# SUSTech-SLAM-XYZZY/SurfelMapping

Hardware: AMD Instinct MI355X
Metric: frames/sec per GPU, 1242x375 KITTI-shaped RGB-D+semantic, full associate+fuse+merge (higher is better)
Workload: dtype f32; 1 GPU; BASELINE configs[1]: KITTI 1242x375 synthetic street sequence, 0.8 m/frame, depth noise 15.0 mm, metricise+conflict+cull+splat+associate+fuse+append per frame; frames=5..6245, multi_gpu=single stream, surfels_start=157613, surfels_end=5487352

## Files before the change

include/sm_c_api.h:

```cpp
#ifndef SM_C_API_H
#define SM_C_API_H

#include <stddef.h>
#include <stdint.h>

#ifdef __cplusplus
extern "C" {
#endif

#define SM_API_VERSION 4

enum {
    SM_OK = 0,
    SM_E_ARG = -1,
    SM_E_CAPACITY = -2,
    SM_E_UNSUPPORTED = -3,
    SM_E_HIP = -4,
    SM_E_NO_DEVICE = -5,
    SM_E_STALL = -6
};

typedef struct sm_config {
    int32_t width, height;
    float fx, fy, cx, cy;
// ... 238 lines not shown
int sm_track_debug_window(sm_ctx *s, const uint16_t *depth_mm, const float *pose16_eval, int32_t min_time, int32_t max_time,
                          int32_t *pred_slot, double *sys29);
int sm_track_frame_rgb_window(sm_ctx *s, const uint8_t *rgb, const uint16_t *depth_mm, const float *guess16, const sm_track_params *params,
                              const sm_track_rgb_params *rgb_params, int32_t min_time, int32_t max_time, float *pose16_out,
                              sm_track_info *info, sm_track_rgb_info *rgb_info, float *anchor_time);
int sm_track_rgb_debug_window(sm_ctx *s, const uint8_t *rgb, const uint16_t *depth_mm, const float *pose16_eval, int level, int which,
                              int32_t min_time, int32_t max_time, int32_t *pred_slot, double *sys29);
int sm_close_loop_rgb(sm_ctx *s, const uint8_t *rgb, const uint16_t *depth_mm, const float *pose16, const sm_map_source *src,
                      const sm_track_params *tp, const sm_track_rgb_params *rp, const sm_loop_params *lp, float *pose16_out,
                      sm_loop_info *info);
int sm_old_in_view(sm_ctx *s, const float *pose16, int32_t max_time, uint32_t *n);
typedef struct sm_auto_loop_params {
    int32_t every, rest;
    uint32_t min_old;
    sm_loop_params loop;
} sm_auto_loop_params;
typedef struct sm_auto_loop_stats_t {
    uint32_t checked, attempts;
    uint32_t closed, none, rejected, failed, no_old_map;
    uint32_t last_census;
    sm_loop_info last;
} sm_auto_loop_stats_t;
int sm_default_auto_loop_params(const sm_config *c, sm_auto_loop_params *p);
int sm_set_auto_loop(sm_ctx *s, const sm_auto_loop_params *p, const sm_map_source *src);
int sm_auto_loop_stats(sm_ctx *s, sm_auto_loop_stats_t *out);

typedef struct sm_search_params {
    int32_t levels;
    float trans_half[3];
    float trans_step[3];
    float rot_half_deg[3];
    float rot_step_deg[3];
    int32_t refine;
    int32_t stride0;
    int32_t top_k;
    float colour_thresh;
} sm_search_params;
typedef struct sm_search_info {
    int32_t status;
    int32_t levels_run;
    uint32_t candidates[4];
    uint32_t best_score[4];
    int32_t winner_rank;
    sm_track_info track;
    float start[16];
    float anchor_time;
    float score_ms, total_ms;
} sm_search_info;
#define SM_SEARCH_MAX_CANDIDATES (1u << 20)
int sm_default_search_params(sm_search_params *p);
int sm_score_poses_window(sm_ctx *s, const uint8_t *rgb, const uint16_t *depth_mm, const float *cand16, uint32_t n,
                          const sm_track_params *tp, int32_t stride, float colour_thresh, int32_t min_time, int32_t max_time,
                          uint32_t *scores);
int sm_search_pose(sm_ctx *s, const uint8_t *rgb, const uint16_t *depth_mm, const float *centre16, const sm_track_params *tp,
                   const sm_track_rgb_params *rp, const sm_search_params *sp, int32_t min_time, int32_t max_time, float *pose16_out,
                   sm_search_info *info);
int sm_close_loop_search(sm_ctx *s, const uint8_t *rgb, const uint16_t *depth_mm, const float *pose16, const sm_map_source *src,
                         const sm_track_params *tp, const sm_track_rgb_params *rp, const sm_loop_params *lp, const sm_search_params *sp,
                         float *pose16_out, sm_loop_info *info);
int sm_set_auto_loop_search(sm_ctx *s, const sm_search_params *sp);

int sm_set_frame(sm_ctx *s, const uint8_t *rgb, const float *depth_metric,
                 const uint8_t *semantic);
int sm_set_tick(sm_ctx *s, int32_t tick);
int sm_stage_conflict(sm_ctx *s, const float *pose16, float min_depth, float max_depth,
                      float fuse_thresh, int is_clean);
int sm_stage_cull(sm_ctx *s);
int sm_stage_splat(sm_ctx *s, const float *pose16, int32_t time, float depth_cutoff,
                   int32_t time_delta);
int sm_stage_associate_fuse(sm_ctx *s, const float *pose16, int32_t time, float depth_min,
                            float depth_max);

int sm_stage_timings(sm_ctx *s, sm_timings *out);
int sm_read_frame_log(sm_ctx *s, sm_frame_log *out, uint32_t n, uint32_t *written);

void *sm_device_alloc(sm_ctx *s, size_t bytes);
int sm_device_free(sm_ctx *s, void *p);
int sm_device_upload(sm_ctx *s, void *dst_device, const void *src_host, size_t bytes);
int sm_export_model_device(sm_ctx *s, void **d_aos, uint32_t *n);
int sm_append_model_aos_device(sm_ctx *s, const float *d_src12, uint32_t n);
int sm_device_download(sm_ctx *s, void *dst_host, const void *src_device, size_t bytes);

int sm_debug_slow_frames(sm_ctx *s, uint32_t *n);
int sm_gpu_process_count(sm_ctx *s);

enum { SM_COLL_SUM = 0, SM_COLL_MIN = 1, SM_COLL_GATHER = 2 };
typedef int (*sm_collective_fn)(void *user, const void *send, void *recv, size_t count, int op, void *hip_stream);
int sm_shard_stream_configure(sm_ctx *s, int rank, int world);
int sm_shard_set_collective(sm_ctx *s, sm_collective_fn fn, void *user);
int sm_shard_rccl_unique_id(void *out128);
int sm_shard_rccl_init(sm_ctx *s, const void *id128);
int sm_shard_rccl_finalize(sm_ctx *s);
int sm_shard_rccl_nranks(sm_ctx *s);
int sm_shard_frame_device(sm_ctx *s, const uint8_t *d_rgb, const uint16_t *d_depth_mm, const uint8_t *d_semantic, const float *pose16);
int sm_shard_frame(sm_ctx *s, const uint8_t *rgb, const uint16_t *depth_mm, const uint8_t *semantic, const float *pose16);
int sm_shard_compact(sm_ctx *s);
int sm_shard_export_dense_device(sm_ctx *s, const float **d_out12, uint32_t *count);

int sm_rig_configure(sm_ctx *s, int rank, int world);
int sm_rig_consolidate(sm_ctx *s, const uint16_t *depth_mm, const uint8_t *semantic, const float *pose16, sm_ctx *global,
                       uint32_t *view_conflicts, uint32_t *total);
int sm_rig_consolidate_step(sm_ctx *s, const uint16_t *depth_mm, const uint8_t *semantic, const float *pose16, sm_ctx *global,
                            uint32_t *new_surfels, uint32_t *global_count);

#ifdef __cplusplus
}
#endif
#endif
```

surfelmapping_amd/capi.py:

```python
from __future__ import annotations

import ctypes as C
import os

import numpy as np

_PKG = os.path.dirname(os.path.abspath(__file__))
LIB_PATH = os.environ.get("SM_HIP_LIB") or os.path.join(_PKG, "libsurfelmapping_hip.so")
API_VERSION = 4

SM_OK, SM_E_ARG, SM_E_CAPACITY, SM_E_UNSUPPORTED, SM_E_HIP, SM_E_NO_DEVICE = 0, -1, -2, -3, -4, -5
TEX_DEPTH_METRIC, TEX_DEPTH_FILTERED, TEX_LAST = 0, 1, 2

SYMBOLS = (
    "sm_api_version", "sm_last_error", "sm_default_config", "sm_create", "sm_destroy",
    "sm_process_frame", "sm_process_frame_device", "sm_process_frame_async",
    "sm_inputs_consumed", "sm_host_alloc", "sm_host_alloc_frame", "sm_host_free", "sm_debug_slow_frames", "sm_sync", "sm_clean_points", "sm_clean_points_ex", "sm_clean_points_cb", "sm_reset",
    "sm_get_counts", "sm_download_model_aos", "sm_upload_model_aos", "sm_save_map", "sm_load_map",
    "sm_download_index_map", "sm_download_raw_cloud", "sm_download_depth", "sm_render_image", "sm_render_model",
    "sm_render_model_device", "sm_render_image_maps", "sm_render_model_maps", "sm_render_maps_stats", "sm_set_frame", "sm_set_tick",
    "sm_stage_conflict", "sm_stage_cull", "sm_stage_splat", "sm_stage_associate_fuse",
    "sm_stage_timings", "sm_read_frame_log", "sm_device_alloc", "sm_device_free", "sm_device_upload",
    "sm_export_model_device", "sm_append_model_aos_device", "sm_device_download",
    "sm_shard_stream_configure", "sm_shard_set_collective", "sm_shard_rccl_unique_id", "sm_shard_rccl_init",
    "sm_shard_rccl_finalize", "sm_shard_rccl_nranks", "sm_shard_frame_device", "sm_shard_frame", "sm_shard_compact", "sm_shard_export_dense_device",
    "sm_gpu_process_count", "sm_rig_configure", "sm_rig_consolidate", "sm_rig_consolidate_step",
    "sm_default_track_params", "sm_track_frame", "sm_track_debug",
    "sm_default_track_rgb_params", "sm_track_frame_rgb", "sm_track_rgb_debug",
    "sm_default_retire_params", "sm_retire", "sm_retire_device", "sm_set_auto_retire", "sm_auto_retire_stats",
    "sm_default_recall_params", "sm_recall", "sm_recall_stats", "sm_set_auto_recall", "sm_auto_recall_stats",
    "sm_warp_by_time", "sm_warp_stats", "sm_loop_spread", "sm_track_frame_old", "sm_track_debug_old",
    "sm_default_loop_params", "sm_close_loop",
    "sm_track_frame_window", "sm_track_debug_window", "sm_track_frame_rgb_window", "sm_track_rgb_debug_window", "sm_close_loop_rgb",
    "sm_old_in_view", "sm_default_auto_loop_params", "sm_set_auto_loop", "sm_auto_loop_stats",
    "sm_default_search_params", "sm_score_poses_window", "sm_search_pose", "sm_close_loop_search", "sm_set_auto_loop_search",
)

SM_COLL_SUM, SM_COLL_MIN, SM_COLL_GATHER = 0, 1, 2
COLLECTIVE_FN = C.CFUNCTYPE(C.c_int, C.c_void_p, C.c_void_p, C.c_void_p, C.c_size_t, C.c_int, C.c_void_p)
CAP_FN = C.CFUNCTYPE(C.c_longlong, C.c_void_p, C.c_uint32)


class SmConfig(C.Structure):
    _fields_ = [
        ("width", C.c_int32), ("height", C.c_int32),
        ("fx", C.c_float), ("fy", C.c_float), ("cx", C.c_float), ("cy", C.c_float),
        ("near_clip", C.c_float), ("far_clip", C.c_float), ("fuse_thresh", C.c_float),
        ("max_sqrt_vertices", C.c_int32), ("time_delta", C.c_int32),
        ("stereo_border", C.c_float), ("preprocess", C.c_int32), ("conflict_cap", C.c_int32),
        ("device", C.c_int32), ("enable_timing", C.c_int32), ("disable_tile_bounds", C.c_int32),
        ("compact_period", C.c_int32),
    ]


class SmCounts(C.Structure):
    _fields_ = [
        ("count", C.c_uint32), ("offset", C.c_uint32), ("data_count", C.c_uint32),
        ("conflict_count", C.c_uint32), ("unstable_count", C.c_uint32),
        ("fused_count", C.c_uint32), ("visible_count", C.c_uint32), ("tick", C.c_int32),
    ]

    def as_dict(self):
        return {n: getattr(self, n) for n, _ in self._fields_}


class SmTimings(C.Structure):
    _fields_ = [(n, C.c_float) for n in (
        "preprocess", "conflict", "index_map", "data_association", "concatenate", "run",
        "k_prep", "k_conflict", "k_scan_cull", "k_compact", "k_associate", "k_scan_new",
        "k_append")] + [("frames", C.c_uint32), ("event_overhead", C.c_float), ("k_compact_own", C.c_float),
                        ("k_cull_lazy", C.c_float), ("frames_compact", C.c_uint32)] + [(n, C.c_float) for n in (
        "k_surfel_pass", "k_pass_fixup", "k_conflict_own", "k_associate_direct", "k_associate_own", "k_append_own")] + [
        ("frames_one_pass", C.c_uint32), ("frames_direct", C.c_uint32), ("k_assoc_prep", C.c_float), ("k_prep_own", C.c_float),
        ("frames_merged", C.c_uint32), ("frames_assoc_alone", C.c_uint32), ("k_scan_own", C.c_float)]

    def as_dict(self):
        return {n: getattr(self, n) for n, _ in self._fields_}


FRAME_LOG_LEN = 1024
FRAME_LOG_DTYPE = np.dtype([(n, np.uint32) for n in (
    "tick", "n_before", "n_after_cull", "n_kill", "conflict_count", "visible_count",
    "fused_count", "unstable_count", "n_static", "n_conf_skipped", "n_splat_skipped", "n_slots")])


class SmModelView(C.Structure):
    _fields_ = [
        ("mvp", C.c_float * 16), ("mv_inv", C.c_float * 16), ("threshold", C.c_float), ("color_type", C.c_int32),
        ("draw_unstable", C.c_int32), ("draw_points", C.c_int32), ("draw_window", C.c_int32), ("time", C.c_int32),
        ("time_delta", C.c_int32), ("width", C.c_int32), ("height", C.c_int32), ("clear_rgba", C.c_uint8 * 4),
    ]


class SmMapSource(C.Structure):
    _fields_ = [("paths", C.POINTER(C.c_char_p)), ("n_paths", C.c_uint32), ("include_model", C.c_int32)]


class SmMapsStats(C.Structure):
    _fields_ = [("surfels_read", C.c_uint64), ("chunks", C.c_uint32), ("passes", C.c_uint32), ("pairs_tested", C.c_uint64),
                ("pairs_skipped", C.c_uint64), ("read_ms", C.c_float), ("copy_ms", C.c_float), ("device_ms", C.c_float),
# ... 229 lines not shown
    def __init__(self, what, rc, detail=""):
        super().__init__(f"{what} failed: rc={rc} {detail}".strip())
        self.rc = rc


_lib = None


def _preload_torch_hip_runtime():
    if os.environ.get("SM_NO_TORCH_HIP_PRELOAD") == "1":
        return
    import importlib.util
    import sys
    if "torch" in sys.modules:
        return
    try:
        spec = importlib.util.find_spec("torch")
    except (ImportError, ValueError):
        return
    if not spec or not spec.submodule_search_locations:
        return
    cand = os.path.join(list(spec.submodule_search_locations)[0], "lib", "libamdhip64.so")
    if os.path.exists(cand):
        try:
            C.CDLL(cand, mode=C.RTLD_GLOBAL)
        except OSError:
            pass


def _choose_rccl():
    if os.environ.get("SM_RCCL_LIB") or os.environ.get("SM_NO_TORCH_HIP_PRELOAD") == "1":
        return
    import importlib.util
    try:
        spec = importlib.util.find_spec("torch")
    except (ImportError, ValueError):
        return
    if spec and spec.submodule_search_locations:
        cand = os.path.join(list(spec.submodule_search_locations)[0], "lib", "librccl.so")
        if os.path.exists(cand):
            os.environ["SM_RCCL_LIB"] = cand


def rccl_unique_id() -> bytes:
    _choose_rccl()
    L = load()
    buf = C.create_string_buffer(128)
    rc = L.sm_shard_rccl_unique_id(buf)
    if rc:
        raise SurfelMapError("sm_shard_rccl_unique_id", rc, L.sm_last_error().decode())
    return buf.raw


def load():
    global _lib
    if _lib is not None:
        return _lib
    if not os.path.exists(LIB_PATH):
        raise ImportError(
            f"{LIB_PATH} is missing: build it with `python -c 'import __graft_entry__ as g; g.build()'` "
            "(make -C surfelmapping_amd/csrc). surfelmapping_amd has no CPU fallback.")
    _preload_torch_hip_runtime()
    L = C.CDLL(LIB_PATH)
    vp, u32p = C.c_void_p, C.POINTER(C.c_uint32)
    L.sm_api_version.restype = C.c_int
    if L.sm_api_version() != API_VERSION:
        raise ImportError(f"{LIB_PATH} has API version {L.sm_api_version()}, this binding expects {API_VERSION}: rebuild it "
                          "(python -c 'import __graft_entry__ as g; g.build()')")
    L.sm_last_error.restype = C.c_char_p
    L.sm_default_config.argtypes = [C.POINTER(SmConfig), C.c_int, C.c_int] + [C.c_float] * 4
    L.sm_create.restype = vp
    L.sm_create.argtypes = [C.POINTER(SmConfig)]
    L.sm_destroy.restype = None
    L.sm_destroy.argtypes = [vp]
    L.sm_process_frame.argtypes = [vp, vp, vp, vp, vp]
    L.sm_process_frame_device.argtypes = [vp, vp, vp, vp, vp]
    L.sm_process_frame_async.argtypes = [vp, vp, vp, vp, vp]
    L.sm_inputs_consumed.argtypes = [vp]
    L.sm_host_alloc.restype = vp
    L.sm_host_alloc.argtypes = [vp, C.c_size_t]
    L.sm_host_free.argtypes = [vp, vp]
    L.sm_host_alloc_frame.argtypes = [vp, C.POINTER(vp), C.POINTER(vp), C.POINTER(vp)]
    L.sm_debug_slow_frames.argtypes = [vp, u32p]
    L.sm_sync.argtypes = [vp]
    L.sm_clean_points.argtypes = [vp, vp, vp, vp]
    L.sm_clean_points_ex.argtypes = [vp, vp, vp, vp, C.c_int]
    L.sm_clean_points_cb.argtypes = [vp, vp, vp, vp, C.c_int, CAP_FN, vp]
    L.sm_reset.argtypes = [vp]
    L.sm_get_counts.argtypes = [vp, C.POINTER(SmCounts)]
    L.sm_download_model_aos.argtypes = [vp, vp, C.c_uint32, u32p]
    L.sm_upload_model_aos.argtypes = [vp, vp, C.c_uint32]
    L.sm_save_map.argtypes = [vp, C.c_char_p, C.c_int32, C.c_int32]
    L.sm_load_map.argtypes = [vp, C.c_char_p, C.POINTER(C.c_int32), C.POINTER(C.c_int32)]
    L.sm_download_index_map.argtypes = [vp, vp, vp, vp, vp]
    L.sm_download_raw_cloud.argtypes = [vp, vp, C.c_uint32, u32p]
    L.sm_download_depth.argtypes = [vp, C.c_int, vp]
    L.sm_render_image.argtypes = [vp, vp, C.c_int, C.c_int] + [C.c_float] * 4 + [vp, vp]
    L.sm_render_model.argtypes = [vp, C.POINTER(SmModelView), vp, vp, vp]
    L.sm_render_model_device.argtypes = [vp, C.POINTER(SmModelView), vp, vp, vp]
    L.sm_render_image_maps.argtypes = [vp, C.POINTER(SmMapSource), vp, C.c_uint32, C.c_int, C.c_int] + [C.c_float] * 4 + [vp, vp]
    L.sm_render_model_maps.argtypes = [vp, C.POINTER(SmMapSource), C.POINTER(SmModelView), C.c_uint32, vp, vp, vp]
    L.sm_render_maps_stats.argtypes = [vp, C.POINTER(SmMapsStats)]
    L.sm_set_frame.argtypes = [vp, vp, vp, vp]
    L.sm_set_tick.argtypes = [vp, C.c_int32]
    L.sm_stage_conflict.argtypes = [vp, vp, C.c_float, C.c_float, C.c_float, C.c_int]
    L.sm_stage_cull.argtypes = [vp]
    L.sm_stage_splat.argtypes = [vp, vp, C.c_int32, C.c_float, C.c_int32]
    L.sm_stage_associate_fuse.argtypes = [vp, vp, C.c_int32, C.c_float, C.c_float]
    L.sm_stage_timings.argtypes = [vp, C.POINTER(SmTimings)]
    L.sm_read_frame_log.argtypes = [vp, vp, C.c_uint32, u32p]
    L.sm_device_alloc.restype = vp
    L.sm_device_alloc.argtypes = [vp, C.c_size_t]
    L.sm_device_free.argtypes = [vp, vp]
    L.sm_device_upload.argtypes = [vp, vp, vp, C.c_size_t]
    L.sm_export_model_device.argtypes = [vp, C.POINTER(vp), u32p]
    L.sm_append_model_aos_device.argtypes = [vp, vp, C.c_uint32]
    L.sm_device_download.argtypes = [vp, vp, vp, C.c_size_t]
    L.sm_shard_stream_configure.argtypes = [vp, C.c_int, C.c_int]
    L.sm_shard_set_collective.argtypes = [vp, COLLECTIVE_FN, vp]
    L.sm_shard_rccl_unique_id.argtypes = [vp]
    L.sm_shard_rccl_init.argtypes = [vp, vp]
    L.sm_shard_rccl_finalize.argtypes = [vp]
    L.sm_shard_rccl_nranks.argtypes = [vp]
    L.sm_shard_frame_device.argtypes = [vp, vp, vp, vp, vp]
    L.sm_shard_frame.argtypes = [vp, vp, vp, vp, vp]
    L.sm_shard_compact.argtypes = [vp]
    L.sm_shard_export_dense_device.argtypes = [vp, C.POINTER(vp), u32p]
    L.sm_gpu_process_count.argtypes = [vp]
    L.sm_rig_configure.argtypes = [vp, C.c_int, C.c_int]
    L.sm_rig_consolidate.argtypes = [vp, vp, vp, vp, vp, u32p, u32p]
    L.sm_rig_consolidate_step.argtypes = [vp, vp, vp, vp, vp, u32p, u32p]
    L.sm_default_track_params.argtypes = [C.POINTER(SmTrackParams)]
    L.sm_track_frame.argtypes = [vp, vp, vp, C.POINTER(SmTrackParams), vp, C.POINTER(SmTrackInfo)]
    L.sm_track_debug.argtypes = [vp, vp, vp, vp, vp]
    L.sm_default_track_rgb_params.argtypes = [C.POINTER(SmTrackRgbParams)]
    L.sm_track_frame_rgb.argtypes = [vp, vp, vp, vp, C.POINTER(SmTrackParams), C.POINTER(SmTrackRgbParams), vp,
                                     C.POINTER(SmTrackInfo), C.POINTER(SmTrackRgbInfo)]
    L.sm_track_rgb_debug.argtypes = [vp, vp, vp, vp, C.c_int, C.c_int, vp]
    L.sm_default_retire_params.argtypes = [C.POINTER(SmConfig), C.POINTER(SmRetireParams)]
    L.sm_retire.argtypes = [vp, vp, C.POINTER(SmRetireParams), vp, C.c_uint32, u32p]
    L.sm_retire_device.argtypes = [vp, vp, C.POINTER(SmRetireParams), vp, C.c_uint32, u32p]
    L.sm_set_auto_retire.argtypes = [vp, C.POINTER(SmRetireParams), C.c_int32, C.c_char_p]
    L.sm_auto_retire_stats.argtypes = [vp, u32p, C.POINTER(C.c_uint64)]
    L.sm_default_recall_params.argtypes = [C.POINTER(SmConfig), C.POINTER(SmRecallParams)]
    L.sm_recall.argtypes = [vp, C.POINTER(SmMapSource), vp, C.POINTER(SmRecallParams), C.c_int32, u32p]
    L.sm_recall_stats.argtypes = [vp, C.POINTER(SmRecallStats)]
    L.sm_set_auto_recall.argtypes = [vp, C.POINTER(SmRecallParams)]
    L.sm_auto_recall_stats.argtypes = [vp, u32p, C.POINTER(C.c_uint64)]
    L.sm_warp_by_time.argtypes = [vp, C.POINTER(SmMapSource), C.c_int32, C.c_uint32, vp]
    L.sm_warp_stats.argtypes = [vp, C.POINTER(SmWarpStats)]
    L.sm_loop_spread.argtypes = [vp, C.c_int32, C.c_int32, vp]
    L.sm_track_frame_old.argtypes = [vp, vp, vp, C.POINTER(SmTrackParams), C.c_int32, vp, C.POINTER(SmTrackInfo), C.POINTER(C.c_float)]
    L.sm_track_debug_old.argtypes = [vp, vp, vp, C.c_int32, vp, vp]
    L.sm_default_loop_params.argtypes = [C.POINTER(SmConfig), C.POINTER(SmLoopParams)]
    L.sm_close_loop.argtypes = [vp, vp, vp, C.POINTER(SmMapSource), C.POINTER(SmTrackParams), C.POINTER(SmLoopParams), vp,
                                C.POINTER(SmLoopInfo)]
    i32, tpp, rpp, lpp = C.c_int32, C.POINTER(SmTrackParams), C.POINTER(SmTrackRgbParams), C.POINTER(SmLoopParams)
    L.sm_track_frame_window.argtypes = [vp, vp, vp, tpp, i32, i32, vp, C.POINTER(SmTrackInfo), C.POINTER(C.c_float)]
    L.sm_track_debug_window.argtypes = [vp, vp, vp, i32, i32, vp, vp]
    L.sm_track_frame_rgb_window.argtypes = [vp, vp, vp, vp, tpp, rpp, i32, i32, vp, C.POINTER(SmTrackInfo), C.POINTER(SmTrackRgbInfo),
                                            C.POINTER(C.c_float)]
    L.sm_track_rgb_debug_window.argtypes = [vp, vp, vp, vp, C.c_int, C.c_int, i32, i32, vp, vp]
    L.sm_close_loop_rgb.argtypes = [vp, vp, vp, vp, C.POINTER(SmMapSource), tpp, rpp, lpp, vp, C.POINTER(SmLoopInfo)]
    L.sm_old_in_view.argtypes = [vp, vp, i32, u32p]
    L.sm_default_auto_loop_params.argtypes = [C.POINTER(SmConfig), C.POINTER(SmAutoLoopParams)]
    L.sm_set_auto_loop.argtypes = [vp, C.POINTER(SmAutoLoopParams), C.POINTER(SmMapSource)]
# ... 11 lines not shown


def _ptr(a):
    return None if a is None else a.ctypes.data_as(C.c_void_p)


def make_config(width, height, fx, fy, cx, cy, **over) -> SmConfig:
    c = SmConfig()
    load().sm_default_config(C.byref(c), width, height, fx, fy, cx, cy)
    for k, v in over.items():
        if not hasattr(c, k):
            raise KeyError(k)
        setattr(c, k, v)
    return c


class SurfelMap:

    def __init__(self, cfg: SmConfig):
        self._L = load()
        self.cfg = cfg
        self.W, self.H = cfg.width, cfg.height
        self.P = self.W * self.H
        self._h = self._L.sm_create(C.byref(cfg))
        if not self._h:
            raise SurfelMapError("sm_create", SM_E_NO_DEVICE, self._L.sm_last_error().decode())

    def _chk(self, rc, what, allow=(0,)):
        if rc not in allow:
            raise SurfelMapError(what, rc, self._L.sm_last_error().decode())
        return rc

    def close(self):
        if getattr(self, "_h", None):
            self._L.sm_destroy(self._h)
            self._h = None

    def __del__(self):
        try:
            self.close()
        except Exception:
            pass

    def process_frame(self, rgb, depth, sem, pose, allow=(0,)):
        rgb = np.ascontiguousarray(rgb, np.uint8)
        depth = None if depth is None else np.ascontiguousarray(depth, np.uint16)
        sem = None if sem is None else np.ascontiguousarray(sem, np.uint8)
        pose = np.ascontiguousarray(pose, np.float32)
        return self._chk(self._L.sm_process_frame(self._h, _ptr(rgb), _ptr(depth), _ptr(sem), _ptr(pose)),
                         "sm_process_frame", allow)

    def process_frame_device(self, d_rgb, d_depth, d_sem, pose):
        pose = np.ascontiguousarray(pose, np.float32)
        return self._chk(self._L.sm_process_frame_device(self._h, d_rgb, d_depth, d_sem, _ptr(pose)),
                         "sm_process_frame_device")

    def process_frame_async(self, rgb, depth, sem, pose):
        assert rgb.dtype == np.uint8 and rgb.flags.c_contiguous
        pose = np.ascontiguousarray(pose, np.float32)
        return self._chk(self._L.sm_process_frame_async(self._h, _ptr(rgb), _ptr(depth), _ptr(sem), _ptr(pose)), "sm_process_frame_async")

    def host_array(self, shape, dtype) -> np.ndarray:
        n = int(np.prod(shape)) * np.dtype(dtype).itemsize
        p = self._L.sm_host_alloc(self._h, n)
        if not p:
            raise SurfelMapError("sm_host_alloc", SM_E_HIP, self._L.sm_last_error().decode())
        buf = (C.c_ubyte * n).from_address(p)
        return np.frombuffer(buf, dtype=dtype).reshape(shape)

    def host_frame(self):
        a, b, c = C.c_void_p(), C.c_void_p(), C.c_void_p()
        self._chk(self._L.sm_host_alloc_frame(self._h, C.byref(a), C.byref(b), C.byref(c)), "sm_host_alloc_frame")
        H, W = self.H, self.W
        rgb = np.frombuffer((C.c_ubyte * (H * W * 3)).from_address(a.value), dtype=np.uint8).reshape(H, W, 3)
        dep = np.frombuffer((C.c_ubyte * (H * W * 2)).from_address(b.value), dtype=np.uint16).reshape(H, W)
        sem = np.frombuffer((C.c_ubyte * (H * W)).from_address(c.value), dtype=np.uint8).reshape(H, W)
        return rgb, dep, sem

    def debug_slow_frames(self) -> int:
        n = C.c_uint32()
        self._chk(self._L.sm_debug_slow_frames(self._h, C.byref(n)), "sm_debug_slow_frames")
        return int(n.value)

    def inputs_consumed(self):
        self._chk(self._L.sm_inputs_consumed(self._h), "sm_inputs_consumed")

    def sync(self, allow=(0,)):
        return self._chk(self._L.sm_sync(self._h), "sm_sync", allow)

    def clean_points(self, depth, sem, pose):
        depth = np.ascontiguousarray(depth, np.uint16)
        sem = np.ascontiguousarray(sem, np.uint8)
        pose = np.ascontiguousarray(pose, np.float32)
        self._chk(self._L.sm_clean_points(self._h, _ptr(depth), _ptr(sem), _ptr(pose)), "sm_clean_points")

    def clean_points_slice(self, depth, sem, pose, exempt_first: bool, cap_hook=None):
        depth = np.ascontiguousarray(depth, np.uint16)
        sem = np.ascontiguousarray(sem, np.uint8)
        pose = np.ascontiguousarray(pose, np.float32)
        if cap_hook is None:
            self._chk(self._L.sm_clean_points_ex(self._h, _ptr(depth), _ptr(sem), _ptr(pose), 1 if exempt_first else 0), "sm_clean_points_ex")
            return
        err = []

        def tramp(user, local):
            try:
                return int(cap_hook(int(local)))
            except Exception as e:
                err.append(e)
                return SM_E_HIP
        cb = CAP_FN(tramp)
        rc = self._L.sm_clean_points_cb(self._h, _ptr(depth), _ptr(sem), _ptr(pose), 1 if exempt_first else 0, cb, None)
        if err:
            raise err[0]
        self._chk(rc, "sm_clean_points_cb")

    def reset(self):
        self._chk(self._L.sm_reset(self._h), "sm_reset")

    def track(self, depth, guess=None, **params):
        depth = np.ascontiguousarray(depth, np.uint16)
        assert depth.size == self.P, depth.shape
        g = None if guess is None else _mat16(guess)
        p = track_params(**params) if params else None
        out = np.zeros(16, np.float32)
        info = SmTrackInfo()
        self._chk(self._L.sm_track_frame(self._h, _ptr(depth), _ptr(g), C.byref(p) if p is not None else None, _ptr(out),
                                         C.byref(info)), "sm_track_frame")
        d = dict(status=TRACK_STATUS.get(info.status, str(info.status)), status_code=int(info.status),
                 iterations=int(info.iterations), inliers=int(info.inliers), rmse=float(info.rmse),
                 guess=np.array(info.guess[:], np.float32).reshape(4, 4).T.copy())
        return out.reshape(4, 4).T.copy(), d

    def track_debug(self, depth, pose_eval):
        depth = np.ascontiguousarray(depth, np.uint16)
        assert depth.size == self.P, depth.shape
        pe = _mat16(pose_eval)
        pred = np.zeros((self.H, self.W), np.int32)
        sys29 = np.zeros(29, np.float64)
        self._chk(self._L.sm_track_debug(self._h, _ptr(depth), _ptr(pe), _ptr(pred), _ptr(sys29)), "sm_track_debug")
        return pred, sys29

    def track_stats(self):
        f = self._L.sm_debug_track_stats
        f.argtypes = [C.c_void_p, C.POINTER(C.c_float), C.c_int, C.POINTER(C.c_int)]
        ms, n = (C.c_float * 256)(), C.c_int()
        self._chk(f(self._h, ms, 256, C.byref(n)), "sm_debug_track_stats")
        return [float(x) for x in ms[:n.value]]

    def process_frame_tracked(self, rgb, depth, sem, guess=None, **params):
        pose, info = self.track(depth, guess, **params)
        self.process_frame(rgb, depth, sem, _mat16(pose))
        return pose, info

    _RGB_KEYS = ("levels", "iters", "rgb_weight", "rgb_max_residual")

    def track_rgb(self, rgb, depth, guess=None, **params):
        rgb = np.ascontiguousarray(rgb, np.uint8)
        depth = np.ascontiguousarray(depth, np.uint16)
        assert depth.size == self.P and rgb.size == self.P * 3, (depth.shape, rgb.shape)
        g = None if guess is None else _mat16(guess)
        icp = {k: v for k, v in params.items() if k not in self._RGB_KEYS}
        col = {k: v for k, v in params.items() if k in self._RGB_KEYS}
        p = track_params(**icp) if icp else None
        q = track_rgb_params(**col) if col else None
        out = np.zeros(16, np.float32)
# ... 551 lines not shown
```

surfelmapping_amd/csrc/sm_api.hip:

```cpp
#include "sm_ctx.h"
#include "sm_kernels.h"

#include <hip/hip_runtime.h>

#include <dirent.h>
#include <link.h>

#include <algorithm>
#include <chrono>
#include <cmath>
#include <cstdio>
#include <cstdlib>
#include <cstring>
#include <atomic>
#include <functional>
#include <memory>
#include <mutex>
#include <string>
#include <thread>
#include <vector>

using namespace sm;

namespace {
// ... 60 lines not shown
    if (sscanf(bus, "%x:%x:%x.%x", &dom, &b, &d, &f) != 4) return -1;
    const unsigned long want_loc = ((unsigned long)b << 8) | ((unsigned long)d << 3) | f;
    unsigned long gpuid = 0;
    bool found = false;
    for (int n = 0; n < 64 && !found; ++n) {
        char path[128];
        snprintf(path, sizeof path, "/sys/class/kfd/kfd/topology/nodes/%d/properties", n);
        FILE *fp = fopen(path, "r");
        if (!fp) { if (n > 16) break; continue; }
        char key[64]; unsigned long val, loc = ~0ul, domain = 0;
        while (fscanf(fp, "%63s %lu", key, &val) == 2) {
            if (!strcmp(key, "location_id")) loc = val;
            else if (!strcmp(key, "domain")) domain = val;
        }
        fclose(fp);
        if (loc == want_loc && domain == dom) {
            snprintf(path, sizeof path, "/sys/class/kfd/kfd/topology/nodes/%d/gpu_id", n);
            FILE *fg = fopen(path, "r");
            if (fg) { found = fscanf(fg, "%lu", &gpuid) == 1 && gpuid != 0; fclose(fg); }
        }
    }
    if (!found) return -1;
    DIR *pd = opendir("/sys/class/kfd/kfd/proc");
    if (!pd) return -1;
    int procs = 0;
    while (struct dirent *pe = readdir(pd)) {
        if (pe->d_name[0] < '0' || pe->d_name[0] > '9') continue;
        char qdir[256];
        snprintf(qdir, sizeof qdir, "/sys/class/kfd/kfd/proc/%s/queues", pe->d_name);
        DIR *qd = opendir(qdir);
        if (!qd) continue;
        bool here = false;
        while (struct dirent *qe = readdir(qd)) {
            if (qe->d_name[0] < '0' || qe->d_name[0] > '9') continue;
            char gp[400];
            snprintf(gp, sizeof gp, "%s/%s/gpuid", qdir, qe->d_name);
            FILE *fg = fopen(gp, "r");
            unsigned long g = 0;
            if (fg) { if (fscanf(fg, "%lu", &g) == 1 && g == gpuid) here = true; fclose(fg); }
            if (here) break;
        }
        closedir(qd);
        if (here) ++procs;
    }
    closedir(pd);
    return procs;
}

bool gpu_shared_with_other_process(int dev)
{
    static std::mutex mu;
    static std::chrono::steady_clock::time_point last[MAX_DEV];
    static int cached[MAX_DEV];
    static bool valid[MAX_DEV] = {};
    if (dev < 0 || dev >= MAX_DEV) return false;
    std::lock_guard<std::mutex> lk(mu);
    const auto now = std::chrono::steady_clock::now();
    if (!valid[dev] || std::chrono::duration_cast<std::chrono::milliseconds>(now - last[dev]).count() > 1000) {
        cached[dev] = kfd_processes_on_gpu(dev);
        last[dev] = now; valid[dev] = true;
    }
    return cached[dev] > 1;
}

bool compaction_needs_tickets(const sm_ctx *s)
{
    const int dev = s->cfg.device;
    if (s->sw.compact_tickets >= 0) return s->sw.compact_tickets != 0;
    if (dev < 0 || dev >= MAX_DEV) return true;
    {
        std::lock_guard<std::mutex> lk(g_compact_mu);
        if (g_ctx_on_dev[dev] > 1) return true;
    }
    return gpu_shared_with_other_process(dev);
}

Switches read_switches()
{
    Switches sw;
    auto off = [](const char *name) { const char *e = std::getenv(name); return e && e[0] == '0'; };
    auto num = [](const char *name, long unset) { const char *e = std::getenv(name); return e ? std::atol(e) : unset; };
    sw.defer_assoc = !off("SM_DEFER_ASSOC");
    sw.two_launch = !off("SM_TWO_LAUNCH");
    sw.pass_split = (int)num("SM_PASS_SPLIT", 0);
    if (const char *e = std::getenv("SM_PASS_TRACE")) { sw.trace = true; sw.trace_prefix = e; }
    if (std::getenv("SM_COMPACT_TICKETS")) sw.compact_tickets = off("SM_COMPACT_TICKETS") ? 0 : 1;
    sw.capacity_wait_us = num("SM_CAPACITY_WAIT_US", 2000);
    sw.check_alive = std::getenv("SM_CHECK_ALIVE") != nullptr;
    if (std::getenv("SM_PASS_WG_PER_CU")) sw.pass_wg_per_cu = (int)std::max(1l, num("SM_PASS_WG_PER_CU", 1));
    if (std::getenv("SM_COMPACT_WG_PER_CU")) sw.compact_wg_per_cu = (int)std::max(1l, num("SM_COMPACT_WG_PER_CU", 1));
    return sw;
}

void resident_grids(const Switches &sw, int device, int *pass_grid, int *compact_grid)
{
    int cus = 0, per_cu = 0;
    if (hipDeviceGetAttribute(&cus, hipDeviceAttributeMultiprocessorCount, device) != hipSuccess || cus <= 0) return;
    if (hipOccupancyMaxActiveBlocksPerMultiprocessor(&per_cu, k_surfel_pass<1>, 256, 0) == hipSuccess && per_cu > 0) {
        const int want = sw.pass_wg_per_cu ? sw.pass_wg_per_cu : std::max(1, per_cu - 1);
        *pass_grid = std::max(256, std::min(cus * want, MAX_GRID));
    }
    if (hipOccupancyMaxActiveBlocksPerMultiprocessor(&per_cu, k_compact<true>, 256, 0) == hipSuccess && per_cu > 0) {
        const int want = sw.compact_wg_per_cu ? std::min(per_cu, sw.compact_wg_per_cu) : std::min(per_cu, 4);
        *compact_grid = std::max(1, cus * want);
    }
}

int alloc_set(SetBufs &b, size_t cap)
{
    return dalloc(b.pos_conf, cap) || dalloc(b.norm_rad, cap) || dalloc(b.color, cap) || dalloc(b.init_time, cap) ||
           dalloc(b.time, cap) ? SM_E_HIP : SM_OK;
}

int grid_surfels(const sm_ctx *s)
{
    return (int)std::min<uint64_t>(std::max<uint64_t>(s->slots.tiles(), 1), MAX_GRID);
}

void check_alive(sm_ctx *s, uint32_t stage)
{
    if (!s->d_chk) return;
    hipLaunchKernelGGL(k_check_alive, dim3(64), dim3(256), 0, s->stream, s->d_state, s->d_alive, s->d_tile_dead, s->d_chk, stage);
}

int take_error(sm_ctx *s)
{
    if (s->h_state->error != 0) {
        const int e = s->h_state->error;
        s->h_state->error = 0;
        HIPCK(hipMemcpyAsync(&s->d_state->error, &s->h_state->error, sizeof(int32_t), hipMemcpyHostToDevice, s->stream));
        HIPCK(hipStreamSynchronize(s->stream));
        g_err = e == SM_E_CAPACITY ? "model capacity (MAX_VERTICES) exceeded; frame's new surfels dropped"
              : e == SM_E_UNSUPPORTED ? "unsupported operation flagged on the device"
              : "device-side error";
        return e;
    }
    return SM_OK;
}


static inline uint32_t assoc_wgs(const sm_ctx *s)
{
    return (uint32_t)(s->n_pix_blocks + 1) / 2u;
}

int launch_fixup(sm_ctx *s, const FrameParams &fp, const FixArgs &x)
{
    hipLaunchKernelGGL(k_pass_fixup, dim3(x.n_crew + 1), dim3(256), 0, s->stream, s->M, s->d_state, fp, x);
    HIPCK(hipGetLastError());
    return SM_OK;
}

int launch_assoc(sm_ctx *s, const AssocArgs &a, uint32_t stage)
{
    hipLaunchKernelGGL((k_associate_direct<false>), dim3(assoc_wgs(s)), dim3(PIX_BLOCK), 0, s->stream, a, ShardArgs{});
    HIPCK(hipGetLastError());
    check_alive(s, stage + 16u * (uint32_t)(s->tick & 0xFFFF));
    return SM_OK;
}

int launch_settle(sm_ctx *s, const ShardSettle &ss)
{
    hipLaunchKernelGGL(k_shard_settle, dim3(ss.n), dim3(PIX_BLOCK), 0, s->stream, ss);
    HIPCK(hipGetLastError());
    return SM_OK;
}
// ... 2 lines not shown
{
    FixArgs *fx;
    if (const AssocArgs *a = s->held.take_assoc(fx)) {
        if (fx && launch_fixup(s, a->fp, *fx)) return SM_E_HIP;
        if (launch_assoc(s, *a, 3u)) return SM_E_HIP;
    }
    if (!all) return SM_OK;
    if (const ShardSettle *ss = s->held.take_settle()) if (launch_settle(s, *ss)) return SM_E_HIP;
    if (uint32_t *nf = s->held.take_stats()) {
        hipLaunchKernelGGL(k_frame_finalize, dim3(1), dim3(256), 0, s->stream, s->d_state, nf, s->part.fix_cur(), s->part.n_fix, s->d_log);
        HIPCK(hipGetLastError());
    }
    return SM_OK;
}

int launch_prep(sm_ctx *s, const uint8_t *rgb, const uint16_t *raw, const uint8_t *sem, const FrameParams &fp, bool clear_keys,
                bool tile_flags = false, bool carry = false, const ChainArgs *chain = nullptr)
{
    const int tiles = ((s->W + 31) / 32) * ((s->H + 31) / 32);
    TilePrep tp{};
    const uint64_t ntl = s->slots.tiles();
    const FrameSet &f = s->cur();
    if (clear_keys && tile_flags) {
        tp.nfb = (uint32_t)std::min<uint64_t>(std::max<uint64_t>((ntl + 1023) / 1024, 1), 64);
        tp.st = s->d_state; tp.tb = s->d_tb; tp.tile_flags = f.tile_flags; tp.wave_cnt = f.wave_cnt; tp.prep_part = f.prep_part;
    }
    FixArgs *fxp = nullptr;
    AssocArgs *carried = carry ? s->held.take_assoc(fxp) : nullptr;
    s->tl.frame().merged = carried || chain;
    uint32_t *conf_sub = clear_keys ? f.conf_sub : nullptr;
    if (carried || chain) {
        if (const ShardSettle *ss = chain ? s->held.take_settle() : nullptr) if (launch_settle(s, *ss)) return SM_E_HIP;
        static const AssocArgs none{};
        const AssocArgs &a = carried ? *carried : none;
        if (tp.nfb) {
            tp.nfb = (uint32_t)std::min<uint64_t>(std::max<uint64_t>((ntl + 255) / 256, 1), 128);
            if (carried) { tp.grp_cand = a.grp_cand; tp.n_grp = a.n_grp; tp.prev_time = a.fp.time; }
        }
        const FixArgs fx = fxp ? *fxp : FixArgs{};
        const uint32_t n_fix = fxp ? 1u + fx.n_crew : 0u;
        if (fxp) {
            carried->slow_conf_sub = fx.conf_sub; carried->slow_need = n_fix;
            if (tp.nfb) { tp.slow_conf_sub = fx.conf_sub; tp.slow_cap = a.fp.conflict_cap; tp.slow_need = n_fix; tp.slow_par = a.fp.par; }
        }
        PrepArgs pa;
        pa.rgb = rgb; pa.depth_raw = raw; pa.sem = sem; pa.depth_f32 = nullptr; pa.depthT = f.depthT; pa.rgbsT = f.rgbsT;
        pa.keyT = clear_keys ? s->keyT() : nullptr; pa.dcT = f.dcT;
        pa.conf_sub = conf_sub;
        const uint32_t n_assoc = carried ? assoc_wgs(s) : 0u;
        const ChainArgs ca = chain ? *chain : ChainArgs{};
        const uint32_t n_img = chain ? (uint32_t)(((s->W + CH_TX - 1) / CH_TX) * ((s->H + CH_TY - 1) / CH_TY)) : (uint32_t)tiles;
        if (s->d_ap_trace) { s->ap_trace_n[0] = (int)n_assoc; s->ap_trace_n[1] = (int)tp.nfb; s->ap_trace_n[2] = (int)n_img; s->ap_trace_n[3] = (int)n_fix; }
        const dim3 grid(n_fix + tp.nfb + n_assoc + n_img);
        const auto assoc_prep = chain ? k_assoc_prep<true> : k_assoc_prep<false>;
        hipLaunchKernelGGL(assoc_prep, grid, dim3(PIX_BLOCK), 0, s->stream, a, pa, fp, tp, n_assoc, n_img, ca, fx, n_fix, s->d_ap_trace);
        HIPCK(hipGetLastError());
        return (int)tp.nfb;
    }
    const ShardSettle *held = s->held.take_settle();
    const ShardSettle ss = held ? *held : ShardSettle{};
    hipLaunchKernelGGL(k_prep, dim3(tiles + tp.nfb + (ss.n + 3u) / 4u), dim3(1024), 0, s->stream, rgb, raw, sem, (const float *)nullptr, f.depthT, f.rgbsT,
                       clear_keys ? s->keyT() : nullptr, fp, f.dcT, conf_sub, tp, ss);
    HIPCK(hipGetLastError());
    return (int)tp.nfb;
}

int launch_conflict_test(sm_ctx *s, const FrameParams &fp, bool timed = false)
{
    if (finalize_if_pending(s)) return SM_E_HIP;
    s->n_conf_part = (uint32_t)grid_surfels(s);
    hipLaunchKernelGGL(k_conflict, dim3(s->n_conf_part), dim3(256), 0, s->stream, s->M, s->d_state, fp, s->cur().dcT,
                       s->d_cm, s->d_dm, s->d_zm, s->d_tile_cnt, s->d_tb, s->cur().tile_flags, s->d_conf_part, s->d_alive,
                       s->cur().conf_sub);
    HIPCK(hipGetLastError());
    if (s->tl.mark(s->stream, 2, timed)) return SM_E_HIP;
    return SM_OK;
}

int launch_conflict_finalize(sm_ctx *s, const FrameParams &fp, bool timed = false)
{
    if (fp.compact_now) {
        const int ngroups = std::max<int>(1, (int)((s->slots.tiles() + GROUP - 1) / GROUP));
        hipLaunchKernelGGL(k_scan_cull, dim3(ngroups), dim3(1024), 0, s->stream, s->d_state, s->d_tile_cnt, s->d_tile_allow,
                           s->d_tile_keep, s->d_group_tot, s->d_tile_dead);
        HIPCK(hipGetLastError());
    }
    hipLaunchKernelGGL(k_cull_finalize, dim3(1), dim3(1024), 0, s->stream, s->d_state, fp, s->d_cm, s->d_dm, s->d_zm,
                       s->d_tile_cnt, s->d_tile_allow, s->d_tile_keep, s->d_group_tot, s->d_group_base, s->d_conf_part, s->n_conf_part,
                       s->d_alive, s->d_tile_dead, s->d_stat);
    HIPCK(hipGetLastError());
    if (s->tl.mark(s->stream, 3, timed)) return SM_E_HIP;
    return SM_OK;
}

int launch_conflict(sm_ctx *s, const FrameParams &fp, bool timed = false)
{
    int rc = launch_conflict_test(s, fp, timed);
    if (rc) return rc;
    return launch_conflict_finalize(s, fp, timed);
}

struct PassGrid { int split, grid, fix_workers; };

PassGrid pass_grid_policy(sm_ctx *s, bool two, bool direct)
{
    const uint64_t tiles_b = s->slots.tiles_of(s->slots.estimate_slots());
    const bool persistent = tiles_b > (uint64_t)(4 * MAX_GRID);
    PassGrid g;
    g.split = s->sw.pass_split == 1 || s->sw.pass_split == 4 ? s->sw.pass_split : persistent ? 1 : 4;
    g.grid = persistent ? std::min(grid_surfels(s), s->pass_grid) : grid_surfels(s);
    if (g.split == 4) {
        const int max_seq = 3 * MAX_GRID / 16;
        g.grid = 4 * (int)std::min<uint64_t>(std::max<uint64_t>(s->slots.tiles(), 1), (uint64_t)max_seq);
    }
    g.fix_workers = two ? (int)sm_ctx::N_CREW
                  : direct ? std::max(std::min(g.grid, s->fix_grid), (int)std::min<uint32_t>(s->n_grp, MAX_GRID)) : std::min(g.grid, s->fix_grid);
    return g;
}

int launch_surfel_pass(sm_ctx *s, const FrameParams &fp, bool timed, bool direct, uint32_t n_prep)
{
    if (n_prep == 0) { g_err = "internal: one-pass frame without tile flags from the preparation launch"; return SM_E_ARG; }
    const bool two = s->sw.two_launch && s->defer_ok && timed && direct;
    const PassGrid g = pass_grid_policy(s, two, direct);
    const int grid = g.grid;
    PassPartials &pp = s->part;
    const uint32_t n_fix_prev = pp.n_fix;
    const uint2 *fix_prev = pp.fix_cur();
    pp.fix_set ^= 1;
    s->n_conf_part = (uint32_t)grid;
    pp.n_compact = (uint32_t)grid;
    pp.pass_live = true;
    pp.n_fix = (uint32_t)g.fix_workers;
    const FrameSet &f = s->cur();
    uint32_t *sub = f.conf_sub;
    const uint32_t tile_bound = (uint32_t)std::max<uint64_t>(s->slots.tiles(), 1);
    if (s->d_pass_trace) s->pass_trace_grid = grid;
    CandArgs ca{};
    ca.n_pass = (uint32_t)grid;
    if (two) {
        ca.n_grp = s->n_grp; ca.cg = s->cand_group; ca.n_pix_blocks = s->n_pix_blocks;
        ca.depthT = f.depthT; ca.xs = s->d_xs; ca.ys = s->d_ys; ca.blk_cand = s->d_blk_cand; ca.grp_cand = s->d_grp_cand;
    }
    const auto pass = g.split == 4 ? k_surfel_pass<4> : k_surfel_pass<1>;
    hipLaunchKernelGGL(pass, dim3(grid + (two ? (int)s->n_grp : 0)), dim3(256), 0, s->stream, s->M, s->d_state, fp, f.dcT, s->d_cm, s->d_dm ,
                       f.wave_cnt, s->d_tb, f.tile_flags, pp.d_lazy, s->d_alive, s->d_tile_dead, sub, s->keyT(), s->d_undo, tile_bound,
                       s->d_frame_sub, ca, s->d_pass_trace);
    HIPCK(hipGetLastError());
    if (s->tl.mark(s->stream, 2, timed) || s->tl.mark(s->stream, 3, timed)) return SM_E_HIP;
    FixArgs x{};
    DirectArgs &da = x.da;
    da.on = direct ? (two ? 2 : 1) : 0;
    da.blk_cand = s->d_blk_cand; da.grp_cand = s->d_grp_cand; da.n_grp = s->n_grp; da.cg = s->cand_group; da.n_pix_blocks = s->n_pix_blocks;
    da.depthT = f.depthT; da.xs = s->d_xs; da.ys = s->d_ys;
    da.frame_sub = s->d_frame_sub;
    da.nf_prev = s->prev().nf_sub;
    da.fix_prev = fix_prev; da.n_fix_prev = s->held.take_stats() ? n_fix_prev : 0u;
    da.log = s->d_log;
    x.cm = s->d_cm; x.km = s->d_dm; x.wave_cnt = f.wave_cnt; x.tile_flags = f.tile_flags; x.part = pp.d_lazy; x.n_part = (uint32_t)grid;
    x.fix_part = pp.fix_cur(); x.alive = s->d_alive; x.tile_dead = s->d_tile_dead; x.conf_sub = sub; x.keyT = s->keyT(); x.undo = s->d_undo;
    x.host_stat = s->d_stat; x.prep_part = f.prep_part; x.n_prep = n_prep; x.tb = s->d_tb; x.n_crew = (uint32_t)g.fix_workers;
    if (two) s->held.hold_fixup(x);
    else if (launch_fixup(s, fp, x)) return SM_E_HIP;
    if (s->tl.mark(s->stream, 4, timed)) return SM_E_HIP;
    check_alive(s, 1u + 16u * (uint32_t)(s->tick & 0xFFFF));
    return SM_OK;
}

void fill_assoc_args(const sm_ctx *s, const FrameParams &fp, AssocArgs &a)
{
    a.M = s->M; a.st = s->d_state; a.fp = fp;
    const FrameSet &f = s->cur();
    a.depthT = f.depthT; a.rgbsT = f.rgbsT; a.keyT = s->keyT(); a.xs = s->d_xs; a.ys = s->d_ys;
    a.blk_cand = s->d_blk_cand; a.grp_cand = s->d_grp_cand; a.nf = f.nf_sub; a.tb = s->d_tb;
    a.alive = s->d_alive; a.tile_dead = s->d_tile_dead; a.n_grp = s->n_grp; a.cg = s->cand_group; a.host_stat = s->d_stat;
    a.slow_conf_sub = nullptr; a.slow_need = 0u;
}

int launch_associate_direct(sm_ctx *s, const FrameParams &fp, bool timed)
{
    AssocArgs a;
    fill_assoc_args(s, fp, a);
    s->tl.frame().deferred = s->defer_ok;
    if (s->defer_ok && timed) s->held.hold_assoc(a);
    else if (launch_assoc(s, a, 2u)) return SM_E_HIP;
    s->part.clear();
    s->held.hold_stats(s->cur().nf_sub);
    s->slots.append_enqueued();
    if (s->tl.mark(s->stream, 5, timed) || s->tl.mark(s->stream, 6, timed) || s->tl.mark(s->stream, 7, timed)) return SM_E_HIP;
    return SM_OK;
}

int launch_compact(sm_ctx *s, const FrameParams &fp, bool splat, bool timed)
{
    s->part.clear();
    if (!fp.compact_now) {
        if (splat) { g_err = "internal: a frame's cull that only marks the dead is k_surfel_pass"; return SM_E_ARG; }
        const int grid = grid_surfels(s);
        s->part.n_compact = 0u;
        hipLaunchKernelGGL(k_cull_lazy, dim3(grid), dim3(256), 0, s->stream, s->M, s->d_state, fp, s->d_cm, s->d_dm, s->d_zm,
                           s->d_tile_cnt, s->d_tile_allow, s->d_alive, s->d_tile_dead);
        HIPCK(hipGetLastError());
        if (s->tl.mark(s->stream, 4, timed)) return SM_E_HIP;
        return SM_OK;
    }
    const int grid = std::min(grid_surfels(s), s->compact_grid);
    const uint32_t epoch = s->slots.next_cull_epoch();
    if (!fp.maintenance) s->part.n_compact = splat ? (uint32_t)grid : 0u;
    FrameParams fpc = fp;
    fpc.compact_tickets = compaction_needs_tickets(s) ? 1 : 0;
    const auto compact = splat ? k_compact<true> : k_compact<false>;
    hipLaunchKernelGGL(compact, dim3(grid), dim3(256), 0, s->stream, s->M, s->d_state, fpc, s->d_cm,
                       s->d_dm, s->d_zm, s->d_tile_cnt, s->d_tile_allow, s->d_tile_keep, s->keyT(), s->d_tile_flag, epoch,
                       s->d_group_base, s->d_tb, s->cur().tile_flags, s->part.d_compact, s->d_alive, s->d_tile_dead);
    HIPCK(hipGetLastError());
    if (s->tl.mark(s->stream, 4, timed)) return SM_E_HIP;
    return SM_OK;
}

int launch_post_fill(sm_ctx *s)
{
    hipLaunchKernelGGL(k_post_fill, dim3(1024), dim3(256), 0, s->stream, s->d_state, s->d_alive, s->d_tile_dead);
    HIPCK(hipGetLastError());
    check_alive(s, 4u + 16u * (uint32_t)(s->tick & 0xFFFF));
    return SM_OK;
}

int ss_compact(sm_ctx *s);

int launch_associate_only(sm_ctx *s, const FrameParams &fp)
{
    hipLaunchKernelGGL(k_associate, dim3(s->n_pix_blocks), dim3(PIX_BLOCK), 0, s->stream, s->M, s->d_state, fp,
                       s->cur().depthT, s->cur().rgbsT, s->keyT(), s->d_xs, s->d_ys, s->d_validmask, s->d_fusedmask, s->d_blk_cnt, s->d_tb);
    HIPCK(hipGetLastError());
    return SM_OK;
}

int launch_associate(sm_ctx *s, const FrameParams &fp, bool timed)
{
    int rc = launch_associate_only(s, fp);
    if (rc) return rc;
    if (s->tl.mark(s->stream, 5, timed) || s->tl.mark(s->stream, 6, timed)) return SM_E_HIP;
    const PassPartials::Fold f = s->part.fold();
    hipLaunchKernelGGL(k_append_scan, dim3(s->n_pix_blocks), dim3(PIX_BLOCK), 0, s->stream, s->M, s->d_state, fp, s->cur().depthT,
                       s->cur().rgbsT, s->d_xs, s->d_ys, s->d_validmask, s->d_fusedmask, s->d_blk_cnt, s->d_log, s->d_tb, f.compact,
                       f.n_compact, s->d_alive, s->d_tile_dead, s->d_stat, f.lazy, f.fix, f.n_fix);
    s->part.clear();
    s->slots.append_enqueued();
    HIPCK(hipGetLastError());
    if (s->tl.mark(s->stream, 7, timed)) return SM_E_HIP;
    check_alive(s, 5u + 16u * (uint32_t)(s->tick & 0xFFFF));
    return SM_OK;
}

int discard_model(sm_ctx *s)
{
    int rc = pull_state(s);
    if (rc) return rc;
    if (s->h_state->count == 0 && !s->slots.maybe_garbage() && s->h_state->conflict_count == 0 && s->h_state->visible_count == 0) return SM_OK;
    if (s->slots.maybe_garbage()) {
        HIPCK(hipMemsetAsync(s->d_alive, 0xFF, s->alive_words * 8, s->stream));
        HIPCK(hipMemsetAsync(s->d_tile_dead, 0, s->dead_tiles * 4, s->stream));
        s->slots.model_discarded();
    }
    s->h_state->conflict_count = 0; s->h_state->visible_count = 0;
    return publish_dense(s, 0, 0);
}

void end_frame(sm_ctx *s, bool timed = true)
{
    if (s->cfg.preprocess) std::swap(s->d_lastT, s->d_filteredT);
    memcpy(s->last_pose, s->curr_pose, 64);
    s->tl.end_frame(timed);
    s->tick++;
}

int begin_frame(sm_ctx *s, const uint8_t *d_rgb, const uint16_t *d_raw, const uint8_t *d_sem, const float *pose, bool tile_flags, bool carry,
                FrameParams *fp_out, uint32_t *n_prep)
{
    if (s->pending_cull) { g_err = "sm_stage_conflict without sm_stage_cull"; return SM_E_ARG; }
    memcpy(s->curr_pose, pose, 64);
    s->trk.note_pose(pose);
    FrameParams fp = make_params(s, pose);
    const bool fusing = s->ref_set && s->tick != 0;
    int rc;
    if ((rc = s->tl.mark(s->stream, 8, fusing))) return rc;
    if ((rc = s->tl.mark(s->stream, 0, fusing))) return rc;
    const bool will_splat = fusing;
    s->plane_set ^= 1;
    fp.par = s->plane_set;
    if (s->defer_ok && will_splat) s->key_set ^= 1;
    ChainArgs ca{};
    if (s->cfg.preprocess) {
        ca.lastT = s->d_lastT; ca.filteredT = s->d_filteredT; memcpy(ca.w, s->h_wtab, sizeof ca.w);
        ca.border = (int)std::ceil(s->cfg.stereo_border - 0.5f);
        ca.do_movings = s->ref_set ? 1 : 0;
        if (s->ref_set) {
            float linv[16];
            invert4(s->last_pose, linv);
            mul4(linv, s->curr_pose, ca.t_c2l.m);
        }
    }
    if ((rc = launch_prep(s, d_rgb, d_raw, d_sem, fp, will_splat, tile_flags, carry, s->cfg.preprocess ? &ca : nullptr)) < 0) return rc;
    *n_prep = (uint32_t)rc;
    if (!s->ref_set) {
        if (s->cfg.preprocess) std::swap(s->d_lastT, s->d_filteredT);
        memcpy(s->last_pose, s->curr_pose, 64);
        s->ref_set = true;
        s->tick++;
        return 0;
    }
    if ((rc = s->tl.mark(s->stream, 1, fusing))) return rc;
    s->raw_valid = true;
    s->raw_tick = s->tick;
    if (s->tick == 0) {
        fp.init_mode = 1;
        fp.log_frame = 0;
        if ((rc = discard_model(s))) return rc;
        s->part.clear();
        s->part.n_compact = 0;
        if ((rc = launch_associate(s, fp, false))) return rc;
        end_frame(s, false);
        return 0;
    }
    fp.splat_follows = 1;
    fp.log_frame = 1;
    *fp_out = fp;
    return 1;
}

int enqueue_frame(sm_ctx *s, const uint8_t *d_rgb, const uint16_t *d_raw, const uint8_t *d_sem, const float *pose)
{
    if (s->ss_on) { g_err = "context is configured for sharding: use the sm_shard_* entry points"; return SM_E_ARG; }
    FrameParams fp;
    const bool fusing = s->ref_set && s->tick != 0 && !s->pending_cull;
    const bool compact_now = fusing ? s->slots.decide_compact() : true;
    const bool carry = fusing && s->defer_ok;
    int rc = SM_OK;
    uint32_t n_prep = 0;
    if (!carry && (rc = complete_held(s, false))) return rc;
    rc = begin_frame(s, d_rgb, d_raw, d_sem, pose, fusing && !compact_now, carry, &fp, &n_prep);
    if (rc <= 0) return rc;
    fp.compact_now = compact_now ? 1u : 0u;
    s->slots.cull_noted(fp.compact_now != 0u);
    s->slots.keys_drawn(fp.compact_now == 0u);
    const bool one_pass = !fp.compact_now;
    Timeline::Flags &fl = s->tl.frame();
    fl.compacted = !one_pass; fl.one_pass = fl.direct = one_pass;
    if (one_pass) {
        if ((rc = launch_surfel_pass(s, fp, true, true, n_prep))) return rc;
        if ((rc = launch_associate_direct(s, fp, true))) return rc;
        end_frame(s);
        return SM_OK;
    }
    if ((rc = launch_conflict(s, fp, true))) return rc;
    if ((rc = launch_compact(s, fp, true, true))) return rc;
    if ((rc = launch_associate(s, fp, true))) return rc;
    end_frame(s);
    return SM_OK;
}

int upload_inputs(sm_ctx *s, const uint8_t *rgb, const uint16_t *depth, const uint8_t *sem)
{
    const size_t P = (size_t)s->P;
    hipStream_t st = s->stream;
    if (rgb) HIPCK(hipMemcpyAsync(s->d_rgb, rgb, P * 3, hipMemcpyHostToDevice, st));
    if (depth) HIPCK(hipMemcpyAsync(s->d_depth_raw, depth, P * 2, hipMemcpyHostToDevice, st));
    if (sem) HIPCK(hipMemcpyAsync(s->d_sem, sem, P, hipMemcpyHostToDevice, st));
    return SM_OK;
}

int alloc_frame_set(sm_ctx *s, FrameSet &f)
{
    auto get = [s](auto *&p, size_t n, bool zero) -> int {
        Dev<void> m;
        const size_t bytes = std::max<size_t>(n, 1) * sizeof *p;
        HIPCK(hipMalloc(m.put(), bytes));
        if (zero) HIPCK(hipMemset(m, 0, bytes));
        p = static_cast<std::remove_reference_t<decltype(p)>>(m.get());
        s->frame_mem.push_back(std::move(m));
        return SM_OK;
    };
    const size_t P = (size_t)s->P;
    return get(f.depthT, P, true) || get(f.rgbsT, P, true) || get(f.dcT, P, true) || get(f.tile_flags, s->tb_tiles, true) ||
           get(f.wave_cnt, s->dead_tiles, false) || get(f.prep_part, 256, false) ? SM_E_HIP : SM_OK;
}

int alloc_ctx(sm_ctx *s)
{
    const size_t P = (size_t)s->P, cap = s->cap, nwords = s->alive_words, ntiles = s->dead_tiles, tb = s->tb_tiles;
    if (hipStreamCreateWithFlags(s->stream.put(), hipStreamNonBlocking) != hipSuccess ||
        alloc_set(s->m_bufs[0], cap) ||
        dalloc(s->d_state, 1) || dalloc(s->d_log, FRAME_LOG_LEN) || hipHostMalloc(s->h_state.put(), sizeof(DevState), hipHostMallocDefault) != hipSuccess ||
        hipHostMalloc(s->h_stat.put(), 8, hipHostMallocMapped) != hipSuccess || hipHostGetDevicePointer((void **)&s->d_stat, s->h_stat, 0) != hipSuccess ||
        dalloc(s->d_filteredT, P) || dalloc(s->d_lastT, P) ||
        alloc_frame_set(s, s->fset[0]) || dalloc(s->d_key[0], P) ||
        (s->defer_ok && (alloc_frame_set(s, s->fset[1]) || dalloc(s->d_key[1], P))) ||
        dalloc(s->d_rgb, P * 3) || dalloc(s->d_sem, P) || dalloc(s->d_depth_raw, P) || dalloc(s->d_depth_f32, P) ||
        dalloc(s->d_xs, (size_t)s->W * 2) || dalloc(s->d_ys, (size_t)s->H * 2) ||
        dalloc(s->d_cm, nwords) || dalloc(s->d_dm, nwords) || dalloc(s->d_zm, nwords) ||
        dalloc(s->d_alive, nwords) || hipMemset(s->d_alive, 0xFF, nwords * 8) != hipSuccess ||
        dalloc(s->d_tile_dead, ntiles) || hipMemset(s->d_tile_dead, 0, ntiles * 4) != hipSuccess ||
        dalloc(s->d_tile_cnt, ntiles * 3) || dalloc(s->d_tile_allow, ntiles) || dalloc(s->d_tile_keep, ntiles) || dalloc(s->d_tile_flag, ntiles) ||
        hipMemset(s->d_tile_flag, 0, ntiles * 4) != hipSuccess ||
        dalloc(s->d_group_tot, (ntiles / GROUP + 2) * 4) || dalloc(s->d_group_base, ntiles / GROUP + 2) ||
        dalloc(s->d_conf_part, (size_t)MAX_GRID * 4) || dalloc(s->part.d_compact, (size_t)MAX_GRID) || dalloc(s->part.d_lazy, (size_t)MAX_GRID) ||
        dalloc(s->part.d_fix, (size_t)MAX_GRID * 2 + 2) || dalloc(s->d_undo, cap + TILE) ||
        dalloc(s->d_conf_sub, (size_t)2 * SUB_SET) || hipMemset(s->d_conf_sub, 0, (size_t)2 * SUB_SET * 4) != hipSuccess ||
        dalloc(s->d_tb, tb * 8) ||
        dalloc(s->d_validmask, (P + 63) / 64 + 4) || dalloc(s->d_fusedmask, (P + 63) / 64 + 4) || dalloc(s->d_blk_cnt, (size_t)s->n_pix_blocks) ||
        dalloc(s->d_blk_cand, (size_t)s->n_grp * CAND_GROUP_MAX) || dalloc(s->d_grp_cand, (size_t)s->n_grp) ||
        dalloc(s->d_frame_sub, (size_t)6 * SUB_SET) || hipMemset(s->d_frame_sub, 0, (size_t)6 * SUB_SET * 4) != hipSuccess)
        return SM_E_HIP;
    s->M.s[0] = s->m_bufs[0].view();
    *s->h_stat = 0ull;
    for (int i = 0; i < 2; ++i) { s->fset[i].nf_sub = s->d_frame_sub + (2 + 2 * i) * SUB_SET; s->fset[i].conf_sub = s->d_conf_sub + i * SUB_SET; }
    if (!s->defer_ok) s->alias_frame_sets();
    return SM_OK;
}

}


void sm_impl::invert4(const float *m, float *out)
{
    float a[16];
    a[0] = m[5] * m[10] * m[15] - m[5] * m[11] * m[14] - m[9] * m[6] * m[15] + m[9] * m[7] * m[14] +
           m[13] * m[6] * m[11] - m[13] * m[7] * m[10];
    a[4] = -m[4] * m[10] * m[15] + m[4] * m[11] * m[14] + m[8] * m[6] * m[15] - m[8] * m[7] * m[14] -
           m[12] * m[6] * m[11] + m[12] * m[7] * m[10];
    a[8] = m[4] * m[9] * m[15] - m[4] * m[11] * m[13] - m[8] * m[5] * m[15] + m[8] * m[7] * m[13] +
           m[12] * m[5] * m[11] - m[12] * m[7] * m[9];
    a[12] = -m[4] * m[9] * m[14] + m[4] * m[10] * m[13] + m[8] * m[5] * m[14] - m[8] * m[6] * m[13] -
// ... 22 lines not shown
            m[8] * m[1] * m[7] + m[8] * m[3] * m[5];
    a[15] = m[0] * m[5] * m[10] - m[0] * m[6] * m[9] - m[4] * m[1] * m[10] + m[4] * m[2] * m[9] +
            m[8] * m[1] * m[6] - m[8] * m[2] * m[5];
    const float det = m[0] * a[0] + m[1] * a[4] + m[2] * a[8] + m[3] * a[12];
    const float rdet = 1.0f / det;
    for (int i = 0; i < 16; ++i) out[i] = a[i] * rdet;
}

FrameParams sm_impl::make_params(const sm_ctx *s, const float *pose)
{
    FrameParams fp;
    memset(&fp, 0, sizeof fp);
    memcpy(fp.pose, pose, 64);
    invert4(pose, fp.t_inv);
    const sm_config &c = s->cfg;
    fp.fx = c.fx; fp.fy = c.fy; fp.cx = c.cx; fp.cy = c.cy;
    fp.inv_fx = (float)(1.0 / (double)c.fx);
    fp.inv_fy = (float)(1.0 / (double)c.fy);
    fp.cols = (float)c.width; fp.rows = (float)c.height;
    fp.W = c.width; fp.H = c.height; fp.P = s->P;
    fp.min_depth = c.near_clip; fp.max_depth = c.far_clip;
    fp.conflict_thresh = c.fuse_thresh;
    fp.fuse_thresh = c.fuse_thresh;
    fp.stereo_border = c.stereo_border;
    fp.is_clean = 0;
    fp.time = s->tick;
    fp.time_delta = c.time_delta;
    fp.depth_cutoff = c.far_clip;
    fp.conflict_cap = c.conflict_cap ? (uint32_t)s->P : 0xFFFFFFFFu;
    fp.max_vertices = s->cap;
    fp.init_mode = 0;
    fp.inv_fx_fb = 1.0f / c.fx;
    fp.inv_fy_fb = 1.0f / c.fy;
    fp.use_bounds = c.disable_tile_bounds ? 0 : 1;
    fp.compact_now = 1;
    fp.maintenance = 0;
    fp.par = s->plane_set;
    return fp;
}

int sm_impl::push_state(sm_ctx *s)
{
    HIPCK(hipMemcpyAsync(s->d_state, s->h_state, sizeof(DevState), hipMemcpyHostToDevice, s->stream));
    HIPCK(hipStreamSynchronize(s->stream));
    s->slots.state_pushed(s->h_state->stat_frames, s->h_state->count);
    return SM_OK;
}

int sm_impl::finalize_if_pending(sm_ctx *s)
{
    return complete_held(s, true);
}

int sm_impl::pull_state(sm_ctx *s)
{
    int rcf = finalize_if_pending(s);
    if (rcf) return rcf;
    HIPCK(hipMemcpyAsync(s->h_state, s->d_state, sizeof(DevState), hipMemcpyDeviceToHost, s->stream));
    HIPCK(hipStreamSynchronize(s->stream));
    const DevState &d = *s->h_state;
    s->counts.count = s->pending_cull ? s->count_before_cull : d.count - d.garbage;
    s->counts.offset = d.offset - (d.garbage - d.holes_last);
    s->counts.data_count = d.data_count;
    s->counts.conflict_count = d.conflict_count;
    s->counts.unstable_count = d.unstable_count;
    s->counts.fused_count = d.fused_count;
    s->counts.visible_count = d.visible_count;
    s->counts.tick = s->tick;
    s->slots.state_pulled(d.count, d.cull_n, s->pending_cull);
    return SM_OK;
}

int sm_impl::ensure_compact(sm_ctx *s)
{
    if (finalize_if_pending(s)) return SM_E_HIP;
    if (s->ss_on) {
        int rc = ss_compact(s);
        if (rc) return rc;
        HIPCK(hipStreamSynchronize(s->stream));
        return SM_OK;
    }
    if (!s->slots.maybe_garbage()) return SM_OK;
    if (s->pending_cull) { g_err = "internal: deferred compaction with a pending per-pass cull"; return SM_E_ARG; }
    FrameParams fp = make_params(s, s->curr_pose);
    fp.maintenance = 1;
    fp.compact_now = 1;
    fp.conflict_cap = 0xFFFFFFFFu;
    const uint64_t tiles = s->slots.tiles() + 1;
    const size_t words = std::min<size_t>(tiles * TILE_WORDS, s->alive_words);
    HIPCK(hipMemsetAsync(s->d_cm, 0, words * 8, s->stream));
    HIPCK(hipMemsetAsync(s->d_dm, 0, words * 8, s->stream));
    HIPCK(hipMemsetAsync(s->d_zm, 0, words * 8, s->stream));
    HIPCK(hipMemsetAsync(s->d_tile_cnt, 0, std::min<size_t>(tiles, s->dead_tiles) * 12, s->stream));
    const int ngroups = std::max<int>(1, (int)((tiles + GROUP - 1) / GROUP));
    hipLaunchKernelGGL(k_scan_cull, dim3(ngroups), dim3(1024), 0, s->stream, s->d_state, s->d_tile_cnt, s->d_tile_allow,
                       s->d_tile_keep, s->d_group_tot, s->d_tile_dead);
    hipLaunchKernelGGL(k_cull_finalize, dim3(1), dim3(1024), 0, s->stream, s->d_state, fp, s->d_cm, s->d_dm, s->d_zm,
                       s->d_tile_cnt, s->d_tile_allow, s->d_tile_keep, s->d_group_tot, s->d_group_base, s->d_conf_part, 0u,
                       s->d_alive, s->d_tile_dead, s->d_stat);
    if (s->slots.keys_are_slots())
        hipLaunchKernelGGL(k_remap_keys, dim3((s->P + 255) / 256), dim3(256), 0, s->stream, s->d_state, s->keyT(), s->P, s->d_alive,
                           s->d_tile_keep, s->d_group_base);
    HIPCK(hipGetLastError());
    int rc = launch_compact(s, fp, false, false);
    if (rc) return rc;
    if ((rc = launch_post_fill(s))) return rc;
    s->slots.compacted_outside_frame();
    HIPCK(hipStreamSynchronize(s->stream));
    return SM_OK;
}

int sm_impl::rebuild_bounds(sm_ctx *s, uint32_t first_surfel, uint32_t count)
{
    const uint32_t t0 = first_surfel / TILE;
    if (t0 < s->tb_tiles) {
        const uint32_t n = s->tb_tiles - t0;
        hipLaunchKernelGGL(k_tile_bounds_reset, dim3((n + 255) / 256), dim3(256), 0, s->stream, s->d_tb, t0, n);
        HIPCK(hipGetLastError());
    }
    const uint32_t k0 = t0 * TILE;
    if (count > k0) {
        hipLaunchKernelGGL(k_tile_bounds_build, dim3((count - k0 + 255) / 256), dim3(256), 0, s->stream, s->M, s->d_state, s->d_tb, k0);
        HIPCK(hipGetLastError());
    }
    HIPCK(hipStreamSynchronize(s->stream));
    return SM_OK;
}

int sm_impl::publish_dense(sm_ctx *s, uint32_t count, uint32_t first_new)
{
    DevState &d = *s->h_state;
    d.count = count;
    d.offset = count;
    d.garbage = 0; d.garbage_prev = 0; d.first_live = 0; d.do_compact = 0;
    s->slots.published_dense();
    int rc = push_state(s);
    if (rc) return rc;
    if ((rc = rebuild_bounds(s, first_new, count))) return rc;
    return pull_state(s);
}

int sm_impl::ensure_export(sm_ctx *s, size_t bytes)
{
    s->rm.scratch_reused();
    if (bytes <= s->export_bytes) return SM_OK;
    s->export_bytes = 0;
    HIPCK(hipMalloc(s->d_export.put(), bytes));
    s->export_bytes = bytes;
    return SM_OK;
}

void sm_impl::fill_keys(sm_ctx *s, uint64_t *key, size_t n)
{
    hipLaunchKernelGGL(k_fill_keys, dim3((unsigned)((n + 255) / 256)), dim3(256), 0, s->stream, key, (int)n);
}

int sm_impl::clean_points_device(sm_ctx *s, const uint16_t *d_depth_mm, const uint8_t *d_semantic, const float *pose16, int exempt_first,
                                 const std::function<long long(uint32_t)> *cap_hook)
{
    if (s->pending_cull) { g_err = "sm_stage_conflict without sm_stage_cull"; return SM_E_ARG; }
    int rc = ensure_compact(s);
    if (rc) return rc;
    memcpy(s->curr_pose, pose16, 64);
    FrameParams fp = make_params(s, pose16);
    if ((rc = launch_prep(s, s->d_rgb, d_depth_mm, d_semantic, fp, false)) < 0) return rc;
    fp.max_depth = s->cfg.far_clip - 15.0f;
    fp.conflict_thresh = 0.1f;
    fp.is_clean = 1;
    fp.no_exempt = exempt_first ? 0 : 1;
    fp.compact_now = s->slots.decide_compact() ? 1u : 0u;
    if ((rc = launch_conflict_test(s, fp))) return rc;
    if (cap_hook) {
        std::vector<uint32_t> part((size_t)s->n_conf_part * 4);
        HIPCK(hipMemcpyAsync(part.data(), s->d_conf_part, part.size() * 4, hipMemcpyDeviceToHost, s->stream));
        HIPCK(hipStreamSynchronize(s->stream));
        uint64_t local = 0;
        for (uint32_t b = 0; b < s->n_conf_part; ++b) local += part[(size_t)b * 4 + 1];
        const long long allow = (*cap_hook)((uint32_t)local);
        if (allow < 0) return (int)allow;
        fp.conflict_cap = (uint32_t)std::min<long long>(allow, 0xFFFFFFFFll);
    }
    s->slots.cull_noted(fp.compact_now != 0u);
    if ((rc = launch_conflict_finalize(s, fp))) return rc;
    if ((rc = launch_compact(s, fp, false, false))) return rc;
    if ((rc = launch_post_fill(s))) return rc;
    return sm_sync(s);
}
// ... 386 lines not shown
    int rc = s->pending_cull ? SM_OK : ensure_compact(s);
    if (rc) return rc;
    if ((rc = pull_state(s))) return rc;
    if (s->pending_cull) {
        s->h_state->count = s->h_state->cull_n;
        s->h_state->cur = s->h_state->cull_src;
        s->h_state->offset = s->offset_before_cull;
        s->pending_cull = false;
        if ((rc = push_state(s))) return rc;
        if ((rc = pull_state(s))) return rc;
    }
    memcpy(s->curr_pose, pose16, 64);
    FrameParams fp = make_params(s, pose16);
    fp.min_depth = min_depth; fp.max_depth = max_depth; fp.conflict_thresh = fuse_thresh; fp.is_clean = is_clean;
    s->count_before_cull = s->h_state->count;
    s->offset_before_cull = s->h_state->offset;
    if ((rc = launch_conflict(s, fp))) return rc;
    s->pending_cull = true;
    return sm_sync(s);
}

int sm_stage_cull(sm_ctx *s)
{
    if (!s) return SM_E_ARG;
    HIPCK(hipSetDevice(s->cfg.device));
    if (!s->pending_cull) { g_err = "sm_stage_cull without sm_stage_conflict"; return SM_E_ARG; }
    FrameParams fp = make_params(s, s->curr_pose);
    int rc = launch_compact(s, fp, false, false);
    if (rc) return rc;
    s->pending_cull = false;
    return sm_sync(s);
}

int sm_stage_splat(sm_ctx *s, const float *pose16, int32_t time, float depth_cutoff, int32_t time_delta)
{
    if (!s || !pose16) return SM_E_ARG;
    HIPCK(hipSetDevice(s->cfg.device));
    if (s->pending_cull) { g_err = "sm_stage_splat between sm_stage_conflict and sm_stage_cull"; return SM_E_ARG; }
    int rc = ensure_compact(s);
    if (rc) return rc;
    if ((rc = pull_state(s))) return rc;
    memcpy(s->curr_pose, pose16, 64);
    FrameParams fp = make_params(s, pose16);
    fp.time = time; fp.depth_cutoff = depth_cutoff; fp.time_delta = time_delta;
    HIPCK(hipMemsetAsync(&s->d_state->visible_count, 0, 4, s->stream));
    s->part.clear();
    s->part.n_compact = 0;
    fill_keys(s, s->keyT(), s->P);
    HIPCK(hipGetLastError());
    const int grid = (int)std::min<uint64_t>(std::max<uint64_t>(((uint64_t)s->h_state->count + 255) / 256, 1), MAX_GRID);
    hipLaunchKernelGGL(k_splat, dim3(grid), dim3(256), 0, s->stream, s->M, s->d_state, fp, s->keyT());
    HIPCK(hipGetLastError());
    return sm_sync(s);
}

int sm_stage_associate_fuse(sm_ctx *s, const float *pose16, int32_t time, float depth_min, float depth_max)
{
    if (!s || !pose16) return SM_E_ARG;
    HIPCK(hipSetDevice(s->cfg.device));
    if (s->pending_cull) { g_err = "sm_stage_associate_fuse between sm_stage_conflict and sm_stage_cull"; return SM_E_ARG; }
    memcpy(s->curr_pose, pose16, 64);
    FrameParams fp = make_params(s, pose16);
    fp.time = time; fp.min_depth = depth_min; fp.max_depth = depth_max;
    int rc = ensure_compact(s);
    if (rc) return rc;
    if ((rc = launch_associate(s, fp, false))) return rc;
    return sm_sync(s);
}

int sm_stage_timings(sm_ctx *s, sm_timings *out)
{
    if (!s || !out) return SM_E_ARG;
    memset(out, 0, sizeof *out);
    if (!s->tl.ev) { g_err = "sm_stage_timings: create the context with enable_timing=1"; return SM_E_UNSUPPORTED; }
    HIPCK(hipSetDevice(s->cfg.device));
    HIPCK(hipStreamSynchronize(s->stream));
    Timeline &tl = s->tl;
    uint64_t first = tl.read;
    if (tl.frames - first > EV_RING) first = tl.frames - EV_RING;
    double seg[7] = {0}, run = 0, ovh = 0, cull[2] = {0, 0};
    double own[6] = {0};
    double prep2[2] = {0, 0};
    double scan_own = 0;
    uint32_t nfr = 0, ncls[2] = {0, 0}, n_op = 0, n_dir = 0, n_merged = 0, n_alone = 0;
    for (uint64_t f = first; f < tl.frames; ++f) {
        const int slot = (int)(f % EV_RING);
        const Timeline::Flags &fl = tl.flags[slot];
        float ms = 0;
        bool ok = true;
        double loc[7];
        for (int k = 0; k < 7 && ok; ++k) {
            ok = hipEventElapsedTime(&ms, tl.ev[k][slot], tl.ev[k + 1][slot]) == hipSuccess;
            loc[k] = ms;
        }
        float o = 0;
        if (!ok || hipEventElapsedTime(&ms, tl.ev[0][slot], tl.ev[7][slot]) != hipSuccess ||
            hipEventElapsedTime(&o, tl.ev[8][slot], tl.ev[0][slot]) != hipSuccess)
            continue;
        for (int k = 0; k < 7; ++k) seg[k] += loc[k];
        cull[fl.compacted ? 1 : 0] += loc[3];
        ncls[fl.compacted ? 1 : 0]++;
        if (fl.one_pass) { own[0] += loc[1]; own[1] += loc[3]; n_op++; } else { own[2] += loc[1]; scan_own += loc[2]; }
        if (fl.direct) { n_dir++; if (!fl.deferred) { own[3] += loc[4]; n_alone++; } } else { own[4] += loc[4]; own[5] += loc[6]; }
        prep2[fl.merged ? 1 : 0] += loc[0];
        if (fl.merged) n_merged++;
        run += ms;
        ovh += o;
        nfr++;
    }
    tl.read = tl.frames;
    out->frames = nfr;
    if (nfr) {
        const double inv = 1.0 / nfr;
        const double oh = ovh * inv;
        out->event_overhead = (float)oh;
        for (double &x : seg) x = std::max(0.0, x - oh * nfr);
        out->k_prep = (float)(seg[0] * inv); out->k_conflict = (float)(seg[1] * inv); out->k_scan_cull = (float)(seg[2] * inv);
        out->k_compact = (float)(seg[3] * inv); out->k_associate = (float)(seg[4] * inv); out->k_scan_new = (float)(seg[5] * inv);
        out->k_append = (float)(seg[6] * inv);
        out->k_cull_lazy = ncls[0] ? (float)std::max(0.0, cull[0] / ncls[0] - oh) : 0.0f;
        out->k_compact_own = ncls[1] ? (float)std::max(0.0, cull[1] / ncls[1] - oh) : 0.0f;
        out->frames_compact = ncls[1];
        auto avg = [&](double sum, uint32_t n) { return n ? (float)std::max(0.0, sum / n - oh) : 0.0f; };
        out->k_surfel_pass = avg(own[0], n_op); out->k_pass_fixup = avg(own[1], n_op); out->k_conflict_own = avg(own[2], nfr - n_op);
        out->k_scan_own = avg(scan_own, nfr - n_op);
        out->k_associate_direct = avg(own[3], n_alone); out->k_associate_own = avg(own[4], nfr - n_dir); out->k_append_own = avg(own[5], nfr - n_dir);
        out->frames_one_pass = n_op; out->frames_direct = n_dir;
        out->k_assoc_prep = avg(prep2[1], n_merged); out->k_prep_own = avg(prep2[0], nfr - n_merged);
        out->frames_merged = n_merged; out->frames_assoc_alone = n_alone;
        out->preprocess = out->k_prep;
        out->conflict = out->k_conflict + out->k_scan_cull + out->k_compact;
        out->index_map = 0.0f;
        out->data_association = out->k_associate;
        out->concatenate = out->k_scan_new + out->k_append;
        out->run = (float)(run * inv);
    }
    return SM_OK;
}

int sm_read_frame_log(sm_ctx *s, sm_frame_log *out, uint32_t n, uint32_t *written)
{
    if (!s || !out || !written) return SM_E_ARG;
    static_assert(sizeof(sm_frame_log) == sizeof(FrameLog), "frame log layout");
    static_assert(SM_FRAME_LOG_LEN == FRAME_LOG_LEN, "frame log length");
    HIPCK(hipSetDevice(s->cfg.device));
    int rc = pull_state(s);
    if (rc) return rc;
    const uint32_t total = s->h_state->frames_logged;
    uint32_t m = std::min(std::min(n, total), (uint32_t)FRAME_LOG_LEN);
    std::vector<FrameLog> ring(FRAME_LOG_LEN);
    HIPCK(hipMemcpy(ring.data(), s->d_log, sizeof(FrameLog) * FRAME_LOG_LEN, hipMemcpyDeviceToHost));
    for (uint32_t k = 0; k < m; ++k) {
        const uint32_t idx = (total - m + k) % FRAME_LOG_LEN;
        memcpy(&out[k], &ring[idx], sizeof(FrameLog));
    }
    *written = m;
    return SM_OK;
}

int sm_debug_slow_frames(sm_ctx *s, uint32_t *n)
{
    if (!s || !n) return SM_E_ARG;
    HIPCK(hipSetDevice(s->cfg.device));
    int rc = pull_state(s);
    if (rc) return rc;
    *n = s->h_state->slow_frames;
    return SM_OK;
}

int sm_gpu_process_count(sm_ctx *s)
{
    if (!s) return SM_E_ARG;
    return kfd_processes_on_gpu(s->cfg.device);
}

}


int sm_impl::ss_collective(sm_ctx *s, const void *send, void *recv, size_t count, int op)
{
    if (!s->ss_coll) {
        if (s->ss_world == 1) {
            if (send != recv) HIPCK(hipMemcpyAsync(recv, send, count * 8, hipMemcpyDeviceToDevice, s->stream));
            return SM_OK;
        }
        g_err = "sharded stream: no collective installed (sm_shard_rccl_init or sm_shard_set_collective)";
        return SM_E_ARG;
    }
    const int rc = s->ss_coll(s->ss_user, send, recv, count, op, s->stream);
    if (rc && g_err.empty()) g_err = "sharded stream: the collective callback failed";
    return rc;
}

namespace {

int ss_compact(sm_ctx *s)
{
    if (finalize_if_pending(s)) return SM_E_HIP;
    const uint64_t nw = ((uint64_t)s->slots.bound() + 63) / 64;
    const uint64_t tiles = s->slots.tiles();
    const int g1 = (int)std::min<uint64_t>(std::max<uint64_t>((nw + 255) / 256, 1), 1024);
    const int gt = (int)std::min<uint64_t>(std::max<uint64_t>(tiles, 1), MAX_GRID);
    hipLaunchKernelGGL(k_shard_alive_copy, dim3(g1), dim3(256), 0, s->stream, s->d_state, s->d_alive, s->d_galive, s->d_new_alive, (uint32_t)nw);
    HIPCK(hipGetLastError());
    int rc = ss_collective(s, s->d_galive, s->d_galive, (size_t)nw, SM_COLL_SUM);
    if (rc) return rc;
    hipLaunchKernelGGL(k_shard_tile_popc, dim3(std::max(1, std::min(gt / 16 + 1, 256))), dim3(256), 0, s->stream, s->d_state, s->d_galive, s->d_tile_keep);
    hipLaunchKernelGGL(k_shard_scan, dim3(1), dim3(1024), 0, s->stream, s->d_state, s->d_tile_keep, s->d_tile_allow, s->d_ss_info, s->d_stat);
    hipLaunchKernelGGL(k_shard_stage, dim3(gt), dim3(256), 0, s->stream, s->M, s->d_state, s->d_alive, s->d_galive, s->d_tile_allow, s->d_ss_info,
                       s->d_new_alive);
    hipLaunchKernelGGL(k_shard_unstage, dim3(gt), dim3(256), 0, s->stream, s->M, s->d_state, s->d_ss_info, s->d_new_alive, s->d_alive,
                       s->d_tile_dead, s->d_tb);
    HIPCK(hipGetLastError());
    s->slots.compacted_sharded();
    s->part.clear();
    return SM_OK;
}

}

extern "C" {

int sm_shard_stream_configure(sm_ctx *s, int rank, int world)
{
    if (!s || world < 1 || rank < 0 || rank >= world) return SM_E_ARG;
    HIPCK(hipSetDevice(s->cfg.device));
    if (s->ss_on) { g_err = "sm_shard_stream_configure: already configured"; return SM_E_ARG; }
    int rc = pull_state(s);
    if (rc) return rc;
    if (s->h_state->count != 0 || s->slots.maybe_garbage() || s->tick != 0 || s->ref_set) {
        g_err = "sm_shard_stream_configure: the context must be new (no frame, no model)";
        return SM_E_ARG;
    }
    SetBufs set1;
    Dev<uint64_t> galive, new_alive, gmask, capx;
    Dev<uint32_t> info;
    if ((rc = alloc_set(set1, s->cap)) || (rc = dalloc(galive, s->alive_words)) || (rc = dalloc(new_alive, s->alive_words)) ||
        (rc = dalloc(gmask, (size_t)(s->P + 63) / 64 + 4)) || (rc = dalloc(info, 4)) ||
        (rc = dalloc(capx, (size_t)1 + (size_t)(2 + TILE_WORDS) * s->dead_tiles)))
        return rc;
    HIPCK(hipMemset(info, 0, 16));
    s->M.s[1] = set1.view();
    s->m_bufs[1] = std::move(set1);
    s->d_galive = std::move(galive); s->d_new_alive = std::move(new_alive); s->d_gmask = std::move(gmask);
    s->d_ss_info = std::move(info); s->d_capx = std::move(capx);
    s->ss_on = true; s->ss_rank = rank; s->ss_world = world; s->ss_frames = 0;
    s->aloop.on = false;
    s->defer_ok = false;
    s->alias_frame_sets();
    return SM_OK;
}

int sm_shard_set_collective(sm_ctx *s, sm_collective_fn fn, void *user)
{
    if (!s || !(s->ss_on || s->rig_on)) { g_err = "sm_shard_set_collective: call sm_shard_stream_configure or sm_rig_configure first"; return SM_E_ARG; }
    s->ss_coll = fn; s->ss_user = user;
    return SM_OK;
}

int sm_shard_compact(sm_ctx *s)
{
    if (!s || !s->ss_on) return SM_E_ARG;
    HIPCK(hipSetDevice(s->cfg.device));
    return ss_compact(s);
}

int sm_shard_frame_device(sm_ctx *s, const uint8_t *d_rgb, const uint16_t *d_depth_mm, const uint8_t *d_semantic, const float *pose16)
{
    if (!s || !d_rgb || !pose16) { g_err = "sm_shard_frame_device: null argument"; return SM_E_ARG; }
    if (!s->ss_on) { g_err = "sm_shard_frame_device: call sm_shard_stream_configure first"; return SM_E_ARG; }
    HIPCK(hipSetDevice(s->cfg.device));
    if (s->pending_cull) { g_err = "sm_stage_conflict without sm_stage_cull"; return SM_E_ARG; }
    if (s->ref_set && s->tick == 0) { g_err = "reset() is not supported in sharded mode"; return SM_E_UNSUPPORTED; }
    const bool fusing = s->ref_set && s->tick != 0;
    int rc;
    if (fusing) {
        bool compact = s->slots.period_due();
        if (!compact && s->slots.bound_may_overflow()) {
            if ((rc = pull_state(s))) return rc;
            compact = s->slots.bound_may_overflow();
        }
        if (compact && s->slots.culls_since_compact() > 0) {
            if ((rc = ss_compact(s))) return rc;
            if (s->slots.bound_may_overflow() && (rc = pull_state(s))) return rc;
        }
    }
    FrameParams fp;
    uint32_t n_prep = 0;
    rc = begin_frame(s, d_rgb, d_depth_mm ? d_depth_mm : s->d_depth_raw, d_semantic ? d_semantic : s->d_sem, pose16, fusing, false, &fp, &n_prep);
    if (rc <= 0) return rc;
    fp.compact_now = 0u;
    fp.conflict_cap = 0xFFFFFFFFu;
    fp.shard_slots = 1;
    s->slots.cull_noted(false);
    s->slots.keys_drawn(true);
    Timeline::Flags &fl = s->tl.frame();
    fl.compacted = false; fl.one_pass = fl.direct = true;
    if ((rc = launch_surfel_pass(s, fp, true, true, n_prep))) return rc;
    if (s->cfg.conflict_cap && (uint64_t)s->slots.bound() > (uint64_t)s->P) {
        const uint32_t tbnd = (uint32_t)std::min<uint64_t>(s->slots.tiles(), s->dead_tiles);
        const int gp = (int)std::min<uint32_t>(std::max<uint32_t>((tbnd * (uint32_t)TILE_WORDS + 255u) / 256u, 1u), 1024u);
        hipLaunchKernelGGL(k_shard_cap_pack, dim3(gp), dim3(256), 0, s->stream, s->d_state, s->cur().wave_cnt, s->d_cm,
                           s->cur().conf_sub, s->d_capx, tbnd);
        HIPCK(hipGetLastError());
        if ((rc = ss_collective(s, s->d_capx, s->d_capx, (size_t)1 + (size_t)(2 + TILE_WORDS) * tbnd, SM_COLL_SUM))) return rc;
        hipLaunchKernelGGL(k_shard_cap_repair, dim3(std::min<uint32_t>(std::max<uint32_t>(tbnd, 1u), (uint32_t)MAX_GRID)), dim3(256), 0, s->stream, s->M,
                           s->d_state, fp, s->d_capx, tbnd, (uint32_t)s->P, s->cur().wave_cnt, s->d_dm , s->cur().tile_flags, s->d_alive,
                           s->d_tile_dead, s->keyT(), s->d_undo, s->d_tb);
        HIPCK(hipGetLastError());
    }
    if ((rc = ss_collective(s, s->keyT(), s->keyT(), (size_t)s->P, SM_COLL_MIN))) return rc;
    ShardArgs sh;
    sh.validmask = s->d_validmask; sh.ownmask = s->d_fusedmask; sh.gmask = s->d_gmask; sh.nwords = (uint32_t)((s->P + 63) / 64);
    sh.owner = (int)(s->ss_frames % (uint32_t)s->ss_world) == s->ss_rank ? 1 : 0;
    AssocArgs aa;
    fill_assoc_args(s, fp, aa);
    hipLaunchKernelGGL((k_associate_direct<true>), dim3(assoc_wgs(s)), dim3(PIX_BLOCK), 0, s->stream, aa, sh);
    HIPCK(hipGetLastError());
    if ((rc = s->tl.mark(s->stream, 5, true))) return rc;
    if ((rc = ss_collective(s, s->d_gmask, s->d_gmask, (size_t)sh.nwords + 4, SM_COLL_SUM))) return rc;
    ShardSettle ss;
    ss.n = (uint32_t)s->n_pix_blocks; ss.st = s->d_state; ss.validmask = s->d_validmask; ss.ownmask = s->d_fusedmask; ss.gmask = s->d_gmask;
    ss.nwords = sh.nwords; ss.blk_cand = s->d_blk_cand; ss.grp_cand = s->d_grp_cand; ss.nf = s->cur().nf_sub; ss.alive = s->d_alive;
    ss.tile_dead = s->d_tile_dead; ss.owner = sh.owner; ss.cap_pixels = s->cfg.conflict_cap ? (uint32_t)s->P : 0xFFFFFFFFu; ss.max_vertices = s->cap; ss.cg = s->cand_group;
    s->held.hold_settle(ss);
    if ((rc = s->tl.mark(s->stream, 6, true)) || (rc = s->tl.mark(s->stream, 7, true))) return rc;
    s->part.clear();
    s->held.hold_stats(s->cur().nf_sub);
    s->slots.append_enqueued();
    s->ss_frames++;
    end_frame(s);
    return SM_OK;
}

int sm_shard_frame(sm_ctx *s, const uint8_t *rgb, const uint16_t *depth_mm, const uint8_t *semantic, const float *pose16)
{
    if (!s || !rgb || !pose16) { g_err = "sm_shard_frame: null argument"; return SM_E_ARG; }
    HIPCK(hipSetDevice(s->cfg.device));
    int rc = upload_inputs(s, rgb, depth_mm, semantic);
    if (rc) return rc;
    if ((rc = sm_shard_frame_device(s, s->d_rgb, s->d_depth_raw, s->d_sem, pose16))) return rc;
    return sm_sync(s);
}

int sm_shard_export_dense_device(sm_ctx *s, const float **d_out12, uint32_t *count)
{
    if (!s || !d_out12 || !count || !s->ss_on) return SM_E_ARG;
    HIPCK(hipSetDevice(s->cfg.device));
    if (hip_runtime_conflict("sm_shard_export_dense_device")) return SM_E_HIP;
    int rc = ensure_compact(s);
    if (rc) return rc;
    if ((rc = pull_state(s))) return rc;
    const uint32_t n = s->h_state->count;
    if ((rc = ensure_export(s, (size_t)std::max<uint32_t>(n, 1) * 48))) return rc;
    if (n) hipLaunchKernelGGL(k_shard_export_aos, dim3((n + 255) / 256), dim3(256), 0, s->stream, s->M, s->d_state, s->d_alive, (float *)s->d_export.get(), n);
    HIPCK(hipGetLastError());
    HIPCK(hipStreamSynchronize(s->stream));
    *d_out12 = (const float *)s->d_export.get();
    *count = n;
    return SM_OK;
}

}
```

surfelmapping_amd/csrc/sm_ctx.h:

```cpp
#pragma once

#include "../../include/sm_c_api.h"
#include "sm_device.h"
#include "sm_slots.h"

#include <hip/hip_runtime.h>

#include <algorithm>
#include <cassert>
#include <cmath>
#include <cstdio>
#include <cstring>
#include <functional>
#include <map>
#include <memory>
#include <string>
#include <utility>
#include <vector>

namespace sm { struct TrackState; struct TrackRgbState; struct RenderParams; struct ViewParams; struct ViewShade; struct RecallChunk; struct WarpChunk; }

namespace sm_impl __attribute__((visibility("hidden"))) {

using namespace sm;
// ... 88 lines not shown
};

struct Retire {
    Dev<uint64_t> d_mask;
    Dev<uint32_t> d_tile_ret, d_tile_base, d_total;
    int32_t every = 0;
    sm_retire_params params{};
    std::string prefix;
    Host<float> h_stage;
    uint32_t files = 0;
    uint64_t surfels = 0;
    int32_t last_tick = 0;
    bool timed = false, stats_valid = false;
    Event ev[8];
};

struct RenderMaps {
    static constexpr uint32_t CHUNK = 1u << 20;
    Stream copy;
    Host<float4> h_rec[2];
    Dev<float4> d_rec[2];
    Event ev_copy0[2], ev_copied[2];
    Event ev_k0[2], ev_k1[2];
    Dev<float4> d_pos_conf, d_norm_rad, d_box;
    Dev<uint32_t> d_color;
    Dev<float> d_time;
    Dev<uint8_t> d_par;
    size_t par_bytes = 0;
    sm_maps_stats stats{};
    bool stats_valid = false;
};

struct Recall {
    struct Entry { uint64_t size; int64_t mtime_ns; float lo[3], hi[3]; float max_time; };
    std::map<std::string, Entry> index;
    Dev<uint64_t> d_mask;
    Dev<uint32_t> d_blk_cnt, d_blk_base, d_run;
    Dev<float4> d_box;
    Dev<RecallChunk> d_chunk;
    Host<RecallChunk> h_chunk;
    sm_recall_stats_t stats{};
    bool stats_valid = false;
    float radius = 0.0f;
    uint32_t rounds = 0;
    uint64_t surfels = 0;
};

struct Warp {
    Dev<float4> d_corr;
    size_t corr_rows = 0;
    Dev<float4> d_box;
    Dev<uint32_t> d_sel;
    Dev<WarpChunk> d_chunk;
    Host<WarpChunk> h_chunk;
    Event ev[2];
    sm_warp_stats_t stats{};
    bool stats_valid = false;
};

struct Search {
    Dev<uint8_t> d_rgb;
    Dev<float4> d_samp;
    Dev<float4> d_plane;
    Dev<uint32_t> d_nsamp;
    Dev<float> d_cand;
    Dev<uint32_t> d_scores;
    size_t cand_cap = 0;
    Event ev[2];
};

struct AutoLoop {
    bool on = false;
    bool search = false;
    sm_search_params sp{};
    sm_auto_loop_params p{};
    std::vector<std::string> paths;
    int64_t rest_until = 0;
    sm_auto_loop_stats_t stats{};
};

struct Switches {
    bool defer_assoc = true;
    bool two_launch = true;
    int pass_split = 0;
    bool trace = false;
    std::string trace_prefix;
    int compact_tickets = -1;
    long capacity_wait_us = 2000;
    bool check_alive = false;
    int pass_wg_per_cu = 0;
    int compact_wg_per_cu = 0;
};

class HeldBack {
public:
    void hold_fixup(const FixArgs &x) { assert(!has_fix_ && !has_assoc_); fix_ = x; has_fix_ = true; }
    void hold_assoc(const AssocArgs &a) { assoc_ = a; has_assoc_ = true; }
    AssocArgs *take_assoc(FixArgs *&fix)
    {
        assert(has_assoc_ || !has_fix_);
        fix = std::exchange(has_fix_, false) ? &fix_ : nullptr;
        return std::exchange(has_assoc_, false) ? &assoc_ : nullptr;
    }
    void hold_settle(const ShardSettle &ss) { settle_ = ss; has_settle_ = true; }
    ShardSettle *take_settle() { return std::exchange(has_settle_, false) ? &settle_ : nullptr; }
    void hold_stats(uint32_t *nf) { nf_ = nf; }
    uint32_t *take_stats() { return std::exchange(nf_, nullptr); }
private:
    bool has_fix_ = false, has_assoc_ = false, has_settle_ = false;
    FixArgs fix_{};
    AssocArgs assoc_{};
    ShardSettle settle_{};
    uint32_t *nf_ = nullptr;
};

struct FrameSet {
    float *depthT = nullptr;
    uint32_t *rgbsT = nullptr;
    uint2 *dcT = nullptr;
    uint8_t *tile_flags = nullptr;
    uint4 *wave_cnt = nullptr;
    uint2 *prep_part = nullptr;
    uint32_t *nf_sub = nullptr;
    uint32_t *conf_sub = nullptr;
};

struct PassPartials {
    Dev<uint2> d_compact;
    Dev<uint4> d_lazy;
    Dev<uint2> d_fix;
    int fix_set = 0;
    uint32_t n_compact = 0;
    uint32_t n_fix = 0;
    bool pass_live = false;
    void clear() { pass_live = false; }
    uint2 *fix_cur() const { return d_fix + (size_t)fix_set * MAX_GRID; }
    struct Fold { const uint2 *compact; uint32_t n_compact; const uint4 *lazy; const uint2 *fix; uint32_t n_fix; };
    Fold fold() const { return {d_compact, n_compact, pass_live ? d_lazy.get() : nullptr, pass_live ? fix_cur() : nullptr, n_fix}; }
};

struct Timeline {
    struct Flags { bool compacted, one_pass, direct, merged, deferred; };
    std::unique_ptr<Event[][EV_RING]> ev;
    Flags flags[EV_RING] = {};
    uint64_t frames = 0, read = 0;
    int mark(hipStream_t st, int which, bool timed)
    {
        if (timed && ev) HIPCK(hipEventRecord(ev[which][frames % EV_RING], st));
        return SM_OK;
    }
    Flags &frame() { return flags[frames % EV_RING]; }
    void end_frame(bool timed) { if (timed && ev) frames++; }
};

}

using namespace sm_impl;

struct sm_ctx {
    Stream stream;
    Stream stream_in;
    sm_config cfg{};
    int W = 0, H = 0, P = 0;
    uint32_t cap = 0;
    int plane_set = 0;
    FrameSet fset[2];
    const FrameSet &cur() const { return fset[plane_set]; }
    const FrameSet &prev() const { return fset[plane_set ^ 1]; }
    void alias_frame_sets() { uint32_t *c = fset[1].conf_sub; fset[1] = fset[0]; fset[1].conf_sub = c; }
    Dev<uint64_t> d_key[2];
    int key_set = 0;
    uint64_t *keyT() const { return d_key[key_set]; }
    std::vector<Dev<void>> frame_mem;
    Model M{};
    SetBufs m_bufs[2];
    Dev<DevState> d_state;
    Host<DevState> h_state;
    Dev<float> d_filteredT, d_lastT;
    Dev<uint8_t> d_rgb, d_sem;
    Dev<uint16_t> d_depth_raw;
    static constexpr int IN_RING = 3;
    struct InSlot { Dev<uint8_t> rgb; uint8_t *sem = nullptr; uint16_t *depth = nullptr;
                    Host<unsigned char> h_stage; Event ev_in, ev_free; bool used = false; };
    InSlot in[IN_RING];
    size_t in_off_depth = 0, in_off_sem = 0, in_bytes = 0;
    uint32_t in_next = 0;
    const uint16_t *in_last_depth = nullptr; const uint8_t *in_last_sem = nullptr;
    int in_depth_slot = -1, in_sem_slot = -1;
    std::vector<std::pair<Host<unsigned char>, size_t>> pinned;
    Dev<float> d_depth_f32;
    Dev<float> d_xs, d_ys;
    float h_wtab[169];
    Dev<uint64_t> d_cm, d_dm, d_zm;
    Dev<uint32_t> d_tile_cnt, d_tile_allow, d_tile_keep, d_tile_flag;
    Dev<uint32_t> d_group_tot, d_group_base;
    Dev<uint64_t> d_alive;
    Dev<uint32_t> d_tile_dead;
    size_t alive_words = 0, dead_tiles = 0;
    sm_slots::SlotSchedule slots;
    Host<unsigned long long> h_stat; unsigned long long *d_stat = nullptr;
    Dev<uint32_t> d_tb;
    Dev<uint32_t> d_conf_part;
    PassPartials part;
    Dev<float> d_undo;
    int fix_grid = 128;
    Dev<uint32_t> d_blk_cand, d_grp_cand;
    Dev<uint32_t> d_frame_sub;
    uint32_t n_grp = 0, cand_group = 16;
    Dev<unsigned long long> d_pass_trace;
    int pass_trace_grid = 0;
    Dev<unsigned long long> d_ap_trace;
    int ap_trace_n[4] = {0, 0, 0, 0};
    Dev<uint32_t> d_conf_sub;
    uint32_t n_conf_part = 0;
    uint32_t tb_tiles = 0;
    int compact_grid = COMPACT_GRID;
    int pass_grid = MAX_GRID;
    Dev<uint64_t> d_validmask, d_fusedmask;
    Dev<uint2> d_blk_cnt;
    bool ss_on = false;
    bool rig_on = false;
    float rig_last_time = -1.0e30f;
    int ss_rank = 0, ss_world = 1;
    uint32_t ss_frames = 0;
    sm_collective_fn ss_coll = nullptr;
// ... 119 lines not shown
```

surfelmapping_amd/csrc/sm_device.h:

```cpp
#pragma once

#include <hip/hip_runtime.h>
#include <stdint.h>

namespace sm {

constexpr uint64_t KEY_EMPTY = 0x7FFFFFFFFFFFFFFFull;
constexpr int TILE = 1024;
constexpr int TILE_WORDS = TILE / 64;
constexpr int PIX_BLOCK = 256;
constexpr int SUB_STRIDE = 32;
constexpr int SUB_SET = 64 * SUB_STRIDE;

struct SurfelSet {
    float4 *pos_conf;
    float4 *norm_rad;
    uint32_t *color;
    float *init_time;
    float *time;
};

struct Model {
    SurfelSet s[2];
};

struct DevState {
    uint32_t count;
    uint32_t offset;
    uint32_t cur;
    uint32_t cull_n;
    uint32_t cull_src, cull_dst;
    uint32_t n_kill;
    uint32_t conflict_count;
    uint32_t data_count, unstable_count, fused_count;
    uint32_t visible_count;
    uint32_t append_n;
    int32_t error;
    uint32_t frames_logged;
    uint32_t n_static;
    uint32_t n_conf_skipped;
    uint32_t n_splat_skipped;
    uint32_t garbage;
    uint32_t garbage_prev;
    uint32_t do_compact;
    uint32_t cap_binds;
    uint32_t first_moving;
    uint32_t compact_ticket;
    uint32_t stat_frames;
    uint32_t first_live;
    uint32_t fl_dirty2[2];
    uint32_t slow_frames;
    uint32_t slow_done[2];
    uint32_t pend;
    uint32_t pend_tick;
    uint32_t holes_last;
};

struct FrameLog { uint32_t tick, n_before, n_after_cull, n_kill, conflict_count, visible_count, fused_count, unstable_count, n_static, n_conf_skipped, n_splat_skipped, n_slots; };
constexpr uint32_t FRAME_LOG_LEN = 1024;

struct FrameParams {
    float pose[16];
    float t_inv[16];
    float fx, fy, cx, cy;
    float inv_fx, inv_fy;
    float cols, rows;
    int W, H, P;
    float min_depth, max_depth;
    float conflict_thresh;
    float fuse_thresh;
    float stereo_border;
    int is_clean;
    int time;
    int time_delta;
    float depth_cutoff;
    uint32_t conflict_cap;
    int splat_follows;
    int log_frame;
    uint32_t max_vertices;
    int init_mode;
    float inv_fx_fb, inv_fy_fb;
    int use_bounds;
    uint32_t compact_now;
    int maintenance;
    int compact_tickets;
    int no_exempt;
    int shard_slots;
    int par;
};

__device__ __forceinline__ float min_glsl(float a, float b) { return (b < a) ? b : a; }

__device__ __forceinline__ int tex_idx(float t, int n)
{
    float f = floorf(t * (float)n);
    if (!(f >= 0.0f)) return 0;
    if (f > (float)(n - 1)) return n - 1;
    return (int)f;
}

__device__ __forceinline__ float3 xform3(const float *m, float x, float y, float z)
{
    float3 r;
    r.x = ((m[0] * x + m[4] * y) + m[8] * z) + m[12];
    r.y = ((m[1] * x + m[5] * y) + m[9] * z) + m[13];
    r.z = ((m[2] * x + m[6] * y) + m[10] * z) + m[14];
    return r;
}

__device__ __forceinline__ float3 rot3(const float *m, float x, float y, float z)
{
    float3 r;
    r.x = (m[0] * x + m[4] * y) + m[8] * z;
    r.y = (m[1] * x + m[5] * y) + m[9] * z;
    r.z = (m[2] * x + m[6] * y) + m[10] * z;
    return r;
}

__device__ __forceinline__ float dot3(float3 a, float3 b) { return (a.x * b.x + a.y * b.y) + a.z * b.z; }

__device__ __forceinline__ float3 cross3(float3 a, float3 b)
{
    float3 r;
    r.x = a.y * b.z - a.z * b.y;
    r.y = a.z * b.x - a.x * b.z;
    r.z = a.x * b.y - a.y * b.x;
    return r;
}

__device__ __forceinline__ float3 normalize3(float3 v)
{
    float l = sqrtf(dot3(v, v));
    float3 r;
    r.x = v.x / l; r.y = v.y / l; r.z = v.z / l;
    return r;
}

__device__ __forceinline__ float acos_spec(float x)
{
    const float pS0 = 1.6666586697e-01f, pS1 = -4.2743422091e-02f, pS2 = -8.6563630030e-03f;
    const float qS1 = -7.0662963390e-01f;
    const float PIO2 = 1.57079637050628662109375f, PI = 3.1415927410125732421875f;
    float ax = fabsf(x);
    if (ax <= 0.5f) {
        float z = x * x;
        float r = (z * (pS0 + z * (pS1 + z * pS2))) / (1.0f + z * qS1);
        return PIO2 - (x + x * r);
    } else if (x > 0.0f) {
        float z = (1.0f - x) * 0.5f;
        float s = sqrtf(z);
        float r = (z * (pS0 + z * (pS1 + z * pS2))) / (1.0f + z * qS1);
        return 2.0f * (s + s * r);
    } else {
        float z = (1.0f + x) * 0.5f;
        float s = sqrtf(z);
        float r = (z * (pS0 + z * (pS1 + z * pS2))) / (1.0f + z * qS1);
        return PI - 2.0f * (s + s * r);
    }
}

__device__ __forceinline__ uint32_t round_u8(float v)
{
    float r = roundf(v);
    if (!(r >= 0.0f)) return 0u;
    if (r > 4294967040.0f) return 4294967040u;
    return (uint32_t)r;
}
// ... 288 lines not shown
```

surfelmapping_amd/csrc/sm_k_cull.h:

```cpp
#pragma once

#ifndef SM_CONFLICT_WAVES
#define SM_CONFLICT_WAVES 5
#endif
__global__ __launch_bounds__(256) __attribute__((amdgpu_waves_per_eu(SM_CONFLICT_WAVES, 8))) void k_conflict(Model M, const DevState *__restrict__ st, FrameParams fp,
                                                  const uint2 *__restrict__ dcT ,
                                                  uint64_t *__restrict__ cm, uint64_t *__restrict__ dm,
                                                  uint64_t *__restrict__ zm, uint32_t *__restrict__ tile_cnt,
                                                  const uint32_t *__restrict__ tb, uint8_t *__restrict__ tile_flags,
                                                  uint32_t *__restrict__ blk_part ,
                                                  const uint64_t *__restrict__ alive,
                                                  uint32_t *__restrict__ conf_sub )
{
    __shared__ uint32_t s_red[4][3];
    __shared__ uint64_t s_m[3][TILE_WORDS];
    __shared__ uint8_t s_flags[64];
    const uint32_t N = st->count;
    const bool has_dead = st->garbage != 0u;
    const uint32_t exempt = fp.no_exempt ? 0xFFFFFFFFu : st->first_live;
    const float4 *__restrict__ pc = M.s[st->cur].pos_conf;
    const uint32_t ntiles = (N + TILE - 1) / TILE;
    const int lane = threadIdx.x & 63, wave = threadIdx.x >> 6;
    uint32_t skipped = 0;
    uint32_t acc = 0;
// ... 26 lines not shown
        for (int r = 0; r < 4; ++r) {
            const uint32_t k = (tile * TILE_WORDS + r * 4 + wave) * 64u + lane;
            valid[r] = k < N;
            v[r] = pc[min(k, N - 1u)];
        }
        if (has_dead) {
#pragma unroll
            for (int r = 0; r < 4; ++r) valid[r] = valid[r] && ((alive[tile * TILE_WORDS + r * 4 + wave] >> lane) & 1ull);
        }
        float zc[4], lam[4], dep[4];
        uint32_t cls[4], qq[4];
        bool inview[4];
#pragma unroll
        for (int r = 0; r < 4; ++r) {
            inview[r] = false; zc[r] = 0.f; lam[r] = 0.f; qq[r] = 0u;
            if (valid[r]) {
                const float3 ph = xform3(fp.t_inv, v[r].x, v[r].y, v[r].z);
                if (!(ph.z <= fp.min_depth || ph.z >= fp.max_depth)) {
                    const float xl = ph.x / ph.z;
                    const float yl = ph.y / ph.z;
                    const float u = fp.fx * xl + fp.cx;
                    const float vv = fp.fy * yl + fp.cy;
                    if (!(u < fp.stereo_border || u > fp.cols || vv < 0.0f || vv > fp.rows)) {
                        const int ti = tex_idx(u / fp.cols, fp.W), tj = tex_idx(vv / fp.rows, fp.H);
                        qq[r] = (uint32_t)(ti * fp.H + tj);
                        lam[r] = sqrtf((xl * xl + yl * yl) + 1.0f);
                        zc[r] = ph.z;
                        inview[r] = true;
                    }
                }
            }
        }
#pragma unroll
        for (int r = 0; r < 4; ++r) {
            const uint2 g = dcT[qq[r]];
            dep[r] = __uint_as_float(g.x);
            cls[r] = g.y >> 24;
        }
#pragma unroll
        for (int r = 0; r < 4; ++r) {
            const uint32_t word = tile * TILE_WORDS + r * 4 + wave;
            const uint32_t k = word * 64u + lane;
            bool conflict = false;
            if (inview[r]) {
                float depth = dep[r];
                if (cls[r] == 10u) depth = fp.max_depth + 1.0f;
                if (fp.is_clean == 0 && depth == 0.0f) depth = fp.max_depth + 20.0f;
                conflict = (depth * lam[r] - zc[r] * lam[r] > fp.conflict_thresh * zc[r]) && (k != exempt);
            }
            const bool dies = valid[r] && !(v[r].w - 1.0f > 0.0f);
            const bool dead = valid[r] && !(v[r].w > 0.0f);
            const uint64_t cw = __ballot(conflict), dw = __ballot(dies), zw = __ballot(dead);
            if (lane == 0) { s_m[0][r * 4 + wave] = cw; s_m[1][r * 4 + wave] = dw; s_m[2][r * 4 + wave] = zw; }
            nconf += __popcll(cw);
            nkill += __popcll(zw | (cw & dw));
            nzero += __popcll(zw);
        }
        if (lane == 0) { s_red[wave][0] = nconf; s_red[wave][1] = nkill; s_red[wave][2] = nzero; }
        __syncthreads();
        if (threadIdx.x < 3) {
            const uint32_t tsum = s_red[0][threadIdx.x] + s_red[1][threadIdx.x] + s_red[2][threadIdx.x] + s_red[3][threadIdx.x];
            tile_cnt[tile * 3 + threadIdx.x] = tsum;
            acc += tsum;
        }
        if (threadIdx.x >= 64 && threadIdx.x < 64 + 3 * TILE_WORDS) {
            const int m = (threadIdx.x - 64) / TILE_WORDS, w = (threadIdx.x - 64) % TILE_WORDS;
            const uint32_t word = tile * TILE_WORDS + w;
            if ((uint64_t)word * 64u < N) {
                uint64_t *dst = m == 0 ? cm : (m == 1 ? dm : zm);
                dst[word] = s_m[m][w];
            }
        }
        __syncthreads();
    }
    if (threadIdx.x < 2) blk_part[blockIdx.x * 4 + 1 + threadIdx.x] = acc;
    if (threadIdx.x == 0) {
        blk_part[blockIdx.x * 4] = skipped;
        if (acc) atomicAdd(&conf_sub[(blockIdx.x & 63u) * SUB_STRIDE], acc);
    }
}

constexpr int GROUP = 1024;

__global__ __launch_bounds__(1024) void k_scan_cull(const DevState *__restrict__ st,
                                                    const uint32_t *__restrict__ tile_cnt,
                                                    uint32_t *__restrict__ tile_allow,
                                                    uint32_t *__restrict__ tile_keep_prefix,
                                                    uint32_t *__restrict__ group_tot ,
                                                    const uint32_t *__restrict__ tile_dead)
{
    __shared__ uint32_t s_scan[17];
    __shared__ uint32_t s_first;
    const uint32_t N = st->count;
    const uint32_t ntiles = (N + TILE - 1) / TILE;
    const uint32_t t = blockIdx.x * GROUP + threadIdx.x;
    if (threadIdx.x == 0) s_first = 0xFFFFFFFFu;
    uint32_t nconf = 0, keep = 0;
    bool kills = false;
    if (t < ntiles) {
        nconf = tile_cnt[t * 3];
        const uint32_t nkill = tile_cnt[t * 3 + 1];
        keep = min((uint32_t)TILE, N - t * TILE) - tile_dead[t] - nkill;
        kills = nkill != 0 || tile_dead[t] != 0;
        tile_allow[t] = nconf;
    }
    uint32_t ctot, ktot;
    block_scan_1024(nconf, &ctot, s_scan);
    const uint32_t kpre = block_scan_1024(keep, &ktot, s_scan);
    if (kills) atomicMin(&s_first, t);
    if (t < ntiles) tile_keep_prefix[t] = kpre;
    __syncthreads();
    if (threadIdx.x == 0) {
        group_tot[blockIdx.x * 4 + 0] = ctot;
        group_tot[blockIdx.x * 4 + 1] = ktot;
        group_tot[blockIdx.x * 4 + 2] = s_first;
    }
}

__device__ __forceinline__ uint64_t keep_word(uint32_t t, int w, uint32_t N, const uint64_t *__restrict__ cm,
                                              const uint64_t *__restrict__ dm, const uint64_t *__restrict__ zm,
                                              const uint64_t *__restrict__ alive, uint32_t allow, uint32_t nconf)
{
    const uint32_t word = t * TILE_WORDS + (uint32_t)w;
    const uint64_t base = (uint64_t)word * 64u;
    if (base >= N) return 0ull;
    const uint64_t rem = (uint64_t)N - base;
    const uint64_t valid = (rem >= 64 ? ~0ull : ((1ull << rem) - 1ull)) & alive[word];
    uint64_t ce = cm[word];
    if (allow != nconf) {
        uint32_t before = 0;
        for (int x = 0; x < w; ++x) before += (uint32_t)__popcll(cm[t * TILE_WORDS + x]);
        ce = before >= allow ? 0ull : first_n_bits(ce, allow - before);
    }
    return ~(zm[word] | (ce & dm[word])) & valid;
}

__global__ __launch_bounds__(1024) void k_cull_finalize(DevState *__restrict__ st, FrameParams fp,
                                                        const uint64_t *__restrict__ cm,
                                                        const uint64_t *__restrict__ dm,
                                                        const uint64_t *__restrict__ zm,
                                                        const uint32_t *__restrict__ tile_cnt,
                                                        uint32_t *__restrict__ tile_allow,
                                                        uint32_t *__restrict__ tile_keep_prefix,
                                                        const uint32_t *__restrict__ group_tot,
                                                        uint32_t *__restrict__ group_keep_base,
                                                        const uint32_t *__restrict__ conf_part, uint32_t n_conf_part,
                                                        const uint64_t *__restrict__ alive,
                                                        const uint32_t *__restrict__ tile_dead,
                                                        unsigned long long *__restrict__ host_stat)
{
    __shared__ uint32_t s_scan[17];
    __shared__ uint32_t s_first, s_ft, s_fl, s_keep_first;
    const uint32_t N = st->count;
    const uint32_t g0 = st->garbage;
    const uint32_t old_first = st->first_live, old_offset = st->offset;
    const uint32_t holes = st->holes_last;
    const uint32_t ntiles = (N + TILE - 1) / TILE;
    const uint32_t ngroups = (ntiles + GROUP - 1) / GROUP;
    const uint32_t cap = fp.conflict_cap;
    const bool have_scan = fp.compact_now != 0u || fp.maintenance != 0;
    if (threadIdx.x == 0) { s_first = 0xFFFFFFFFu; s_ft = 0xFFFFFFFFu; s_fl = 0xFFFFFFFFu; }
    if (threadIdx.x == 1023) {
        uint32_t survive = 0;
        if (old_first < N) {
            const uint32_t w = old_first / 64u, bit = old_first % 64u;
            survive = (((zm[w] | (cm[w] & dm[w])) >> bit) & 1ull) ? 0u : 1u;
        }
        s_keep_first = survive;
    }
    uint32_t cskip = 0, cconf = 0, ckill = 0, cskip_tot, cconf_tot, ckill_tot;
    for (uint32_t b = threadIdx.x; b < n_conf_part; b += 1024u) {
        cskip += conf_part[b * 4]; cconf += conf_part[b * 4 + 1]; ckill += conf_part[b * 4 + 2];
    }
    __syncthreads();
    block_scan_1024(cskip, &cskip_tot, s_scan);
    block_scan_1024(cconf, &cconf_tot, s_scan);
    block_scan_1024(ckill, &ckill_tot, s_scan);
    uint32_t ctotal = cconf_tot, ktotal = (N - g0) - ckill_tot, gkpre = 0;
    uint32_t nstatic = N;
    if (have_scan) {
        uint32_t gc = 0, gk = 0;
        if (threadIdx.x < ngroups) {
            gc = group_tot[threadIdx.x * 4 + 0];
            gk = group_tot[threadIdx.x * 4 + 1];
            atomicMin(&s_first, group_tot[threadIdx.x * 4 + 2]);
        }
        block_scan_1024(gc, &ctotal, s_scan);
        gkpre = block_scan_1024(gk, &ktotal, s_scan);
        nstatic = (s_first == 0xFFFFFFFFu) ? N : min(N, s_first * (uint32_t)TILE);
    }
    const bool cap_binds = ctotal > cap;
    if (!cap_binds) {
        if (have_scan && threadIdx.x < ngroups) group_keep_base[threadIdx.x] = gkpre;
    } else {
        if (threadIdx.x < ngroups) group_keep_base[threadIdx.x] = 0;
        const uint32_t per = (ntiles + 1023u) / 1024u;
        const uint32_t t0 = min(threadIdx.x * per, ntiles), t1 = min(t0 + per, ntiles);
        uint32_t csum = 0;
        for (uint32_t t = t0; t < t1; ++t) csum += tile_cnt[t * 3];
        uint32_t dummy;
        uint32_t cpre = block_scan_1024(csum, &dummy, s_scan);
        uint32_t ksum = 0;
        for (uint32_t t = t0; t < t1; ++t) {
            const uint32_t nconf = tile_cnt[t * 3];
            uint32_t allow = nconf;
            if (cpre >= cap) allow = 0;
            else if (cap - cpre < nconf) allow = cap - cpre;
            tile_allow[t] = allow;
            uint32_t kills;
            if (allow == nconf) kills = tile_cnt[t * 3 + 1];
            else if (allow == 0) kills = tile_cnt[t * 3 + 2];
            else {
                kills = 0;
                uint32_t rem = allow;
                for (int w = 0; w < TILE_WORDS; ++w) {
                    const uint32_t word = t * TILE_WORDS + w;
                    if ((uint64_t)word * 64u >= N) break;
                    const uint64_t c = cm[word];
                    const uint64_t ce = first_n_bits(c, rem);
                    rem -= (uint32_t)__popcll(ce);
                    kills += (uint32_t)__popcll(zm[word] | (ce & dm[word]));
                }
            }
            tile_keep_prefix[t] = kills;
            ksum += min((uint32_t)TILE, N - t * TILE) - tile_dead[t] - kills;
            cpre += nconf;
        }
        uint32_t kpre = block_scan_1024(ksum, &ktotal, s_scan);
        uint32_t ns = 0;
        for (uint32_t t = t0; t < t1; ++t) {
            const uint32_t kills = tile_keep_prefix[t];
            const uint32_t nv = min((uint32_t)TILE, N - t * TILE) - tile_dead[t];
            if (kpre == t * TILE && kills == 0 && tile_dead[t] == 0u) ns += nv;
            else atomicMin(&s_first, t);
            tile_keep_prefix[t] = kpre;
            kpre += nv - kills;
        }
        block_scan_1024(ns, &nstatic, s_scan);
        __syncthreads();
    }
    const uint32_t kept = ktotal;
    const uint32_t g1 = N - kept;
    const bool compact = have_scan;
    uint32_t first_live = compact ? 0u : N;
    if (!compact && kept != 0u) {
        __syncthreads();
        if (s_keep_first) {
            first_live = old_first;
        } else {
            for (uint32_t base = min(old_first, N - 1u) / TILE; base < ntiles; base += 1024u) {
                const uint32_t t = base + threadIdx.x;
                if (t < ntiles) {
                    uint32_t keep_t;
                    if (cap_binds) keep_t = ((t + 1 < ntiles) ? tile_keep_prefix[t + 1] : kept) - tile_keep_prefix[t];
                    else keep_t = min((uint32_t)TILE, N - t * TILE) - tile_dead[t] - tile_cnt[t * 3 + 1];
                    if (keep_t != 0u) atomicMin(&s_ft, t);
                }
                __syncthreads();
                const uint32_t found = s_ft;
                __syncthreads();
                if (found != 0xFFFFFFFFu) break;
            }
            const uint32_t ft = s_ft;
            if (ft != 0xFFFFFFFFu && threadIdx.x < TILE_WORDS) {
                const uint32_t nconf = tile_cnt[ft * 3];
                const uint64_t k = keep_word(ft, (int)threadIdx.x, N, cm, dm, zm, alive, cap_binds ? tile_allow[ft] : nconf, nconf);
                if (k) atomicMin(&s_fl, (ft * TILE_WORDS + threadIdx.x) * 64u + (uint32_t)(__ffsll((long long)k) - 1));
            }
            __syncthreads();
            first_live = s_fl;
        }
    }
    if (threadIdx.x == 0) {
        if (!fp.maintenance) {
            st->n_conf_skipped = cskip_tot;
            st->n_static = compact ? nstatic : N;
            st->n_kill = (N - g0) - kept;
            st->conflict_count = min(ctotal, cap);
            if (fp.splat_follows) st->visible_count = 0;
        }
        st->cull_n = N;
        st->cull_src = st->cur;
        st->cull_dst = st->cur;
        st->garbage_prev = g0;
        st->cap_binds = cap_binds ? 1u : 0u;
        st->do_compact = compact ? 1u : 0u;
        st->first_moving = (compact && s_first != 0xFFFFFFFFu) ? min(s_first, ntiles) : ntiles;
        st->compact_ticket = 0u;
        st->first_live = first_live;
        st->fl_dirty2[0] = 0u; st->fl_dirty2[1] = 0u;
        st->slow_done[0] = 0u; st->slow_done[1] = 0u;
        st->holes_last = 0u;
        if (compact) {
            st->count = kept;
            st->offset = fp.maintenance ? old_offset - (g0 - holes) : kept;
            st->garbage = 0;
        } else {
            st->count = N;
            st->offset = N;
            st->garbage = g1;
        }
        if (host_stat)
            __hip_atomic_store(host_stat, ((unsigned long long)st->stat_frames << 32) | (unsigned long long)(compact ? kept : N),
                               __ATOMIC_RELAXED, __HIP_MEMORY_SCOPE_SYSTEM);
    }
}

__device__ __forceinline__ void post_compact_fill(const DevState *__restrict__ st, uint64_t *__restrict__ alive,
                                                  uint32_t *__restrict__ tile_dead, uint32_t tid, uint32_t nthreads)
{
    if (st->do_compact == 0u || st->garbage_prev == 0u) return;
    const uint32_t n = st->cull_n;
    const uint32_t nwords = (n + 63u) / 64u, ntiles = (n + TILE - 1) / TILE;
    for (uint32_t w = tid; w < nwords; w += nthreads) alive[w] = ~0ull;
    for (uint32_t t = tid; t < ntiles; t += nthreads) tile_dead[t] = 0u;
}

__global__ void k_post_fill(const DevState *__restrict__ st, uint64_t *__restrict__ alive, uint32_t *__restrict__ tile_dead)
{
    post_compact_fill(st, alive, tile_dead, blockIdx.x * blockDim.x + threadIdx.x, gridDim.x * blockDim.x);
}

__global__ void k_remap_keys(const DevState *__restrict__ st, uint64_t *__restrict__ keyT, int P,
                             const uint64_t *__restrict__ alive, const uint32_t *__restrict__ tile_keep_prefix,
                             const uint32_t *__restrict__ group_keep_base)
{
    const int q = blockIdx.x * blockDim.x + threadIdx.x;
    if (q >= P || st->garbage_prev == 0u) return;
    const uint64_t key = keyT[q];
    if (key == KEY_EMPTY) return;
    const uint32_t id = (uint32_t)(key & 0xFFFFFFFFull);
    if (id >= st->cull_n) return;
    const uint32_t tile = id / TILE, w = (id % TILE) / 64u, bit = id % 64u;
    uint32_t nid = tile_keep_prefix[tile] + group_keep_base[tile / GROUP];
    for (uint32_t x = 0; x < w; ++x) nid += (uint32_t)__popcll(alive[tile * TILE_WORDS + x]);
    nid += (uint32_t)__popcll(alive[tile * TILE_WORDS + w] & ((1ull << bit) - 1ull));
    keyT[q] = (key & 0xFFFFFFFF00000000ull) | (uint64_t)nid;
}

__device__ __forceinline__ bool splat_one(const FrameParams &fp, float x, float y, float z, float t_last,
                                          uint32_t id, uint64_t *__restrict__ keyT)
{
    const float3 ph = xform3(fp.t_inv, x, y, z);
    if (ph.z >= fp.depth_cutoff * 1.5f || ph.z <= 0.0f || (float)fp.time - t_last > (float)fp.time_delta)
        return false;
    const float xn = ((((fp.fx * ph.x) / ph.z) + fp.cx) - (fp.cols * 0.5f)) / (fp.cols * 0.5f);
    const float yn = ((((fp.fy * ph.y) / ph.z) + fp.cy) - (fp.rows * 0.5f)) / (fp.rows * 0.5f);
    const float zn = ph.z / fp.depth_cutoff;
    if (!(xn >= -1.0f && xn <= 1.0f && yn >= -1.0f && yn <= 1.0f && zn >= -1.0f && zn <= 1.0f)) return false;
    const float xw = (fp.cols * 0.5f) * xn + (fp.cols * 0.5f);
    const float yw = (fp.rows * 0.5f) * yn + (fp.rows * 0.5f);
    const float fxw = floorf(xw), fyw = floorf(yw);
    if (!(fxw >= 0.0f && fxw < fp.cols && fyw >= 0.0f && fyw < fp.rows)) return false;
    const int px = (int)fxw, py = (int)fyw;
    const float zw = 0.5f * zn + 0.5f;
    const uint32_t d24 = (uint32_t)floor((double)zw * 16777215.0 + 0.5);
    if (d24 >= 16777215u) return false;
    const uint64_t key = ((uint64_t)d24 << 32) | (uint64_t)id;
    atomicMin((unsigned long long *)&keyT[(size_t)px * fp.H + py], (unsigned long long)key);
    return true;
}

template <bool SPLAT>
__global__ __launch_bounds__(256) void k_compact(Model M, DevState *__restrict__ st, FrameParams fp,
                                                 const uint64_t *__restrict__ cm,
                                                 const uint64_t *__restrict__ dm,
                                                 const uint64_t *__restrict__ zm,
                                                 const uint32_t *__restrict__ tile_cnt,
                                                 const uint32_t *__restrict__ tile_allow,
                                                 const uint32_t *__restrict__ tile_keep_prefix,
                                                 uint64_t *__restrict__ keyT,
                                                 uint32_t *__restrict__ tile_flag, uint32_t epoch,
                                                 const uint32_t *__restrict__ group_keep_base,
                                                 uint32_t *__restrict__ tb, const uint8_t *__restrict__ tile_flags,
                                                 uint2 *__restrict__ blk_part ,
                                                 uint64_t *__restrict__ alive, uint32_t *__restrict__ tile_dead)
{
    __shared__ uint64_t s_keep[TILE_WORDS], s_ceff[TILE_WORDS];
    __shared__ uint32_t s_cpop[TILE_WORDS], s_kpre[TILE_WORDS + 1];
    __shared__ uint32_t s_vis[4];
    const uint32_t N = st->cull_n;
    const SurfelSet set = M.s[st->cull_src];
    const uint32_t ntiles = (N + TILE - 1) / TILE;
    const int lane = threadIdx.x & 63, wave = threadIdx.x >> 6;
    uint32_t vis = 0, skipped = 0, iter = 0;
    uint64_t skipmask = 0;
    uint32_t m_nconf = 0, m_nkill = 0, m_allow = 0, m_base = 0, m_dead = 0;
    const bool had_dead = st->garbage_prev != 0u;
    const bool cap_binds = st->cap_binds != 0u;
    const bool use_tickets = fp.compact_tickets != 0;
    const uint32_t fm = use_tickets ? min(st->first_moving, ntiles) : ntiles;
    constexpr uint32_t TICKET = 1;
    __shared__ uint32_t s_tk;
    bool ticketing = false;
    uint32_t rr_tile = blockIdx.x, tk_tile = 0, tk_left = 0;
    for (;;) {
        uint32_t tile, allow, nconf, nkill_full, base_id, tdead;
        bool skipbit;
        if (!ticketing && rr_tile >= fm) {
            if (!use_tickets) break;
            ticketing = true;
        }
        if (!ticketing) {
            tile = rr_tile;
            if ((iter & 63u) == 0u) {
                const uint64_t tl = (uint64_t)tile + (uint64_t)lane * gridDim.x;
                const bool in = tl < fm;
                const uint32_t tt = in ? (uint32_t)tl : 0u;
                skipmask = __ballot(in && (tile_flags[tt] & 2u));
                m_nconf = tile_cnt[tt * 3]; m_nkill = tile_cnt[tt * 3 + 1];
                m_allow = cap_binds ? tile_allow[tt] : m_nconf;
                m_base = tile_keep_prefix[tt] + group_keep_base[tt / GROUP];
                m_dead = had_dead ? tile_dead[tt] : 0u;
            }
            const int sl = (int)(iter & 63u);
            allow = lane_bcast(m_allow, sl); nconf = lane_bcast(m_nconf, sl);
            nkill_full = lane_bcast(m_nkill, sl); base_id = lane_bcast(m_base, sl);
            tdead = lane_bcast(m_dead, sl);
            skipbit = (skipmask >> (iter & 63u)) & 1ull;
            rr_tile += gridDim.x; ++iter;
        } else {
            if (tk_left == 0u) {
                __syncthreads();
                if (threadIdx.x == 0) s_tk = atomicAdd(&st->compact_ticket, TICKET);
                __syncthreads();
                tk_tile = fm + s_tk; tk_left = TICKET;
            }
            tile = tk_tile;
            if (tile >= ntiles) break;
            ++tk_tile; --tk_left;
            nconf = tile_cnt[tile * 3]; nkill_full = tile_cnt[tile * 3 + 1];
            allow = cap_binds ? tile_allow[tile] : nconf;
            base_id = tile_keep_prefix[tile] + group_keep_base[tile / GROUP];
            tdead = had_dead ? tile_dead[tile] : 0u;
            skipbit = false;
        }
        if (!ticketing && nconf == 0 && nkill_full == 0 && base_id == tile * (uint32_t)TILE && tdead == 0u) {
            if (SPLAT && skipbit) {
                skipped += min((uint32_t)TILE, N - tile * TILE);
                continue;
            }
            if (SPLAT) {
                float4 pv[4];
                float pt[4];
#pragma unroll
                for (int r = 0; r < 4; ++r) {
                    const uint32_t k = (tile * TILE_WORDS + r * 4 + wave) * 64u + lane;
                    const uint32_t kc = min(k, N - 1u);
                    pv[r] = set.pos_conf[kc];
                    pt[r] = set.time[kc];
                }
#pragma unroll
                for (int r = 0; r < 4; ++r) {
                    const uint32_t k = (tile * TILE_WORDS + r * 4 + wave) * 64u + lane;
                    bool drew = false;
                    if (k < N)
                        drew = splat_one(fp, pv[r].x, pv[r].y, pv[r].z, pt[r], k, keyT);
                    vis += (uint32_t)__popcll(__ballot(drew));
                }
            }
            continue;
        }
        const bool moving = ticketing || (base_id != tile * (uint32_t)TILE) || nkill_full != 0u || tdead != 0u;
        float4 v[4], nr[4];
        uint32_t col[4], nid[4];
        float it[4], tl[4];
        bool kept[4];
#pragma unroll
        for (int r = 0; r < 4; ++r) {
            const uint32_t k = (tile * TILE_WORDS + r * 4 + wave) * 64u + lane;
            const uint32_t kc = min(k, N - 1u);
            v[r] = set.pos_conf[kc];
            tl[r] = set.time[kc];
            nr[r] = make_float4(0.f, 0.f, 0.f, 0.f); col[r] = 0; it[r] = 0.f;
            if (moving) { nr[r] = set.norm_rad[kc]; col[r] = set.color[kc]; it[r] = set.init_time[kc]; }
        }
        uint64_t c = 0, d = 0, z = 0, valid = 0;
        if (threadIdx.x < TILE_WORDS) {
            const uint32_t word = tile * TILE_WORDS + threadIdx.x;
            const uint64_t base = (uint64_t)word * 64u;
            if (base < N) {
                c = cm[word]; d = dm[word]; z = zm[word];
                const uint64_t rem = (uint64_t)N - base;
                valid = rem >= 64 ? ~0ull : ((1ull << rem) - 1ull);
                if (had_dead) valid &= alive[word];
            }
            s_cpop[threadIdx.x] = (uint32_t)__popcll(c);
        }
        __syncthreads();
        if (threadIdx.x < TILE_WORDS) {
            uint64_t ce = c;
            if (allow != nconf) {
                uint32_t before = 0;
                for (int w = 0; w < (int)threadIdx.x; ++w) before += s_cpop[w];
                ce = before >= allow ? 0ull : first_n_bits(c, allow - before);
            }
            const uint64_t keep = ~(z | (ce & d)) & valid;
            s_ceff[threadIdx.x] = ce;
            s_keep[threadIdx.x] = keep;
        }
        __syncthreads();
        if (threadIdx.x <= TILE_WORDS) {
            uint32_t before = 0;
            for (int w = 0; w < (int)threadIdx.x; ++w) before += (uint32_t)__popcll(s_keep[w]);
            s_kpre[threadIdx.x] = before;
        }
        __syncthreads();
        const uint32_t kcount = s_kpre[TILE_WORDS];
#pragma unroll
        for (int r = 0; r < 4; ++r) {
            const int w = r * 4 + wave;
            const uint64_t keepw = s_keep[w];
            kept[r] = (keepw >> lane) & 1ull;
            nid[r] = base_id + s_kpre[w] + (uint32_t)__popcll(keepw & ((1ull << lane) - 1ull));
            if (kept[r] && ((s_ceff[w] >> lane) & 1ull)) {
                v[r].w -= 1.0f;
                if (!moving) set.pos_conf[(tile * TILE_WORDS + w) * 64u + lane].w = v[r].w;
            }
        }
        if (moving) {
            if (threadIdx.x < 8) atomicExch(&tb[(size_t)tile * 8 + threadIdx.x], 0u);
            asm volatile("s_waitcnt vmcnt(0)" ::: "memory");
            __syncthreads();
            if (threadIdx.x == 0) {
                __hip_atomic_exchange(&tile_flag[tile], epoch, __ATOMIC_RELAXED, __HIP_MEMORY_SCOPE_AGENT);
                if (kcount && base_id != tile * TILE) {
                    const uint32_t first = base_id / TILE;
                    const uint32_t last = min(tile - 1u, (base_id + kcount - 1u) / TILE);
                    for (uint32_t t = first; t <= last; ++t) {
                        uint32_t spins = 0;
                        while (__hip_atomic_load(&tile_flag[t], __ATOMIC_RELAXED, __HIP_MEMORY_SCOPE_AGENT) != epoch) {
                            __builtin_amdgcn_s_sleep(2);
                            if (++spins > (1u << 24)) { st->error = -6; break; }
                        }
                    }
                }
            }
            __syncthreads();
#pragma unroll
            for (int r = 0; r < 4; ++r) {
                if (kept[r]) {
                    set.pos_conf[nid[r]] = v[r];
                    set.norm_rad[nid[r]] = nr[r];
                    set.color[nid[r]] = col[r];
                    set.init_time[nid[r]] = it[r];
                    set.time[nid[r]] = tl[r];
                }
                bounds_expand_wave(tb, kept[r], nid[r] / (uint32_t)TILE, v[r].x, v[r].y, v[r].z, tl[r], false);
            }
        }
        if (SPLAT) {
#pragma unroll
            for (int r = 0; r < 4; ++r) {
                bool drew = false;
                if (kept[r])
                    drew = splat_one(fp, v[r].x, v[r].y, v[r].z, tl[r], nid[r], keyT);
                vis += (uint32_t)__popcll(__ballot(drew));
            }
        }
        __syncthreads();
    }
    if (SPLAT) {
        if (lane == 0) s_vis[wave] = vis;
        __syncthreads();
        if (threadIdx.x == 0)
            blk_part[blockIdx.x] = make_uint2(s_vis[0] + s_vis[1] + s_vis[2] + s_vis[3], skipped);
    }
}

__global__ __launch_bounds__(256) void k_cull_lazy(Model M, const DevState *__restrict__ st, FrameParams fp,
                                                   const uint64_t *__restrict__ cm, const uint64_t *__restrict__ dm,
                                                   const uint64_t *__restrict__ zm, const uint32_t *__restrict__ tile_cnt,
                                                   const uint32_t *__restrict__ tile_allow,
                                                   uint64_t *__restrict__ alive, uint32_t *__restrict__ tile_dead)
{
    const uint32_t N = st->cull_n;
    const SurfelSet set = M.s[st->cull_src];
    const uint32_t ntiles = (N + TILE - 1) / TILE;
    const int lane = threadIdx.x & 63, wave = threadIdx.x >> 6;
    const bool had_dead = st->garbage_prev != 0u, cap_binds = st->cap_binds != 0u;
    uint32_t iter = 0;
    uint32_t m_nconf = 0, m_nkill = 0, m_dead = 0;
    for (uint32_t tile = blockIdx.x; tile < ntiles; tile += gridDim.x, ++iter) {
        if ((iter & 63u) == 0u) {
            const uint64_t tl = (uint64_t)tile + (uint64_t)lane * gridDim.x;
            const bool in = tl < ntiles;
            const uint32_t tt = in ? (uint32_t)tl : 0u;
            m_nconf = tile_cnt[tt * 3]; m_nkill = tile_cnt[tt * 3 + 1];
            m_dead = had_dead ? tile_dead[tt] : 0u;
        }
        const int sl = (int)(iter & 63u);
        const uint32_t nconf = lane_bcast(m_nconf, sl), nkill = lane_bcast(m_nkill, sl);
        const uint32_t tdead = lane_bcast(m_dead, sl);
        const bool touched = nconf != 0u || nkill != 0u;
        if (!touched) continue;
        float4 pv[4];
#pragma unroll
        for (int r = 0; r < 4; ++r) {
            const uint32_t kc = min((tile * TILE_WORDS + r * 4 + wave) * 64u + lane, N - 1u);
            pv[r] = set.pos_conf[kc];
        }
        const uint32_t allow = (touched && cap_binds) ? tile_allow[tile] : nconf;
        uint32_t killed = 0;
#pragma unroll
        for (int r = 0; r < 4; ++r) {
            const int w = r * 4 + wave;
            const uint32_t word = tile * TILE_WORDS + (uint32_t)w;
            const uint32_t k = word * 64u + lane;
            const uint64_t base = (uint64_t)word * 64u;
            uint64_t range = 0ull;
            if (base < N) { const uint64_t rem = (uint64_t)N - base; range = rem >= 64 ? ~0ull : ((1ull << rem) - 1ull); }
            const uint64_t valid = range & ((tdead != 0u) ? alive[word] : ~0ull);
            uint64_t keep = valid, ce = 0ull;
            if (touched) {
                ce = cm[word];
                if (allow != nconf) {
                    uint32_t before = 0;
                    for (int x = 0; x < w; ++x) before += (uint32_t)__popcll(cm[tile * TILE_WORDS + x]);
                    ce = before >= allow ? 0ull : first_n_bits(ce, allow - before);
                }
                keep = ~(zm[word] | (ce & dm[word])) & valid;
// ... 50 lines not shown
```

surfelmapping_amd/csrc/sm_k_pass.h:

```cpp
#pragma once

__device__ __forceinline__ bool candidate_pixel(int q, const FrameParams &fp, const float *__restrict__ depthT,
                                                const float *__restrict__ xs, const float *__restrict__ ys)
{
    const int H = fp.H, W = fp.W;
    const int i = q / H, j = q - i * H;
    const float z = depthT[q];
    const float zl = depthT[i > 0 ? q - H : q];
    const float zu = depthT[j > 0 ? q - 1 : q];
    const float zr = depthT[i < W - 1 ? q + H : q];
    const float zd = depthT[j < H - 1 ? q + 1 : q];
    const int par = ((int)xs[i] + (int)ys[j]) % 2;
    return (zl != 0.0f) & (zu != 0.0f) & (zr != 0.0f) & (zd != 0.0f) & (z > fp.min_depth) & (z < fp.max_depth) & (par == 1);
}


template <int CAND_GROUP>
__device__ __forceinline__ void cand_count_block(uint32_t cg, const FrameParams &fp, const float *__restrict__ depthT,
                                                 const float *__restrict__ xs, const float *__restrict__ ys, int nblocks,
                                                 uint32_t *__restrict__ blk_cand, uint32_t *__restrict__ grp_cand)
{
    __shared__ uint32_t s_w[CAND_GROUP][4];
    const int lane = threadIdx.x & 63, wave = threadIdx.x >> 6;
    bool c[CAND_GROUP];
// ... 498 lines not shown

__device__ __forceinline__ void finalize_write(DevState *__restrict__ st, FrameLog *__restrict__ log, const PendFields &pf, uint32_t U,
                                               uint32_t F, uint32_t vadd, uint32_t res);

__device__ __forceinline__ void finalize_frame(DevState *__restrict__ st, uint32_t *__restrict__ nf ,
                                               const uint2 *__restrict__ fix_prev, uint32_t n_fix_prev, FrameLog *__restrict__ log,
                                               uint32_t *s_red )
{
    if (st->pend == 0u) return;
    const int lane = threadIdx.x & 63, wave = threadIdx.x >> 6;
    uint32_t un = 0, fu = 0, va = 0, rs = 0;
    if (wave == 0) {
        uint32_t *a = nf + lane * SUB_STRIDE, *b = nf + SUB_SET + lane * SUB_STRIDE;
        un = *a; fu = *b; *a = 0u; *b = 0u;
    }
    if (st->cap_binds)
        for (uint32_t b = threadIdx.x; b < n_fix_prev; b += 256u) { const uint2 c = fix_prev[b]; va += c.x; rs += c.y; }
    un = wave_sum_u32(un); fu = wave_sum_u32(fu); va = wave_sum_u32(va); rs = wave_sum_u32(rs);
    __syncthreads();
    if (lane == 0) { s_red[wave] = un; s_red[4 + wave] = fu; s_red[8 + wave] = va; s_red[12 + wave] = rs; }
    __syncthreads();
    if (threadIdx.x == 0) {
        const uint32_t U = s_red[0] + s_red[1] + s_red[2] + s_red[3], F = s_red[4] + s_red[5] + s_red[6] + s_red[7];
        const uint32_t vadd = s_red[8] + s_red[9] + s_red[10] + s_red[11], res = s_red[12] + s_red[13] + s_red[14] + s_red[15];
        PendFields pf;
        pf.cull_n = st->cull_n; pf.garbage_prev = st->garbage_prev; pf.n_kill = st->n_kill; pf.visible = st->visible_count;
        pf.conflict = st->conflict_count; pf.n_static = st->n_static; pf.conf_skipped = st->n_conf_skipped;
        pf.splat_skipped = st->n_splat_skipped; pf.tick = st->pend_tick; pf.frames_logged = st->frames_logged;
        finalize_write(st, log, pf, U, F, vadd, res);
    }
    __syncthreads();
}

__device__ __forceinline__ void finalize_write(DevState *__restrict__ st, FrameLog *__restrict__ log, const PendFields &pf, uint32_t U,
                                               uint32_t F, uint32_t vadd, uint32_t res)
{
    const uint32_t n_slots = pf.cull_n, g_prev = pf.garbage_prev;
    const uint32_t n_kill = pf.n_kill - res, vis = pf.visible + vadd;
    const uint32_t g_cull = g_prev + n_kill;
    st->n_kill = n_kill;
    st->visible_count = vis;
    st->garbage = g_cull + F;
    st->holes_last = F;
    st->unstable_count = U;
    st->fused_count = F;
    st->data_count = U + F;
    st->append_n = U;
    if (log) {
        FrameLog e;
        e.tick = pf.tick; e.n_before = n_slots - g_prev; e.n_after_cull = n_slots - g_cull; e.n_kill = n_kill;
        e.conflict_count = pf.conflict; e.visible_count = vis; e.fused_count = F; e.unstable_count = U;
        e.n_static = pf.n_static; e.n_conf_skipped = pf.conf_skipped; e.n_splat_skipped = pf.splat_skipped; e.n_slots = n_slots;
        log[pf.frames_logged % FRAME_LOG_LEN] = e;
        st->frames_logged = pf.frames_logged + 1;
    }
    st->n_conf_skipped = 0;
    st->pend = 0u;
}

__global__ __launch_bounds__(256) void k_frame_finalize(DevState *__restrict__ st, uint32_t *__restrict__ nf,
                                                        const uint2 *__restrict__ fix_prev, uint32_t n_fix_prev, FrameLog *__restrict__ log)
{
    __shared__ uint32_t s_red[16];
    finalize_frame(st, nf, fix_prev, n_fix_prev, log, s_red);
}

template <bool MERGED>
__device__ __forceinline__ void fixup_publisher(DevState *__restrict__ st, const FrameParams &fp, const FixArgs &x, uint32_t ctotal)
{
    __shared__ uint32_t s_c[4];
    __shared__ uint32_t s_fl;
    __shared__ uint32_t s_red9[9][4];
    const DirectArgs &da = x.da;
    const uint64_t *__restrict__ cm = x.cm, *__restrict__ km = x.km;
    const uint4 *__restrict__ wave_cnt = x.wave_cnt;
    const uint64_t *__restrict__ alive = x.alive;
    const int lane = threadIdx.x & 63, wave = threadIdx.x >> 6;
    const uint32_t cap = fp.conflict_cap;
    const bool cap_binds = ctotal > cap;
    const uint32_t N = MERGED ? st->offset : st->count;
    const uint32_t ntiles = (N + TILE - 1) / TILE;
    const uint32_t pend = st->pend, cap_prev = st->cap_binds, g_in = st->garbage, old_first = st->first_live;
    const bool dirty = st->fl_dirty2[fp.par] != 0u;
    PendFields pf;
    pf.cull_n = st->cull_n; pf.garbage_prev = st->garbage_prev; pf.n_kill = st->n_kill; pf.visible = st->visible_count;
    pf.conflict = st->conflict_count; pf.n_static = st->n_static; pf.conf_skipped = st->n_conf_skipped;
    pf.splat_skipped = st->n_splat_skipped; pf.tick = st->pend_tick; pf.frames_logged = st->frames_logged;
    uint32_t red[9] = {0u, 0u, 0u, 0u, 0u, 0u, 0u, 0u, 0u};
    if (wave == 0) {
        uint32_t *c = da.frame_sub + lane * SUB_STRIDE, *n = da.nf_prev + lane * SUB_STRIDE;
        red[6] = c[0]; red[7] = c[SUB_SET]; red[0] = n[0]; red[1] = n[SUB_SET];
        c[0] = 0u; c[SUB_SET] = 0u; n[0] = 0u; n[SUB_SET] = 0u;
    }
    for (uint32_t b = threadIdx.x; b < da.n_fix_prev; b += 256u) { const uint2 c = da.fix_prev[b]; red[2] += c.x; red[3] += c.y; }
    if (x.n_prep) for (uint32_t b = threadIdx.x; b < x.n_prep; b += 256u) { const uint2 c = x.prep_part[b]; red[4] += c.x; red[5] += c.y; }
    else for (uint32_t b = threadIdx.x; b < x.n_part; b += 256u) { const uint4 c = x.part[b]; red[4] += c.w; red[5] += c.y; }
#pragma unroll
    for (int i = 0; i < 9; ++i) red[i] = wave_sum_u32(red[i]);
    if (lane == 0) {
#pragma unroll
        for (int i = 0; i < 9; ++i) s_red9[i][wave] = red[i];
    }
    if (threadIdx.x == 0) s_fl = 0xFFFFFFFFu;
    __syncthreads();
    uint32_t tot[9];
#pragma unroll
    for (int i = 0; i < 9; ++i) tot[i] = s_red9[i][0] + s_red9[i][1] + s_red9[i][2] + s_red9[i][3];
    if (!cap_prev || !pend) { tot[2] = 0u; tot[3] = 0u; }
    uint32_t g0 = g_in;
    if (pend) {
        g0 = pf.garbage_prev + (pf.n_kill - tot[3]) + tot[1];
        if (threadIdx.x == 0) finalize_write(st, da.log, pf, tot[0], tot[1], tot[2], tot[3]);
    }
    const uint32_t cskip_tot = tot[4], sskip_tot = tot[5], vis_tot = tot[6], kill_tot = tot[7];
    uint32_t first_live = old_first;
    if (dirty) {
        first_live = N;
        const uint32_t t0 = min(old_first, N ? N - 1u : 0u) / TILE;
        uint32_t before = 0;
        if (cap_binds) {
            uint32_t p = 0;
            for (uint32_t t = threadIdx.x; t < t0; t += 256u) { const uint4 c = wave_cnt[t]; p += c.x + c.y + c.z + c.w; }
            p = wave_sum_u32(p);
            if (lane == 0) s_c[wave] = p;
            __syncthreads();
            before = s_c[0] + s_c[1] + s_c[2] + s_c[3];
            __syncthreads();
        }
        for (uint32_t t = t0; t < ntiles && N; ++t) {
            const uint4 c4 = wave_cnt[t];
            if (threadIdx.x < TILE_WORDS) {
                const uint32_t word = t * TILE_WORDS + threadIdx.x;
                const uint64_t base = (uint64_t)word * 64u;
                if (base < N) {
                    const uint64_t rem = (uint64_t)N - base;
                    const uint64_t range = rem >= 64 ? ~0ull : ((1ull << rem) - 1ull);
                    uint64_t live = alive[word] & range;
                    if (cap_binds && (c4.x | c4.y | c4.z | c4.w)) {
                        uint32_t pre = before;
                        for (uint32_t w = t * TILE_WORDS; w < word; ++w) pre += (uint32_t)__popcll(cm[w]);
                        live |= km[word] & ineffective_conflicts(cm[word], pre, cap) & range;
                    }
                    if (word == old_first / 64u) live &= ~((2ull << (old_first % 64u)) - 1ull);
                    if (live) atomicMin(&s_fl, word * 64u + (uint32_t)(__ffsll((long long)live) - 1));
                }
            }
            __syncthreads();
            const uint32_t found = s_fl;
            __syncthreads();
            if (found != 0xFFFFFFFFu) { first_live = found; break; }
            before += c4.x + c4.y + c4.z + c4.w;
        }
    }
    if (threadIdx.x == 0) {
        st->n_conf_skipped = cskip_tot;
        st->n_splat_skipped = sskip_tot;
        st->n_static = N;
        st->conflict_count = min(ctotal, cap);
        if (fp.splat_follows) st->visible_count = 0;
        st->cull_n = N;
        st->cull_src = st->cur;
        st->cull_dst = st->cur;
        st->garbage_prev = g0;
        st->cap_binds = cap_binds ? 1u : 0u;
        st->do_compact = 0u;
        if (!MERGED || dirty) st->first_live = first_live;
        if (!MERGED) {
            st->fl_dirty2[fp.par] = 0u;
            st->offset = N;
        }
        st->holes_last = 0u;
        if (da.on) {
            st->visible_count = vis_tot;
            st->n_kill = kill_tot;
            st->pend = 1u;
            st->pend_tick = (uint32_t)fp.time;
        }
        if (!MERGED && x.host_stat)
            __hip_atomic_store(x.host_stat, ((unsigned long long)st->stat_frames << 32) | (unsigned long long)N, __ATOMIC_RELAXED,
                               __HIP_MEMORY_SCOPE_SYSTEM);
        if (MERGED && (cap_binds || dirty)) {
            st->slow_frames = st->slow_frames + 1u;
            __hip_atomic_fetch_add(&st->slow_done[fp.par], 1u, __ATOMIC_RELEASE, __HIP_MEMORY_SCOPE_AGENT);
        }
    }
}

__device__ __forceinline__ void fixup_repair(const Model &M, DevState *__restrict__ st, const FrameParams &fp, const FixArgs &x,
                                             uint32_t wi, uint32_t nwg, uint32_t N)
{
    __shared__ uint32_t s_a[4], s_b[4], s_c[4];
    const uint64_t *__restrict__ cm = x.cm, *__restrict__ km = x.km;
    const uint4 *__restrict__ wave_cnt = x.wave_cnt;
    uint64_t *__restrict__ alive = x.alive; uint32_t *__restrict__ tile_dead = x.tile_dead;
    uint64_t *__restrict__ keyT = x.keyT; const float *__restrict__ undo = x.undo; uint32_t *__restrict__ tb = x.tb;
    const int lane = threadIdx.x & 63, wave = threadIdx.x >> 6;
    const uint32_t cap = fp.conflict_cap;
    const uint32_t ntiles = (N + TILE - 1) / TILE;
    const SurfelSet set = M.s[st->cur];
    uint32_t cpre = 0;
    {
        uint32_t p = 0;
        for (uint32_t t = threadIdx.x; t < min(wi, ntiles); t += 256u) { const uint4 c = wave_cnt[t]; p += c.x + c.y + c.z + c.w; }
        p = wave_sum_u32(p);
        if (lane == 0) s_c[wave] = p;
        __syncthreads();
        cpre = s_c[0] + s_c[1] + s_c[2] + s_c[3];
        __syncthreads();
    }
    uint32_t vis = 0, resurrected = 0;
    for (uint32_t tile = wi; tile < ntiles; tile += nwg) {
        const uint4 c4 = wave_cnt[tile];
        const uint32_t nconf = c4.x + c4.y + c4.z + c4.w;
        const uint32_t tile_pre = cpre;
        {
            uint32_t p = 0;
            for (uint32_t t = tile + threadIdx.x; t < min(tile + nwg, ntiles); t += 256u) { const uint4 c = wave_cnt[t]; p += c.x + c.y + c.z + c.w; }
            p = wave_sum_u32(p);
            __syncthreads();
            if (lane == 0) s_c[wave] = p;
            __syncthreads();
            cpre += s_c[0] + s_c[1] + s_c[2] + s_c[3];
        }
        if (nconf == 0u || tile_pre + nconf <= cap) continue;
        const bool nosplat = (x.tile_flags[tile] & 2u) != 0u;
        uint32_t wpre = tile_pre + (wave > 0 ? c4.x : 0u) + (wave > 1 ? c4.y : 0u) + (wave > 2 ? c4.z : 0u);
        uint32_t res_wave = 0, vis_tile = vis;
#pragma unroll
        for (int r = 0; r < 4; ++r) {
            const uint32_t word = tile * TILE_WORDS + (uint32_t)wave * 4u + (uint32_t)r;
            if ((uint64_t)word * 64u >= N) break;
            const uint64_t c = cm[word];
            const uint64_t ineff = ineffective_conflicts(c, wpre, cap);
            wpre += (uint32_t)__popcll(c);
            if (ineff == 0ull) continue;
            const uint64_t res = ineff & km[word];
            const uint64_t restore = ineff & ~res & alive[word];
            const uint32_t k = word * 64u + lane;
            if ((restore >> lane) & 1ull) set.pos_conf[k].w = undo[k];
            if (res) {
// ... 80 lines not shown
```

surfelmapping_amd/csrc/sm_slots.h:

```cpp
#pragma once

#include <algorithm>
#include <chrono>
#include <cstdint>
#include <thread>

namespace sm_slots {

struct SlotStat { uint32_t fr, slots; bool ahead_known; uint32_t ahead; };

class SlotSchedule {
public:
    SlotSchedule() = default;
    SlotSchedule(uint32_t tile, uint32_t cap, uint32_t max_new, int compact_period, long capacity_wait_us, unsigned long long *stat)
        : tile_(tile), cap_(cap), max_new_(max_new), period_(compact_period), wait_us_(capacity_wait_us), stat_(stat) {}

    SlotStat read_stat() const
    {
        const unsigned long long v = __atomic_load_n(stat_, __ATOMIC_RELAXED);
        const uint32_t fr = (uint32_t)(v >> 32);
        return {fr, (uint32_t)v, frames_enq_ >= fr, frames_enq_ >= fr ? frames_enq_ - fr : 0u};
    }
    uint32_t bound() const { return bound_; }
    uint64_t tiles_of(uint64_t slots) const { return (slots + tile_ - 1) / tile_; }
    uint64_t tiles() const { return tiles_of(bound_); }
    bool maybe_garbage() const { return garbage_; }
    bool keys_are_slots() const { return keys_slots_; }
    int culls_since_compact() const { return culls_; }
    uint32_t next_cull_epoch() { return ++cull_epoch_; }

    bool period_due() const { return period_ <= 1 || culls_ + 1 >= period_; }
    bool bound_may_overflow() const { return (uint64_t)bound_ + max_new_ > cap_; }
    bool decide_compact() const
    {
        if (period_ <= 1) return true;
        const auto t_start = std::chrono::steady_clock::now();
        for (uint32_t spins = 0;; ++spins) {
            const SlotStat st = read_stat();
            uint64_t bound = bound_;
            if (st.ahead_known) bound = std::min<uint64_t>(bound, (uint64_t)st.slots + (uint64_t)st.ahead * max_new_);
            if (bound + max_new_ <= cap_) break;
            if (st.ahead <= 1u) return true;
            if ((uint64_t)st.slots + 2ull * max_new_ > cap_) return true;
            if ((spins & 63u) == 63u &&
                std::chrono::duration_cast<std::chrono::microseconds>(std::chrono::steady_clock::now() - t_start).count() > wait_us_)
                return true;
            std::this_thread::yield();
        }
        return period_due();
    }

    uint64_t estimate_slots()
    {
        uint64_t est = bound_;
        const SlotStat st = read_stat();
        if (st.fr < est_fr0_ || st.slots < est_slots0_) { est_fr0_ = st.fr; est_slots0_ = st.slots; }
        else if (st.fr >= est_fr0_ + 8u) {
            est_rate_ = std::min<uint32_t>((st.slots - est_slots0_) / (st.fr - est_fr0_) + 1u, max_new_);
            est_fr0_ = st.fr; est_slots0_ = st.slots;
        }
        const uint32_t ahead = std::min<uint32_t>(st.ahead, (uint32_t)std::max(period_, 1));
        if (st.ahead_known) est = std::min<uint64_t>(est, (uint64_t)st.slots + (uint64_t)ahead * est_rate_);
        return est;
    }

    void cull_noted(bool compacted)
    {
        if (compacted) { culls_ = 0; }
        else { culls_++; garbage_ = true; }
    }
    void append_enqueued()
    {
        frames_enq_++;
        bound_ = (uint32_t)std::min<uint64_t>((uint64_t)bound_ + max_new_, cap_);
    }
    void state_pulled(uint32_t count, uint32_t cull_n, bool pending_cull) { bound_ = std::max(count, cull_n * (pending_cull ? 1u : 0u)); }
    void state_pushed(uint32_t stat_frames, uint32_t count)
    {
        __atomic_store_n(stat_, ((unsigned long long)stat_frames << 32) | (unsigned long long)count, __ATOMIC_RELAXED);
        frames_enq_ = stat_frames;
    }
    void dead_slots_made() { garbage_ = true; }
    void keys_drawn(bool as_slots) { keys_slots_ = as_slots; }
    void compacted_outside_frame() { garbage_ = false; culls_ = 0; keys_slots_ = false; }
    void compacted_sharded() { culls_ = 0; keys_slots_ = false; }
    void published_dense() { culls_ = 0; }
    void model_discarded() { garbage_ = false; }

private:
    uint32_t tile_ = 1, cap_ = 0, max_new_ = 0;
    int period_ = 1;
    long wait_us_ = 0;
    unsigned long long *stat_ = nullptr;
    uint32_t bound_ = 0;
    uint32_t frames_enq_ = 0;
    int culls_ = 0;
    bool garbage_ = false, keys_slots_ = false;
    uint32_t cull_epoch_ = 0;
    uint32_t est_fr0_ = 0, est_slots0_ = 0, est_rate_ = 0xFFFFFFFFu;
};

}
```

Baseline: 25890 frames/s.

## Replace periodic full compaction with a tail squeeze that skips mostly-live tiles

Frames that were due for periodic compaction now run a separate squeeze before a one-pass surfel step. The squeeze skips conflict masks and compacts only from the first tile whose dead count reaches a threshold, leaving garbage in the dense prefix instead of rewriting the whole model. It also resets the alive and dead bookkeeping per tile inside the compaction kernel and limits post-compaction refills to the moved range. This cuts the bandwidth spent on periodic full compactions, at the cost of carrying leftover garbage and a more complex state machine (n_static handling, tail counters).

```diff
diff --git a/include/sm_c_api.h b/include/sm_c_api.h
--- a/include/sm_c_api.h
+++ b/include/sm_c_api.h
@@ -344,6 +344,7 @@
 int sm_device_download(sm_ctx *s, void *dst_host, const void *src_device, size_t bytes);
 
 int sm_debug_slow_frames(sm_ctx *s, uint32_t *n);
+int sm_debug_squeezes(sm_ctx *s, uint32_t *tail, uint32_t *full);
 int sm_gpu_process_count(sm_ctx *s);
 
 enum { SM_COLL_SUM = 0, SM_COLL_MIN = 1, SM_COLL_GATHER = 2 };
diff --git a/surfelmapping_amd/capi.py b/surfelmapping_amd/capi.py
--- a/surfelmapping_amd/capi.py
+++ b/surfelmapping_amd/capi.py
@@ -15,7 +15,7 @@
 SYMBOLS = (
     "sm_api_version", "sm_last_error", "sm_default_config", "sm_create", "sm_destroy",
     "sm_process_frame", "sm_process_frame_device", "sm_process_frame_async",
-    "sm_inputs_consumed", "sm_host_alloc", "sm_host_alloc_frame", "sm_host_free", "sm_debug_slow_frames", "sm_sync", "sm_clean_points", "sm_clean_points_ex", "sm_clean_points_cb", "sm_reset",
+    "sm_inputs_consumed", "sm_host_alloc", "sm_host_alloc_frame", "sm_host_free", "sm_debug_slow_frames", "sm_debug_squeezes", "sm_sync", "sm_clean_points", "sm_clean_points_ex", "sm_clean_points_cb", "sm_reset",
     "sm_get_counts", "sm_download_model_aos", "sm_upload_model_aos", "sm_save_map", "sm_load_map",
     "sm_download_index_map", "sm_download_raw_cloud", "sm_download_depth", "sm_render_image", "sm_render_model",
     "sm_render_model_device", "sm_render_image_maps", "sm_render_model_maps", "sm_render_maps_stats", "sm_set_frame", "sm_set_tick",
@@ -411,6 +411,7 @@
     L.sm_host_free.argtypes = [vp, vp]
     L.sm_host_alloc_frame.argtypes = [vp, C.POINTER(vp), C.POINTER(vp), C.POINTER(vp)]
     L.sm_debug_slow_frames.argtypes = [vp, u32p]
+    L.sm_debug_squeezes.argtypes = [vp, u32p, u32p]
     L.sm_sync.argtypes = [vp]
     L.sm_clean_points.argtypes = [vp, vp, vp, vp]
     L.sm_clean_points_ex.argtypes = [vp, vp, vp, vp, C.c_int]
@@ -588,6 +589,11 @@
         self._chk(self._L.sm_debug_slow_frames(self._h, C.byref(n)), "sm_debug_slow_frames")
         return int(n.value)
 
+    def debug_squeezes(self):
+        t, f = C.c_uint32(), C.c_uint32()
+        self._chk(self._L.sm_debug_squeezes(self._h, C.byref(t), C.byref(f)), "sm_debug_squeezes")
+        return int(t.value), int(f.value)
+
     def inputs_consumed(self):
         self._chk(self._L.sm_inputs_consumed(self._h), "sm_inputs_consumed")
 
diff --git a/surfelmapping_amd/csrc/sm_api.hip b/surfelmapping_amd/csrc/sm_api.hip
--- a/surfelmapping_amd/csrc/sm_api.hip
+++ b/surfelmapping_amd/csrc/sm_api.hip
@@ -166,6 +166,8 @@
     auto num = [](const char *name, long unset) { const char *e = std::getenv(name); return e ? std::atol(e) : unset; };
     sw.defer_assoc = !off("SM_DEFER_ASSOC");
     sw.two_launch = !off("SM_TWO_LAUNCH");
+    sw.tail_squeeze = !off("SM_TAIL_SQUEEZE");
+    sw.tail_thresh = (uint32_t)std::max(1l, num("SM_TAIL_THRESH", (long)TAIL_DEAD_THRESH));
     sw.pass_split = (int)num("SM_PASS_SPLIT", 0);
     if (const char *e = std::getenv("SM_PASS_TRACE")) { sw.trace = true; sw.trace_prefix = e; }
     if (std::getenv("SM_COMPACT_TICKETS")) sw.compact_tickets = off("SM_COMPACT_TICKETS") ? 0 : 1;
@@ -334,7 +336,7 @@
     if (fp.compact_now) {
         const int ngroups = std::max<int>(1, (int)((s->slots.tiles() + GROUP - 1) / GROUP));
         hipLaunchKernelGGL(k_scan_cull, dim3(ngroups), dim3(1024), 0, s->stream, s->d_state, s->d_tile_cnt, s->d_tile_allow,
-                           s->d_tile_keep, s->d_group_tot, s->d_tile_dead);
+                           s->d_tile_keep, s->d_group_tot, s->d_tile_dead, 0u, 0u);
         HIPCK(hipGetLastError());
     }
     hipLaunchKernelGGL(k_cull_finalize, dim3(1), dim3(1024), 0, s->stream, s->d_state, fp, s->d_cm, s->d_dm, s->d_zm,
@@ -370,7 +372,7 @@
     return g;
 }
 
-int launch_surfel_pass(sm_ctx *s, const FrameParams &fp, bool timed, bool direct, uint32_t n_prep)
+int launch_surfel_pass(sm_ctx *s, const FrameParams &fp, bool timed, bool direct, uint32_t n_prep, bool squeezed = false)
 {
     if (n_prep == 0) { g_err = "internal: one-pass frame without tile flags from the preparation launch"; return SM_E_ARG; }
     const bool two = s->sw.two_launch && s->defer_ok && timed && direct;
@@ -399,7 +401,7 @@
                        f.wave_cnt, s->d_tb, f.tile_flags, pp.d_lazy, s->d_alive, s->d_tile_dead, sub, s->keyT(), s->d_undo, tile_bound,
                        s->d_frame_sub, ca, s->d_pass_trace);
     HIPCK(hipGetLastError());
-    if (s->tl.mark(s->stream, 2, timed) || s->tl.mark(s->stream, 3, timed)) return SM_E_HIP;
+    if (!squeezed && (s->tl.mark(s->stream, 2, timed) || s->tl.mark(s->stream, 3, timed))) return SM_E_HIP;
     FixArgs x{};
     DirectArgs &da = x.da;
     da.on = direct ? (two ? 2 : 1) : 0;
@@ -414,7 +416,7 @@
     x.host_stat = s->d_stat; x.prep_part = f.prep_part; x.n_prep = n_prep; x.tb = s->d_tb; x.n_crew = (uint32_t)g.fix_workers;
     if (two) s->held.hold_fixup(x);
     else if (launch_fixup(s, fp, x)) return SM_E_HIP;
-    if (s->tl.mark(s->stream, 4, timed)) return SM_E_HIP;
+    if (!squeezed && s->tl.mark(s->stream, 4, timed)) return SM_E_HIP;
     check_alive(s, 1u + 16u * (uint32_t)(s->tick & 0xFFFF));
     return SM_OK;
 }
@@ -503,6 +505,29 @@
     if (s->tl.mark(s->stream, 7, timed)) return SM_E_HIP;
     check_alive(s, 5u + 16u * (uint32_t)(s->tick & 0xFFFF));
     return SM_OK;
+}
+
+int launch_squeeze(sm_ctx *s, bool in_frame, bool tail, bool timed)
+{
+    FrameParams fp = make_params(s, s->curr_pose);
+    fp.maintenance = in_frame ? 2 : 1;
+    fp.compact_now = 1;
+    fp.conflict_cap = 0xFFFFFFFFu;
+    fp.no_masks = 1;
+    fp.tail_thresh = tail ? s->sw.tail_thresh : 0u;
+    const uint64_t tiles = s->slots.tiles() + 1;
+    const int ngroups = std::max<int>(1, (int)((tiles + GROUP - 1) / GROUP));
+    hipLaunchKernelGGL(k_scan_cull, dim3(ngroups), dim3(1024), 0, s->stream, s->d_state, s->d_tile_cnt, s->d_tile_allow,
+                       s->d_tile_keep, s->d_group_tot, s->d_tile_dead, 1u, fp.tail_thresh);
+    hipLaunchKernelGGL(k_cull_finalize, dim3(1), dim3(1024), 0, s->stream, s->d_state, fp, s->d_cm, s->d_dm, s->d_zm,
+                       s->d_tile_cnt, s->d_tile_allow, s->d_tile_keep, s->d_group_tot, s->d_group_base, s->d_conf_part, 0u,
+                       s->d_alive, s->d_tile_dead, s->d_stat);
+    if (!in_frame && s->slots.keys_are_slots())
+        hipLaunchKernelGGL(k_remap_keys, dim3((s->P + 255) / 256), dim3(256), 0, s->stream, s->d_state, s->keyT(), s->P, s->d_alive,
+                           s->d_tile_keep, s->d_group_base);
+    HIPCK(hipGetLastError());
+    if (s->tl.mark(s->stream, 2, timed) || s->tl.mark(s->stream, 3, timed)) return SM_E_HIP;
+    return launch_compact(s, fp, false, timed);
 }
 
 int discard_model(sm_ctx *s)
@@ -586,21 +611,29 @@
     if (s->ss_on) { g_err = "context is configured for sharding: use the sm_shard_* entry points"; return SM_E_ARG; }
     FrameParams fp;
     const bool fusing = s->ref_set && s->tick != 0 && !s->pending_cull;
-    const bool compact_now = fusing ? s->slots.decide_compact() : true;
+    using Due = sm_slots::SlotSchedule::Due;
+    const Due due = fusing ? s->slots.decide_due() : Due::forced;
+    const bool compact_now = due != Due::none;
+    const bool squeeze = fusing && due == Due::period && s->sw.tail_squeeze && s->defer_ok;
     const bool carry = fusing && s->defer_ok;
     int rc = SM_OK;
     uint32_t n_prep = 0;
     if (!carry && (rc = complete_held(s, false))) return rc;
-    rc = begin_frame(s, d_rgb, d_raw, d_sem, pose, fusing && !compact_now, carry, &fp, &n_prep);
+    rc = begin_frame(s, d_rgb, d_raw, d_sem, pose, fusing && (!compact_now || squeeze), carry, &fp, &n_prep);
     if (rc <= 0) return rc;
-    fp.compact_now = compact_now ? 1u : 0u;
-    s->slots.cull_noted(fp.compact_now != 0u);
+    fp.compact_now = compact_now && !squeeze ? 1u : 0u;
+    if (squeeze) {
+        if ((rc = complete_held(s, true))) return rc;
+        if ((rc = launch_squeeze(s, true, true, true))) return rc;
+        s->slots.squeezed_in_frame();
+    } else
+        s->slots.cull_noted(fp.compact_now != 0u);
     s->slots.keys_drawn(fp.compact_now == 0u);
     const bool one_pass = !fp.compact_now;
     Timeline::Flags &fl = s->tl.frame();
-    fl.compacted = !one_pass; fl.one_pass = fl.direct = one_pass;
+    fl.compacted = !one_pass || squeeze; fl.one_pass = fl.direct = one_pass; fl.squeezed = squeeze;
     if (one_pass) {
-        if ((rc = launch_surfel_pass(s, fp, true, true, n_prep))) return rc;
+        if ((rc = launch_surfel_pass(s, fp, true, true, n_prep, squeeze))) return rc;
         if ((rc = launch_associate_direct(s, fp, true))) return rc;
         end_frame(s);
         return SM_OK;
@@ -789,27 +822,7 @@
     }
     if (!s->slots.maybe_garbage()) return SM_OK;
     if (s->pending_cull) { g_err = "internal: deferred compaction with a pending per-pass cull"; return SM_E_ARG; }
-    FrameParams fp = make_params(s, s->curr_pose);
-    fp.maintenance = 1;
-    fp.compact_now = 1;
-    fp.conflict_cap = 0xFFFFFFFFu;
-    const uint64_t tiles = s->slots.tiles() + 1;
-    const size_t words = std::min<size_t>(tiles * TILE_WORDS, s->alive_words);
-    HIPCK(hipMemsetAsync(s->d_cm, 0, words * 8, s->stream));
-    HIPCK(hipMemsetAsync(s->d_dm, 0, words * 8, s->stream));
-    HIPCK(hipMemsetAsync(s->d_zm, 0, words * 8, s->stream));
-    HIPCK(hipMemsetAsync(s->d_tile_cnt, 0, std::min<size_t>(tiles, s->dead_tiles) * 12, s->stream));
-    const int ngroups = std::max<int>(1, (int)((tiles + GROUP - 1) / GROUP));
-    hipLaunchKernelGGL(k_scan_cull, dim3(ngroups), dim3(1024), 0, s->stream, s->d_state, s->d_tile_cnt, s->d_tile_allow,
-                       s->d_tile_keep, s->d_group_tot, s->d_tile_dead);
-    hipLaunchKernelGGL(k_cull_finalize, dim3(1), dim3(1024), 0, s->stream, s->d_state, fp, s->d_cm, s->d_dm, s->d_zm,
-                       s->d_tile_cnt, s->d_tile_allow, s->d_tile_keep, s->d_group_tot, s->d_group_base, s->d_conf_part, 0u,
-                       s->d_alive, s->d_tile_dead, s->d_stat);
-    if (s->slots.keys_are_slots())
-        hipLaunchKernelGGL(k_remap_keys, dim3((s->P + 255) / 256), dim3(256), 0, s->stream, s->d_state, s->keyT(), s->P, s->d_alive,
-                           s->d_tile_keep, s->d_group_base);
-    HIPCK(hipGetLastError());
-    int rc = launch_compact(s, fp, false, false);
+    int rc = launch_squeeze(s, false, false, false);
     if (rc) return rc;
     if ((rc = launch_post_fill(s))) return rc;
     s->slots.compacted_outside_frame();
@@ -1362,7 +1375,7 @@
     double own[6] = {0};
     double prep2[2] = {0, 0};
     double scan_own = 0;
-    uint32_t nfr = 0, ncls[2] = {0, 0}, n_op = 0, n_dir = 0, n_merged = 0, n_alone = 0;
+    uint32_t nfr = 0, ncls[2] = {0, 0}, n_op = 0, n_dir = 0, n_merged = 0, n_alone = 0, n_sq = 0;
     for (uint64_t f = first; f < tl.frames; ++f) {
         const int slot = (int)(f % EV_RING);
         const Timeline::Flags &fl = tl.flags[slot];
@@ -1380,7 +1393,8 @@
         for (int k = 0; k < 7; ++k) seg[k] += loc[k];
         cull[fl.compacted ? 1 : 0] += loc[3];
         ncls[fl.compacted ? 1 : 0]++;
-        if (fl.one_pass) { own[0] += loc[1]; own[1] += loc[3]; n_op++; } else { own[2] += loc[1]; scan_own += loc[2]; }
+        if (fl.squeezed) { own[0] += loc[4]; scan_own += loc[1]; n_op++; n_sq++; }
+        else if (fl.one_pass) { own[0] += loc[1]; own[1] += loc[3]; n_op++; } else { own[2] += loc[1]; scan_own += loc[2]; }
         if (fl.direct) { n_dir++; if (!fl.deferred) { own[3] += loc[4]; n_alone++; } } else { own[4] += loc[4]; own[5] += loc[6]; }
         prep2[fl.merged ? 1 : 0] += loc[0];
         if (fl.merged) n_merged++;
@@ -1402,8 +1416,8 @@
         out->k_compact_own = ncls[1] ? (float)std::max(0.0, cull[1] / ncls[1] - oh) : 0.0f;
         out->frames_compact = ncls[1];
         auto avg = [&](double sum, uint32_t n) { return n ? (float)std::max(0.0, sum / n - oh) : 0.0f; };
-        out->k_surfel_pass = avg(own[0], n_op); out->k_pass_fixup = avg(own[1], n_op); out->k_conflict_own = avg(own[2], nfr - n_op);
-        out->k_scan_own = avg(scan_own, nfr - n_op);
+        out->k_surfel_pass = avg(own[0], n_op); out->k_pass_fixup = avg(own[1], n_op - n_sq); out->k_conflict_own = avg(own[2], nfr - n_op);
+        out->k_scan_own = avg(scan_own, nfr - n_op + n_sq);
         out->k_associate_direct = avg(own[3], n_alone); out->k_associate_own = avg(own[4], nfr - n_dir); out->k_append_own = avg(own[5], nfr - n_dir);
         out->frames_one_pass = n_op; out->frames_direct = n_dir;
         out->k_assoc_prep = avg(prep2[1], n_merged); out->k_prep_own = avg(prep2[0], nfr - n_merged);
@@ -1445,6 +1459,16 @@
     int rc = pull_state(s);
     if (rc) return rc;
     *n = s->h_state->slow_frames;
+    return SM_OK;
+}
+
+int sm_debug_squeezes(sm_ctx *s, uint32_t *tail, uint32_t *full)
+{
+    if (!s || !tail || !full) return SM_E_ARG;
+    HIPCK(hipSetDevice(s->cfg.device));
+    int rc = pull_state(s);
+    if (rc) return rc;
+    *tail = s->h_state->sq_tail; *full = s->h_state->sq_full;
     return SM_OK;
 }
 
@@ -1575,7 +1599,7 @@
     s->slots.cull_noted(false);
     s->slots.keys_drawn(true);
     Timeline::Flags &fl = s->tl.frame();
-    fl.compacted = false; fl.one_pass = fl.direct = true;
+    fl.compacted = false; fl.one_pass = fl.direct = true; fl.squeezed = false;
     if ((rc = launch_surfel_pass(s, fp, true, true, n_prep))) return rc;
     if (s->cfg.conflict_cap && (uint64_t)s->slots.bound() > (uint64_t)s->P) {
         const uint32_t tbnd = (uint32_t)std::min<uint64_t>(s->slots.tiles(), s->dead_tiles);
diff --git a/surfelmapping_amd/csrc/sm_ctx.h b/surfelmapping_amd/csrc/sm_ctx.h
--- a/surfelmapping_amd/csrc/sm_ctx.h
+++ b/surfelmapping_amd/csrc/sm_ctx.h
@@ -194,6 +194,8 @@
 struct Switches {
     bool defer_assoc = true;
     bool two_launch = true;
+    bool tail_squeeze = true;
+    uint32_t tail_thresh = 0;
     int pass_split = 0;
     bool trace = false;
     std::string trace_prefix;
@@ -252,7 +254,7 @@
 };
 
 struct Timeline {
-    struct Flags { bool compacted, one_pass, direct, merged, deferred; };
+    struct Flags { bool compacted, one_pass, direct, merged, deferred, squeezed; };
     std::unique_ptr<Event[][EV_RING]> ev;
     Flags flags[EV_RING] = {};
     uint64_t frames = 0, read = 0;
diff --git a/surfelmapping_amd/csrc/sm_device.h b/surfelmapping_amd/csrc/sm_device.h
--- a/surfelmapping_amd/csrc/sm_device.h
+++ b/surfelmapping_amd/csrc/sm_device.h
@@ -54,6 +54,8 @@
     uint32_t pend;
     uint32_t pend_tick;
     uint32_t holes_last;
+    uint32_t sq_static;
+    uint32_t sq_tail, sq_full;
 };
 
 struct FrameLog { uint32_t tick, n_before, n_after_cull, n_kill, conflict_count, visible_count, fused_count, unstable_count, n_static, n_conf_skipped, n_splat_skipped, n_slots; };
@@ -83,6 +85,8 @@
     int use_bounds;
     uint32_t compact_now;
     int maintenance;
+    int no_masks;
+    uint32_t tail_thresh;
     int compact_tickets;
     int no_exempt;
     int shard_slots;
diff --git a/surfelmapping_amd/csrc/sm_k_cull.h b/surfelmapping_amd/csrc/sm_k_cull.h
--- a/surfelmapping_amd/csrc/sm_k_cull.h
+++ b/surfelmapping_amd/csrc/sm_k_cull.h
@@ -132,38 +132,47 @@
 
 constexpr int GROUP = 1024;
 
+constexpr uint32_t TAIL_DEAD_THRESH = TILE / 16;
+constexpr uint32_t TAIL_GARBAGE_DIV = 32;
+
 __global__ __launch_bounds__(1024) void k_scan_cull(const DevState *__restrict__ st,
                                                     const uint32_t *__restrict__ tile_cnt,
                                                     uint32_t *__restrict__ tile_allow,
                                                     uint32_t *__restrict__ tile_keep_prefix,
                                                     uint32_t *__restrict__ group_tot ,
-                                                    const uint32_t *__restrict__ tile_dead)
+                                                    const uint32_t *__restrict__ tile_dead,
+                                                    uint32_t no_masks ,
+                                                    uint32_t tail_thresh )
 {
     __shared__ uint32_t s_scan[17];
-    __shared__ uint32_t s_first;
+    __shared__ uint32_t s_first, s_dense;
     const uint32_t N = st->count;
     const uint32_t ntiles = (N + TILE - 1) / TILE;
     const uint32_t t = blockIdx.x * GROUP + threadIdx.x;
-    if (threadIdx.x == 0) s_first = 0xFFFFFFFFu;
+    if (threadIdx.x == 0) { s_first = 0xFFFFFFFFu; s_dense = 0xFFFFFFFFu; }
     uint32_t nconf = 0, keep = 0;
-    bool kills = false;
+    bool kills = false, dense = false;
     if (t < ntiles) {
-        nconf = tile_cnt[t * 3];
-        const uint32_t nkill = tile_cnt[t * 3 + 1];
-        keep = min((uint32_t)TILE, N - t * TILE) - tile_dead[t] - nkill;
-        kills = nkill != 0 || tile_dead[t] != 0;
-        tile_allow[t] = nconf;
+        uint32_t nkill = 0;
+        if (!no_masks) { nconf = tile_cnt[t * 3]; nkill = tile_cnt[t * 3 + 1]; }
+        const uint32_t dead = tile_dead[t];
+        keep = min((uint32_t)TILE, N - t * TILE) - dead - nkill;
+        kills = nkill != 0 || dead != 0;
+        dense = tail_thresh != 0u && dead >= tail_thresh;
+        if (!no_masks) tile_allow[t] = nconf;
     }
     uint32_t ctot, ktot;
     block_scan_1024(nconf, &ctot, s_scan);
     const uint32_t kpre = block_scan_1024(keep, &ktot, s_scan);
     if (kills) atomicMin(&s_first, t);
+    if (dense) atomicMin(&s_dense, t);
     if (t < ntiles) tile_keep_prefix[t] = kpre;
     __syncthreads();
     if (threadIdx.x == 0) {
         group_tot[blockIdx.x * 4 + 0] = ctot;
         group_tot[blockIdx.x * 4 + 1] = ktot;
         group_tot[blockIdx.x * 4 + 2] = s_first;
+        group_tot[blockIdx.x * 4 + 3] = s_dense;
     }
 }
 
@@ -200,7 +209,7 @@
                                                         unsigned long long *__restrict__ host_stat)
 {
     __shared__ uint32_t s_scan[17];
-    __shared__ uint32_t s_first, s_ft, s_fl, s_keep_first;
+    __shared__ uint32_t s_first, s_ft, s_fl, s_keep_first, s_dense, s_left;
     const uint32_t N = st->count;
     const uint32_t g0 = st->garbage;
     const uint32_t old_first = st->first_live, old_offset = st->offset;
@@ -209,10 +218,10 @@
     const uint32_t ngroups = (ntiles + GROUP - 1) / GROUP;
     const uint32_t cap = fp.conflict_cap;
     const bool have_scan = fp.compact_now != 0u || fp.maintenance != 0;
-    if (threadIdx.x == 0) { s_first = 0xFFFFFFFFu; s_ft = 0xFFFFFFFFu; s_fl = 0xFFFFFFFFu; }
+    if (threadIdx.x == 0) { s_first = 0xFFFFFFFFu; s_ft = 0xFFFFFFFFu; s_fl = 0xFFFFFFFFu; s_dense = 0xFFFFFFFFu; s_left = 0u; }
     if (threadIdx.x == 1023) {
-        uint32_t survive = 0;
-        if (old_first < N) {
+        uint32_t survive = fp.no_masks ? 1u : 0u;
+        if (old_first < N && !fp.no_masks) {
             const uint32_t w = old_first / 64u, bit = old_first % 64u;
             survive = (((zm[w] | (cm[w] & dm[w])) >> bit) & 1ull) ? 0u : 1u;
         }
@@ -228,20 +237,33 @@
     block_scan_1024(ckill, &ckill_tot, s_scan);
     uint32_t ctotal = cconf_tot, ktotal = (N - g0) - ckill_tot, gkpre = 0;
     uint32_t nstatic = N;
+    uint32_t bnd = ntiles, left = 0;
     if (have_scan) {
         uint32_t gc = 0, gk = 0;
         if (threadIdx.x < ngroups) {
             gc = group_tot[threadIdx.x * 4 + 0];
             gk = group_tot[threadIdx.x * 4 + 1];
             atomicMin(&s_first, group_tot[threadIdx.x * 4 + 2]);
+            if (fp.tail_thresh) atomicMin(&s_dense, group_tot[threadIdx.x * 4 + 3]);
         }
         block_scan_1024(gc, &ctotal, s_scan);
         gkpre = block_scan_1024(gk, &ktotal, s_scan);
         nstatic = (s_first == 0xFFFFFFFFu) ? N : min(N, s_first * (uint32_t)TILE);
-    }
+        bnd = (s_first == 0xFFFFFFFFu) ? ntiles : min(s_first, ntiles);
+        if (fp.tail_thresh) {
+            const uint32_t bt = min(s_dense, ntiles);
+            if (bt < ntiles) { if (threadIdx.x == bt / (uint32_t)GROUP) s_left = bt * (uint32_t)TILE - (gkpre + tile_keep_prefix[bt]); }
+            else if (threadIdx.x == 0) s_left = N - ktotal;
+            __syncthreads();
+            left = s_left;
+            if (left == 0u || left > N / TAIL_GARBAGE_DIV) left = 0u;
+            else { bnd = bt; nstatic = min(N, bt * (uint32_t)TILE); }
+        }
+    }
+    const bool tail = left != 0u;
     const bool cap_binds = ctotal > cap;
     if (!cap_binds) {
-        if (have_scan && threadIdx.x < ngroups) group_keep_base[threadIdx.x] = gkpre;
+        if (have_scan && threadIdx.x < ngroups) group_keep_base[threadIdx.x] = gkpre + ((tail && threadIdx.x >= bnd / (uint32_t)GROUP) ? left : 0u);
     } else {
         if (threadIdx.x < ngroups) group_keep_base[threadIdx.x] = 0;
         const uint32_t per = (ntiles + 1023u) / 1024u;
@@ -292,7 +314,7 @@
     const uint32_t kept = ktotal;
     const uint32_t g1 = N - kept;
     const bool compact = have_scan;
-    uint32_t first_live = compact ? 0u : N;
+    uint32_t first_live = compact ? (tail ? old_first : 0u) : N;
     if (!compact && kept != 0u) {
         __syncthreads();
         if (s_keep_first) {
@@ -335,23 +357,27 @@
         st->garbage_prev = g0;
         st->cap_binds = cap_binds ? 1u : 0u;
         st->do_compact = compact ? 1u : 0u;
-        st->first_moving = (compact && s_first != 0xFFFFFFFFu) ? min(s_first, ntiles) : ntiles;
+        st->first_moving = compact ? bnd : ntiles;
+        if (fp.maintenance == 2) {
+            st->sq_static = bnd < ntiles ? nstatic + 1u : 0u;
+            if (tail) st->sq_tail = st->sq_tail + 1u; else st->sq_full = st->sq_full + 1u;
+        }
         st->compact_ticket = 0u;
         st->first_live = first_live;
         st->fl_dirty2[0] = 0u; st->fl_dirty2[1] = 0u;
         st->slow_done[0] = 0u; st->slow_done[1] = 0u;
         st->holes_last = 0u;
         if (compact) {
-            st->count = kept;
-            st->offset = fp.maintenance ? old_offset - (g0 - holes) : kept;
-            st->garbage = 0;
+            st->count = kept + left;
+            st->offset = fp.maintenance ? old_offset - (g0 - holes) + left : kept;
+            st->garbage = left;
         } else {
             st->count = N;
             st->offset = N;
             st->garbage = g1;
         }
         if (host_stat)
-            __hip_atomic_store(host_stat, ((unsigned long long)st->stat_frames << 32) | (unsigned long long)(compact ? kept : N),
+            __hip_atomic_store(host_stat, ((unsigned long long)st->stat_frames << 32) | (unsigned long long)(compact ? kept + left : N),
                                __ATOMIC_RELAXED, __HIP_MEMORY_SCOPE_SYSTEM);
     }
 }
@@ -362,8 +388,9 @@
     if (st->do_compact == 0u || st->garbage_prev == 0u) return;
     const uint32_t n = st->cull_n;
     const uint32_t nwords = (n + 63u) / 64u, ntiles = (n + TILE - 1) / TILE;
-    for (uint32_t w = tid; w < nwords; w += nthreads) alive[w] = ~0ull;
-    for (uint32_t t = tid; t < ntiles; t += nthreads) tile_dead[t] = 0u;
+    const uint32_t t0 = min(st->first_moving, ntiles);
+    for (uint32_t w = t0 * TILE_WORDS + tid; w < nwords; w += nthreads) alive[w] = ~0ull;
+    for (uint32_t t = t0 + tid; t < ntiles; t += nthreads) tile_dead[t] = 0u;
 }
 
 __global__ void k_post_fill(const DevState *__restrict__ st, uint64_t *__restrict__ alive, uint32_t *__restrict__ tile_dead)
@@ -422,7 +449,7 @@
                                                  uint64_t *__restrict__ keyT,
                                                  uint32_t *__restrict__ tile_flag, uint32_t epoch,
                                                  const uint32_t *__restrict__ group_keep_base,
-                                                 uint32_t *__restrict__ tb, const uint8_t *__restrict__ tile_flags,
+                                                 uint32_t *__restrict__ tb, uint8_t *__restrict__ tile_flags,
                                                  uint2 *__restrict__ blk_part ,
                                                  uint64_t *__restrict__ alive, uint32_t *__restrict__ tile_dead)
 {
@@ -438,12 +465,14 @@
     uint32_t m_nconf = 0, m_nkill = 0, m_allow = 0, m_base = 0, m_dead = 0;
     const bool had_dead = st->garbage_prev != 0u;
     const bool cap_binds = st->cap_binds != 0u;
+    const bool nomask = fp.no_masks != 0, in_frame = fp.maintenance == 2;
+    const uint32_t lo = (nomask && !SPLAT) ? min(st->first_moving, ntiles) : 0u;
     const bool use_tickets = fp.compact_tickets != 0;
-    const uint32_t fm = use_tickets ? min(st->first_moving, ntiles) : ntiles;
+    const uint32_t fm = use_tickets ? max(lo, min(st->first_moving, ntiles)) : ntiles;
     constexpr uint32_t TICKET = 1;
     __shared__ uint32_t s_tk;
     bool ticketing = false;
-    uint32_t rr_tile = blockIdx.x, tk_tile = 0, tk_left = 0;
+    uint32_t rr_tile = lo + blockIdx.x, tk_tile = 0, tk_left = 0;
     for (;;) {
         uint32_t tile, allow, nconf, nkill_full, base_id, tdead;
         bool skipbit;
@@ -458,7 +487,7 @@
                 const bool in = tl < fm;
                 const uint32_t tt = in ? (uint32_t)tl : 0u;
                 skipmask = __ballot(in && (tile_flags[tt] & 2u));
-                m_nconf = tile_cnt[tt * 3]; m_nkill = tile_cnt[tt * 3 + 1];
+                if (!nomask) { m_nconf = tile_cnt[tt * 3]; m_nkill = tile_cnt[tt * 3 + 1]; }
                 m_allow = cap_binds ? tile_allow[tt] : m_nconf;
                 m_base = tile_keep_prefix[tt] + group_keep_base[tt / GROUP];
                 m_dead = had_dead ? tile_dead[tt] : 0u;
@@ -479,7 +508,7 @@
             tile = tk_tile;
             if (tile >= ntiles) break;
             ++tk_tile; --tk_left;
-            nconf = tile_cnt[tile * 3]; nkill_full = tile_cnt[tile * 3 + 1];
+            nconf = nomask ? 0u : tile_cnt[tile * 3]; nkill_full = nomask ? 0u : tile_cnt[tile * 3 + 1];
             allow = cap_binds ? tile_allow[tile] : nconf;
             base_id = tile_keep_prefix[tile] + group_keep_base[tile / GROUP];
             tdead = had_dead ? tile_dead[tile] : 0u;
@@ -530,7 +559,7 @@
             const uint32_t word = tile * TILE_WORDS + threadIdx.x;
             const uint64_t base = (uint64_t)word * 64u;
             if (base < N) {
-                c = cm[word]; d = dm[word]; z = zm[word];
+                if (!nomask) { c = cm[word]; d = dm[word]; z = zm[word]; }
                 const uint64_t rem = (uint64_t)N - base;
                 valid = rem >= 64 ? ~0ull : ((1ull << rem) - 1ull);
                 if (had_dead) valid &= alive[word];
@@ -587,6 +616,10 @@
                 }
             }
             __syncthreads();
+            if (in_frame) {
+                if (threadIdx.x < TILE_WORDS && (uint64_t)(tile * TILE_WORDS + threadIdx.x) * 64u < N) alive[tile * TILE_WORDS + threadIdx.x] = ~0ull;
+                if (threadIdx.x == 0) { tile_dead[tile] = 0u; tile_flags[tile] = 0; }
+            }
 #pragma unroll
             for (int r = 0; r < 4; ++r) {
                 if (kept[r]) {
diff --git a/surfelmapping_amd/csrc/sm_k_pass.h b/surfelmapping_amd/csrc/sm_k_pass.h
--- a/surfelmapping_amd/csrc/sm_k_pass.h
+++ b/surfelmapping_amd/csrc/sm_k_pass.h
@@ -604,6 +604,7 @@
     const uint32_t ntiles = (N + TILE - 1) / TILE;
     const uint32_t pend = st->pend, cap_prev = st->cap_binds, g_in = st->garbage, old_first = st->first_live;
     const bool dirty = st->fl_dirty2[fp.par] != 0u;
+    const uint32_t sq = st->sq_static;
     PendFields pf;
     pf.cull_n = st->cull_n; pf.garbage_prev = st->garbage_prev; pf.n_kill = st->n_kill; pf.visible = st->visible_count;
     pf.conflict = st->conflict_count; pf.n_static = st->n_static; pf.conf_skipped = st->n_conf_skipped;
@@ -677,7 +678,8 @@
     if (threadIdx.x == 0) {
         st->n_conf_skipped = cskip_tot;
         st->n_splat_skipped = sskip_tot;
-        st->n_static = N;
+        st->n_static = sq ? min(N, sq - 1u) : N;
+        if (sq) st->sq_static = 0u;
         st->conflict_count = min(ctotal, cap);
         if (fp.splat_follows) st->visible_count = 0;
         st->cull_n = N;
diff --git a/surfelmapping_amd/csrc/sm_slots.h b/surfelmapping_amd/csrc/sm_slots.h
--- a/surfelmapping_amd/csrc/sm_slots.h
+++ b/surfelmapping_amd/csrc/sm_slots.h
@@ -31,23 +31,25 @@
 
     bool period_due() const { return period_ <= 1 || culls_ + 1 >= period_; }
     bool bound_may_overflow() const { return (uint64_t)bound_ + max_new_ > cap_; }
-    bool decide_compact() const
+    enum class Due { none, period, forced };
+    bool decide_compact() const { return decide_due() != Due::none; }
+    Due decide_due() const
     {
-        if (period_ <= 1) return true;
+        if (period_ <= 1) return Due::forced;
         const auto t_start = std::chrono::steady_clock::now();
         for (uint32_t spins = 0;; ++spins) {
             const SlotStat st = read_stat();
             uint64_t bound = bound_;
             if (st.ahead_known) bound = std::min<uint64_t>(bound, (uint64_t)st.slots + (uint64_t)st.ahead * max_new_);
             if (bound + max_new_ <= cap_) break;
-            if (st.ahead <= 1u) return true;
-            if ((uint64_t)st.slots + 2ull * max_new_ > cap_) return true;
+            if (st.ahead <= 1u) return Due::forced;
+            if ((uint64_t)st.slots + 2ull * max_new_ > cap_) return Due::forced;
             if ((spins & 63u) == 63u &&
                 std::chrono::duration_cast<std::chrono::microseconds>(std::chrono::steady_clock::now() - t_start).count() > wait_us_)
-                return true;
+                return Due::forced;
             std::this_thread::yield();
         }
-        return period_due();
+        return period_due() ? Due::period : Due::none;
     }
 
     uint64_t estimate_slots()
@@ -69,6 +71,7 @@
         if (compacted) { culls_ = 0; }
         else { culls_++; garbage_ = true; }
     }
+    void squeezed_in_frame() { culls_ = 0; garbage_ = true; }
     void append_enqueued()
     {
         frames_enq_++;
```

Result: faster. 26360 frames/s (median of 6 runs) (+1.8%).
